# gabrielspmoreira/chameleon_recsys

Measured on AMD Instinct MI355X. Metric: NAR training sessions/sec, higher is better.
Workload: dtype f32

## Files before the change

### chameleon_recsys_amd/_lib.py

```python
import ctypes
import os
from ctypes import c_double, c_float, c_int, c_int32, c_int64, c_long, c_size_t, c_uint32, c_void_p

_HERE = os.path.dirname(os.path.abspath(__file__))
LIB_PATH = os.path.join(_HERE, "libchameleon_nar.so")

P = c_void_p

_SIGNATURES = {
    "cham_neg_sample_workspace_bytes": (c_size_t, [c_int, c_int, c_int]),
    "cham_neg_sample": (c_int, [P, c_int, c_int, P, c_int, c_uint32, c_uint32, c_int, c_int, c_int, c_int, P, P, P, P, P,
                                P, c_size_t, P]),
    "cham_ctx_assemble": (c_int, [P, P, c_int, P, c_int, P, P, P, P, P, P]),
    "cham_set_log_bases": (c_int, [c_float, c_float]),
    "cham_step_ints": (c_int, [P, P, P, P, c_int64, c_int, c_int, P, c_int, P, P, P, P, P, P]),
    "cham_item_dynamic_raw": (c_int, [P, P, c_int, P, P, P, P, P]),
    "cham_norm_stats_from_recent": (c_int, [P, c_int, c_int64, P, P, P, P, P]),
    "cham_norm_stats_from_buffer": (c_int, [P, c_int, c_int64, P, P, P, P, P]),
    "cham_norm_stats_from_rows": (c_int, [P, P, P, c_int, P, P]),
    "cham_row_weights": (c_int, [P, c_int, P, c_size_t, c_int, P, P, P, P]),
    "cham_item_assemble": (c_int, [P, c_int, c_int, c_int, P, c_int, P, c_int, P, P, P, P, c_int, P, P, P, P, P, P]),
    "cham_item_assemble_lds": (c_int, [P, c_int, c_int, c_int, P, c_int, P, c_int, P, P, P, P, c_int, P, c_int, P, c_int, P, P, P, P, P, P]),
    "cham_feature_bwd": (c_int, [P, P, c_int, c_int, P, P, P]),
    "cham_feature_bwd_workspace_bytes": (c_size_t, [c_int]),
    "cham_feature_bwd_ws": (c_int, [P, P, c_int, c_int, P, P, P, c_size_t, P]),
    "cham_emb_grad_scan": (c_int, [P, c_int, c_int, c_int, c_int, P, P, P, c_int, P, P]),
    "cham_group_rows_workspace_bytes": (c_size_t, [c_int]),
    "cham_group_rows_segments_len": (c_size_t, [c_int]),
    "cham_group_rows": (c_int, [P, c_int, c_int, P, P, P, c_size_t, P]),
    "cham_emb_grad_grouped": (c_int, [P, c_int, c_int, c_int, c_int, P, P, P, P, P, P]),
    "cham_dropout": (c_int, [P, P, c_long, c_int, c_int, c_float, c_uint32, c_uint32, c_int, c_int, c_int, P, c_int, c_int, c_int, c_int, P]),
    "cham_dense_rows": (c_int, [P, c_int, P, c_int, c_int, c_int, c_int, P, P, P]),
    "cham_gemm_f32": (c_int, [P, c_int, c_int, P, c_int, c_int, P, c_int, c_int, c_int, c_int, P, c_int, P, c_int, c_int,
                              P, c_int, c_int, c_int, P, c_size_t, c_int, P]),
    "cham_gemm_bf16": (c_int, [P, c_int, c_int, P, c_int, c_int, P, c_int, c_int, c_int, c_int, P, c_int, P, c_int, c_int,
                               P, c_int, c_int, c_int, P, c_size_t, c_int, P]),
    "cham_gemm_f32x3": (c_int, [P, c_int, c_int, P, c_int, c_int, P, c_int, c_int, c_int, c_int, P, c_int, P, c_int, c_int,
                                P, c_int, c_int, c_int, P, c_size_t, c_int, P]),
    "cham_gemm_f32x2h": (c_int, [P, c_int, c_int, P, c_int, c_int, P, c_int, c_int, c_int, c_int, P, c_int,
                                 P, c_int, c_int, c_int, P, c_size_t, c_int, P, P, P]),
    "cham_gemm_f32x3_set_variant": (None, [c_int]),
    "cham_gemm_f32x3_launch_counts": (None, [P, c_int]),
    "cham_gemm_p3": (c_int, [P, c_int64, c_int, P, c_int64, c_int, c_int, P, c_int, c_int, c_int, c_int, P, c_int, P, c_int, c_int, c_int,
                             P, c_size_t, c_int, P]),
    "cham_gemm_b16_dma": (c_int, [P, c_int, P, c_int, c_int, P, c_int, c_int, c_int, c_int, P, c_int, P, c_int, c_int, c_int, P, c_size_t, c_int, P]),
    "cham_gemm_p3_launch_counts": (None, [P, c_int]),
    "cham_gemm_b16_dma_set_nt_wide": (c_int, [c_int]),
    "cham_split3": (c_int, [P, c_int, c_int, c_int, P, c_int64, c_int, P, c_int64, c_int, P]),
    "cham_combine_fwd_p3": (c_int, [P, P, c_int, c_int, c_int, c_int, P, P, c_int64, P]),
    "cham_mulpred_bwd_p3": (c_int, [P, P, P, c_int, c_int, c_int, P, P, c_int64, P, P]),
    "cham_dm_mulpred_p3": (c_int, [P, c_int, c_int, P, c_int64, P, P, c_int, c_int, c_int, P, c_int64, P, P, P]),
    "cham_h2_scale_absmax": (c_int, [P, c_size_t, P, c_size_t, P, P]),
    "cham_h2_scale_rownorm": (c_int, [P, c_long, c_int, c_int, P, P, P]),
    "cham_h2_scale_rownorm2": (c_int, [P, c_long, c_int, c_int, P, P, P, P]),
    "cham_split2h": (c_int, [P, c_int, c_int, c_int, P, c_int64, c_int, P, c_int64, c_int, P, c_int, P]),
    "cham_gemm_h2": (c_int, [P, c_int64, c_int, P, P, c_int64, c_int, P, c_int, P, c_int, c_int, c_int, c_int, P, c_int, P, c_int, c_int, c_int,
                             P, c_size_t, c_int, P]),
    "cham_h2b_block_elements": (c_int, []),
    "cham_gemm_h2b": (c_int, [P, c_int64, c_int, P, P, c_int64, c_int, P, c_int, P, c_int, c_int, c_int, c_int, P, c_int, P, c_int, c_int, c_int,
                              P, c_size_t, c_int, c_int, c_int, c_int, P]),
    "cham_combine_fwd_h2b": (c_int, [P, P, c_int, c_int, c_int, c_int, P, P, c_int64, P, c_int, P]),
    "cham_dm_mulpred_h2_blk": (c_int, [P, c_int, c_int, P, c_int64, P, P, P, P, c_int, c_int, c_int, P, c_int64, P, P, P, P]),
    "cham_gemm_h2_launch_counts": (None, [P, c_int]),
    "cham_gemm_h2_set_nt_wide": (c_int, [c_int]),
    "cham_combine_fwd_h2": (c_int, [P, P, c_int, c_int, c_int, c_int, P, P, c_int64, P, P]),
    "cham_mulpred_bwd_h2": (c_int, [P, P, P, c_int, c_int, c_int, P, P, c_int64, P, P, P]),
    "cham_dm_mulpred_h2": (c_int, [P, c_int, c_int, P, c_int64, P, P, c_int, c_int, c_int, P, c_int64, P, P, P, P]),
    "cham_dm_mulpred_h2h": (c_int, [P, c_int, c_int, P, c_int64, P, P, P, P, c_int, c_int, c_int, P, c_int64, P, P, P, P]),
    "cham_dm_mulpred_b16": (c_int, [P, c_int, c_int, P, P, P, c_int, c_int, c_int, P, P, P, P]),
    "cham_gemm_b16": (c_int, [P, c_int, c_int, P, c_int, c_int, P, c_int, c_int, c_int, c_int, c_int, P, c_int, P, c_int, c_int, c_int,
                              P, c_size_t, c_int, P]),
    "cham_gemm_b16_set_variant": (None, [c_int]),
    "cham_gemm_b16_launch_counts": (None, [P, c_int]),
    "cham_gemm_set_variant": (None, [c_int]),
    "cham_gemm_launch_counts": (None, [P, c_int]),
    "cham_combine_fwd": (c_int, [P, P, c_int, c_int, c_int, c_int, P, P, c_long, c_long, P]),
    "cham_combine_bwd_workspace_bytes": (c_size_t, [c_int, c_int, c_int, c_int]),
    "cham_combine_bwd": (c_int, [P, c_int, c_int, c_int, c_int, P, P, P, P, c_size_t, P]),
    "cham_combine_bwd_gs": (c_int, [P, c_int, c_int, c_int, c_int, P, P, P, P, c_size_t, P, c_size_t, P]),
    "cham_gemm_h2_groupsum_bytes": (c_size_t, [c_int, c_int, c_int]),
    "cham_gemm_h2_dgrad_gs": (c_int, [P, c_int64, c_int, P, P, c_int64, c_int, P, P, c_int, c_int, c_int, c_int, P, c_int, c_int, c_int, c_int, P,
                                      c_size_t, P]),
    "cham_combine_fwd_b16": (c_int, [P, P, c_int, c_int, c_int, c_int, P, P, P]),
    "cham_combine_bwd_b16": (c_int, [P, P, c_int, c_int, c_int, c_int, P, P, P, P, c_size_t, P]),
    "cham_mulpred_bwd_b16": (c_int, [P, P, P, c_int, c_int, c_int, P, P]),
    "cham_mul_rows_b16": (c_int, [P, P, c_int, c_int, c_int, P, P]),
    "cham_score_softmax_fwd_b16": (c_int, [P, c_int, P, P, c_int, c_int, c_float, P, P, P, P, c_float, P, P, P, P]),
    "cham_score_softmax_bwd_b16": (c_int, [P, c_int, P, P, P, c_int, c_int, c_float, c_float, P, P, c_float, P, P, P, P, P]),
    "cham_colsum_b16": (c_int, [P, c_int, c_int, c_int, P, P, c_int, P, c_size_t, P]),
    "cham_cast_b16": (c_int, [P, c_int, c_int, P, P, P]),
    "cham_upcast_b16": (c_int, [P, c_size_t, P, P]),
    "cham_rnn_fwd": (c_int, [c_int, P, P, P, c_int, c_int, c_int, P, P, P, P, P, P, P]),
    "cham_rnn_bwd": (c_int, [c_int, P, P, P, c_int, c_int, c_int, P, P, P, P, P, P]),
    "cham_rnn_coop_workspace_bytes": (c_size_t, [c_int, c_int]),
    "cham_ugrnn_fwd_coop": (c_int, [P, P, P, c_int, c_int, c_int, P, P, P, P, P, c_size_t, P]),
    "cham_ugrnn_bwd_coop": (c_int, [P, P, P, c_int, c_int, c_int, P, P, P, P, P, c_size_t, P]),
    "cham_rnn_coop_timeouts": (c_int, [P, c_int, c_int, P]),
    "cham_ugrnn_point_fwd": (c_int, [P, P, P, c_int, c_int, c_int, c_int, P, P, P, P, P, P]),
    "cham_ugrnn_point_bwd": (c_int, [P, P, P, c_int, c_int, c_int, c_int, P, P, P, P, P, P, P]),
    "cham_transpose_f32": (c_int, [P, c_int, c_int, P, P]),
    "cham_rows_gather": (c_int, [P, P, c_long, c_int, P, P]),
    "cham_rows_scatter": (c_int, [P, P, c_long, c_int, P, P]),
    "cham_mulpred_bwd": (c_int, [P, P, P, c_int, c_int, c_int, P, P]),
    "cham_score_softmax_fwd": (c_int, [P, c_int, P, P, c_int, c_int, c_float, P, P, P, P, c_float, P, P, P, P]),
    "cham_score_softmax_bwd": (c_int, [P, c_int, P, P, P, c_int, c_int, c_float, c_float, P, P, c_float, P, P, P, P, P]),
    "cham_rank_items": (c_int, [P, P, P, P, c_int, c_int, P, P, P, P]),
    "cham_state_workspace_bytes": (c_size_t, [c_int, c_int]),
    "cham_state_update": (c_int, [P, P, c_int, c_int, c_double, P, P, c_int, P, P, P, c_int, c_int, P, P, c_size_t, P]),
    "cham_sumsq_partial": (c_int, [P, c_size_t, P, P]),
    "cham_loss_finalize": (c_int, [P, c_int, c_float, P, c_float, P, P]),
    "cham_adam_tf": (c_int, [P, P, P, P, c_size_t, c_size_t, c_float, c_float, c_float, c_float, c_float, P]),
    "cham_step_scalars_bytes": (c_int, []),
    "cham_step_scalars_set": (c_int, [P, c_uint32, c_uint32, c_int64, c_float, c_float, c_int, P]),
    "cham_neg_sample_dev": (c_int, [P, c_int, c_int, P, c_int, c_uint32, P, c_int, c_int, c_int, c_int, c_int, P, P, P, P, P, P, c_size_t, P]),
    "cham_step_ints_dev": (c_int, [P, P, P, P, P, c_int, c_int, P, c_int, P, P, P, P, P, P]),
    "cham_norm_stats_from_buffer_dev": (c_int, [P, c_int, P, P, P, P, P, P]),
    "cham_score_softmax_bwd_dev": (c_int, [P, c_int, P, P, P, c_int, c_int, c_float, P, P, P, c_float, P, P, P, P, P]),
    "cham_score_softmax_bwd_b16_dev": (c_int, [P, c_int, P, P, P, c_int, c_int, c_float, P, P, P, c_float, P, P, P, P, P]),
    "cham_loss_finalize_dev": (c_int, [P, c_int, P, P, c_float, P, P]),
    "cham_adam_tf_dev": (c_int, [P, P, P, P, c_size_t, c_size_t, c_float, P, c_float, c_float, c_float, P]),
    "cham_accumulate": (c_int, [P, P, c_size_t, c_int, P]),
    "cham_loss_accumulate": (c_int, [P, P, c_int, P]),
    "cham_colsum_workspace_bytes": (c_size_t, [c_int, c_int]),
    "cham_colsum": (c_int, [P, c_int, c_int, c_int, P, P, c_int, P, c_size_t, P]),
    "cham_eval_beyond_accuracy": (c_int, [P, c_int, P, P, c_int, P, c_int, c_int64, P, c_int, c_float, c_float, P, P, P, P]),
    "cham_eval_coverage_seed": (c_int, [P, c_int, c_int64, P, P, P]),
    "cham_eval_coverage_workspace_bytes": (c_size_t, [c_int64]),
    "cham_eval_coverage_count": (c_int, [P, P, c_int64, P, c_size_t, P, P]),
}

EXPORTED_SYMBOLS = tuple(_SIGNATURES.keys())


class ChameleonLibError(RuntimeError):
    pass


_lib = None


def load():
    global _lib
    if _lib is not None:
        return _lib
    if not os.path.exists(LIB_PATH):
        raise ChameleonLibError(
            "HIP extension %s is missing - run `python -c 'import __graft_entry__ as g; g.build()'` "
            "(hipcc --offload-arch=gfx950).  There is no CPU fallback." % LIB_PATH)
    lib = ctypes.CDLL(LIB_PATH)
    for name, (res, args) in _SIGNATURES.items():
        fn = getattr(lib, name)
        fn.restype = res
        fn.argtypes = args
    lib.cham_gemm_h2_set_nt_wide(1 if os.environ.get("CHAM_H2_NT_WIDE", "1") == "1" else 0)
    lib.cham_gemm_b16_dma_set_nt_wide(1 if os.environ.get("CHAM_B16_NT_WIDE", "1") == "1" else 0)
    _lib = lib
    return lib


def check(rc, what):
    if rc != 0:
        raise ChameleonLibError("%s failed with code %d" % (what, rc))


def ptr(t):
# ... 2 lines not shown
```

### chameleon_recsys_amd/csrc/common.h

```cpp
#pragma once
#include <hip/hip_runtime.h>
#include <stdint.h>

#define CHAM_OK 0
#define CHAM_ERR_ARG 22
#define CHAM_ERR_LAUNCH 5

#define CHAM_CHECK_LAUNCH()                                  \
    do {                                                     \
        hipError_t e__ = hipGetLastError();                  \
        if (e__ != hipSuccess) return -CHAM_ERR_LAUNCH;      \
    } while (0)

#include <atomic>
static inline int cham_set_dynamic_lds(const void* kernel, int bytes, std::atomic<unsigned long long>& mask) {
    int dev = 0;
    if (hipGetDevice(&dev) != hipSuccess) return -CHAM_ERR_LAUNCH;
    const unsigned long long bit = 1ull << (dev & 63);
    if (mask.load(std::memory_order_acquire) & bit) return CHAM_OK;
    if (hipFuncSetAttribute(kernel, hipFuncAttributeMaxDynamicSharedMemorySize, bytes) != hipSuccess) return -CHAM_ERR_LAUNCH;
    mask.fetch_or(bit, std::memory_order_release);
    return CHAM_OK;
}
#define CHAM_SET_DYNAMIC_LDS(kernel, bytes)                                                                  \
// ... 50 lines not shown
    for (int r = 0; r < 10; ++r) {
        const uint64_t p0 = (uint64_t)0xD2511F53u * c0;
        const uint64_t p1 = (uint64_t)0xCD9E8D57u * c2;
        const uint32_t n0 = (uint32_t)(p1 >> 32) ^ c1 ^ k0;
        const uint32_t n1 = (uint32_t)p1;
        const uint32_t n2 = (uint32_t)(p0 >> 32) ^ c3 ^ k1;
        const uint32_t n3 = (uint32_t)p0;
        c0 = n0; c1 = n1; c2 = n2; c3 = n3;
        k0 += 0x9E3779B9u; k1 += 0xBB67AE85u;
    }
    return c0;
}
#define CHAM_INF_KEY 0xFFFFFFFFFFFFFFFFull
__device__ __forceinline__ uint64_t philox_sort_key(uint32_t q, uint32_t j, uint32_t b, uint32_t stage,
                                                    uint32_t seed, uint32_t step) {
    return ((uint64_t)philox_rand32(q, j, b, stage, seed, step) << 32) | (uint64_t)q;
}

__device__ __forceinline__ float4 ld4(const float* p) { return *reinterpret_cast<const float4*>(p); }
__device__ __forceinline__ void st4(float* p, const float4& v) { *reinterpret_cast<float4*>(p) = v; }
__device__ __forceinline__ float4 ld4(const __bf16* p) {
    const uint2 u = *reinterpret_cast<const uint2*>(p);
    return make_float4(__uint_as_float(u.x << 16), __uint_as_float(u.x & 0xFFFF0000u), __uint_as_float(u.y << 16),
                       __uint_as_float(u.y & 0xFFFF0000u));
}
__device__ __forceinline__ void st4(__bf16* p, const float4& v) {
    typedef __bf16 bf16x4_t __attribute__((ext_vector_type(4)));
    bf16x4_t b; b[0] = (__bf16)v.x; b[1] = (__bf16)v.y; b[2] = (__bf16)v.z; b[3] = (__bf16)v.w;
    *reinterpret_cast<bf16x4_t*>(p) = b;
}

__device__ __forceinline__ void split3(float a, __bf16& h, __bf16& m, __bf16& l) {
    h = (__bf16)a;
    float r = a - (float)h;
    m = (__bf16)r;
    r -= (float)m;
    l = (__bf16)r;
}

__device__ __forceinline__ void st4_planes(__bf16* p, long long ps, const float4& v) {
    typedef __bf16 bf16x4_t __attribute__((ext_vector_type(4)));
    bf16x4_t h, m, l;
    __bf16 a, b, c;
    split3(v.x, a, b, c); h[0] = a; m[0] = b; l[0] = c;
    split3(v.y, a, b, c); h[1] = a; m[1] = b; l[1] = c;
    split3(v.z, a, b, c); h[2] = a; m[2] = b; l[2] = c;
    split3(v.w, a, b, c); h[3] = a; m[3] = b; l[3] = c;
    *reinterpret_cast<bf16x4_t*>(p) = h;
    *reinterpret_cast<bf16x4_t*>(p + ps) = m;
    *reinterpret_cast<bf16x4_t*>(p + 2 * ps) = l;
}

struct H2Scale { float scale, inv, bound, pad; unsigned max_bits, ticket, pad1, pad2; };
__device__ __forceinline__ void split2h(float xs , _Float16& h, _Float16& l) {
    h = (_Float16)xs;
    l = (_Float16)(xs - (float)h);
}
__device__ __forceinline__ unsigned short h2_keep_sign(_Float16 h, float x) {
    const unsigned short b = __builtin_bit_cast(unsigned short, h);
    return (x > 0.f && b == 0) ? (unsigned short)1 : b;
}
#define H2B_ROWS 256
#define H2B_COLS 32
#ifndef H2B_PAD
#define H2B_PAD 0
#endif
#define H2B_BLOCK (H2B_ROWS * H2B_COLS + H2B_PAD)
__host__ __device__ __forceinline__ size_t h2b_index(size_t row, unsigned col, unsigned col_blocks) {
    return ((row >> 8) * col_blocks + (col >> 5)) * (size_t)H2B_BLOCK + (row & 255u) * H2B_COLS + (col & 31u);
}

__device__ __forceinline__ void st4_planes_h2(_Float16* p, long long ps, const float4& v, float s) {
    typedef unsigned short u16x4_t __attribute__((ext_vector_type(4)));
    typedef _Float16 f16x4_t __attribute__((ext_vector_type(4)));
    u16x4_t h; f16x4_t l;
    _Float16 a, b;
    split2h(v.x * s, a, b); h[0] = h2_keep_sign(a, v.x); l[0] = b;
    split2h(v.y * s, a, b); h[1] = h2_keep_sign(a, v.y); l[1] = b;
    split2h(v.z * s, a, b); h[2] = h2_keep_sign(a, v.z); l[2] = b;
    split2h(v.w * s, a, b); h[3] = h2_keep_sign(a, v.w); l[3] = b;
    *reinterpret_cast<u16x4_t*>(p) = h;
    *reinterpret_cast<f16x4_t*>(p + ps) = l;
}

__device__ __forceinline__ float wave_sum(float v) {
#pragma unroll
    for (int o = 32; o > 0; o >>= 1) v += __shfl_xor(v, o, 64);
    return v;
}
__device__ __forceinline__ float wave_max(float v) {
#pragma unroll
    for (int o = 32; o > 0; o >>= 1) v = fmaxf(v, __shfl_xor(v, o, 64));
    return v;
}
__device__ __forceinline__ float wave_min(float v) {
#pragma unroll
    for (int o = 32; o > 0; o >>= 1) v = fminf(v, __shfl_xor(v, o, 64));
    return v;
}
__device__ __forceinline__ float block_sum(float v, float* red) {
    const int lane = threadIdx.x & 63, w = threadIdx.x >> 6, nw = (blockDim.x + 63) >> 6;
    v = wave_sum(v);
    __syncthreads();
    if (lane == 0) red[w] = v;
    __syncthreads();
    float t = 0.f;
    for (int i = 0; i < nw; ++i) t += red[i];
    return t;
}
```

### chameleon_recsys_amd/csrc/gemm_h2.hip

```cpp
#include "gemm_shared.h"

typedef _Float16 half8 __attribute__((ext_vector_type(8)));
typedef short h2_s16x4 __attribute__((ext_vector_type(4)));

struct H2Params {
    const _Float16* A; const _Float16* B;
    long long a_ps, b_ps;
    int lda, ldb;
    const float* sa; const float* sb;
    float* C; int ldc;
    int M, N, K;
    const float* bias;
    const unsigned short* dref; int ldr;
    int kchunk, splits; float* partial;
    int nbm, nbn, xcd_split, accumulate;
    int a_tiles, b_tiles, r_blk;
    float* gsum; int ggrp, gsk;
};

#define H2_SLAB 8192
#define H2_STAGE (4 * H2_SLAB)
#define H2_RING 4

__device__ __forceinline__ u32x4 h2_rsrc(const void* base, unsigned bytes) {
    const unsigned long long a = (unsigned long long)base;
    u32x4 r;
    r.x = (unsigned)a; r.y = (unsigned)(a >> 32) & 0xFFFFu; r.z = bytes; r.w = 0x00020000u;
    return r;
}

__device__ __forceinline__ void h2_dma_stage(unsigned lds0, unsigned va, unsigned vb, const u32x4& ra0, const u32x4& ra1, const u32x4& rb0,
                                             const u32x4& rb1) {
    unsigned keep;
    const unsigned l1 = lds0 + H2_SLAB, l2 = lds0 + 2 * H2_SLAB, l3 = lds0 + 3 * H2_SLAB;
    asm volatile(
        "s_nop 4\n\t"
        "s_mov_b32 %0, m0\n\t"
        "s_mov_b32 m0, %1\n\ts_nop 0\n\tbuffer_load_dwordx4 %5, %7, 0 offen lds\n\t"
        "s_mov_b32 m0, %2\n\ts_nop 0\n\tbuffer_load_dwordx4 %5, %8, 0 offen lds\n\t"
        "s_mov_b32 m0, %3\n\ts_nop 0\n\tbuffer_load_dwordx4 %6, %9, 0 offen lds\n\t"
        "s_mov_b32 m0, %4\n\ts_nop 0\n\tbuffer_load_dwordx4 %6, %10, 0 offen lds\n\t"
        "s_mov_b32 m0, %0"
        : "=&s"(keep)
        : "s"(lds0), "s"(l1), "s"(l2), "s"(l3), "v"(va), "v"(vb), "s"(ra0), "s"(ra1), "s"(rb0), "s"(rb1)
        : "memory");
}

template <bool TN>
__device__ __forceinline__ half8 h2_frag(const unsigned char* __restrict__ s, unsigned hi_off = 4 * 512) {
    if constexpr (!TN) {
        return *reinterpret_cast<const half8*>(s);
    } else {
        typedef __attribute__((address_space(3))) h2_s16x4 lds_s4;
        const h2_s16x4 lo = __builtin_amdgcn_ds_read_tr16_b64_v4i16((lds_s4*)(s));
        const h2_s16x4 hi = __builtin_amdgcn_ds_read_tr16_b64_v4i16((lds_s4*)(s + hi_off));
        typedef short s16x8 __attribute__((ext_vector_type(8)));
        s16x8 v;
        v[0] = lo[0]; v[1] = lo[1]; v[2] = lo[2]; v[3] = lo[3]; v[4] = hi[0]; v[5] = hi[1]; v[6] = hi[2]; v[7] = hi[3];
        return __builtin_bit_cast(half8, v);
    }
}

__device__ __forceinline__ void h2_barrier() {
    __builtin_amdgcn_fence(__ATOMIC_RELEASE, "workgroup", "local");
    __builtin_amdgcn_s_waitcnt(0xc07f);
    __builtin_amdgcn_s_barrier();
    __builtin_amdgcn_fence(__ATOMIC_ACQUIRE, "workgroup", "local");
    __builtin_amdgcn_sched_barrier(0);
}

template <int EPI, int TM, int TNN>
__device__ __forceinline__ void h2_epilogue(const H2Params& p, floatx16 (&acc)[TM][TNN], int m0, int n0, int wm0, int wn0, int split, int lane) {
    int lane_e = lane;
    asm volatile("" : "+v"(lane_e));
    const int kl = lane_e >> 5, fl = lane_e & 31;
    const float ia = p.sa[1], ib = p.sb[1];
#pragma unroll
    for (int i = 0; i < TM; ++i)
#pragma unroll
        for (int j = 0; j < TNN; ++j)
#pragma unroll
            for (int e = 0; e < 16; ++e) acc[i][j][e] = (acc[i][j][e] * ia) * ib;
    if constexpr (EPI == 3) {
        const int limM = p.M - m0, limN = p.N - n0;
        const __amdgpu_buffer_rsrc_t cw = make_window(p.C + (size_t)m0 * p.ldc + n0);
        const bool rb = p.r_blk != 0;
        const __amdgpu_buffer_rsrc_t dw = make_window(rb ? p.dref + ((size_t)(m0 >> 8) * (size_t)(p.ldr >> 5) + (size_t)(n0 >> 5)) * H2B_BLOCK
                                                         : p.dref + (size_t)m0 * p.ldr + n0);
        const int rstride = rb ? 64 : p.ldr * 2;
        const bool gs = p.gsum != nullptr;
        const int G = gs ? p.ggrp : 1, rbase = m0 + wm0;
        float* gw = gs ? p.gsum + (size_t)(rbase >> 7) * (size_t)p.gsk * (size_t)p.N + n0 + wn0 + fl : nullptr;
        float cur[TNN], hik[TNN];
#pragma unroll
        for (int j = 0; j < TNN; ++j) { cur[j] = 0.f; hik[j] = 0.f; }
        int kk = 0;
        auto emit = [&]() {
#pragma unroll
            for (int j = 0; j < TNN; ++j) {
                const float x = cur[j] + __shfl_xor(cur[j], 32, 64);
                if (kl == 0 && wn0 + j * 32 + fl < limN) gw[(size_t)kk * p.N + j * 32] = x;
            }
            ++kk;
        };
        int bnd = 64;
        auto block_begin = [&](int i) {
            if (!gs) return;
            const int s0 = rbase + 32 * i, gf = s0 / G;
            bnd = (gf + 1) * G - s0;
            if (i > 0 && bnd == G) {
                emit();
#pragma unroll
                for (int j = 0; j < TNN; ++j) cur[j] = 0.f;
            }
        };
        auto block_add = [&](int j, const float (&v)[16]) {
            if (!gs) return;
            float lo = 0.f;
            if (bnd >= 32) {
#pragma unroll
                for (int e = 0; e < 16; ++e) lo += v[e];
            } else {
                float hi = 0.f;
#pragma unroll
                for (int e = 0; e < 16; ++e) {
                    const bool first = (e & 3) + 8 * (e >> 2) + 4 * kl < bnd;
                    lo += first ? v[e] : 0.f;
                    hi += first ? 0.f : v[e];
                }
                hik[j] = hi;
            }
            cur[j] += lo;
        };
        auto block_end = [&]() {
            if (!gs || bnd >= 32) return;
            emit();
#pragma unroll
            for (int j = 0; j < TNN; ++j) cur[j] = hik[j];
        };
        if (limM >= wm0 + TM * 32 && limN >= wn0 + TNN * 32) {
#pragma unroll
            for (int i = 0; i < TM; ++i) {
                block_begin(i);
#pragma unroll
                for (int j = 0; j < TNN; ++j) {
                    const unsigned col = (unsigned)(wn0 + j * 32 + fl), rowb = (unsigned)(wm0 + i * 32 + 4 * kl);
                    const unsigned voff = (rowb * (unsigned)p.ldc + col) * 4u;
                    const unsigned voffr = rb ? (unsigned)((wn0 >> 5) + j) * (unsigned)(H2B_BLOCK * 2) + rowb * 64u + (unsigned)fl * 2u
                                              : (rowb * (unsigned)p.ldr + col) * 2u;
                    unsigned short y[16];
#pragma unroll
                    for (int e = 0; e < 16; ++e) {
                        const int ce = (e & 3) + 8 * (e >> 2);
                        y[e] = __builtin_amdgcn_raw_buffer_load_b16(dw, voffr, ce * rstride, 0);
                    }
                    float v[16];
#pragma unroll
                    for (int e = 0; e < 16; ++e) {
                        const int ce = (e & 3) + 8 * (e >> 2);
                        v[e] = acc[i][j][e] * ((short)y[e] > 0 ? 1.f : 0.2f);
                        __builtin_amdgcn_raw_buffer_store_b32(__float_as_uint(v[e]), cw, voff, ce * p.ldc * 4, 0);
                    }
                    block_add(j, v);
                }
                block_end();
            }
            if (gs) emit();
            return;
        }
#pragma unroll
        for (int i = 0; i < TM; ++i) {
            block_begin(i);
#pragma unroll
            for (int j = 0; j < TNN; ++j) {
                const int col = wn0 + j * 32 + fl;
                const bool cok = col < limN;
                unsigned short y[16];
                unsigned offs[16];
#pragma unroll
                for (int e = 0; e < 16; ++e) {
                    const int row = wm0 + i * 32 + (e & 3) + 8 * (e >> 2) + 4 * kl;
                    const bool ok = cok && row < limM;
                    offs[e] = ok ? ((unsigned)row * (unsigned)p.ldc + (unsigned)col) * 4u : OOB_OFF;
                    const unsigned ro = rb ? (unsigned)((wn0 >> 5) + j) * (unsigned)(H2B_BLOCK * 2) + (unsigned)row * 64u + (unsigned)fl * 2u
                                           : ((unsigned)row * (unsigned)p.ldr + (unsigned)col) * 2u;
                    y[e] = __builtin_amdgcn_raw_buffer_load_b16(dw, ok ? ro : OOB_OFF, 0, 0);
                }
                float v[16];
#pragma unroll
                for (int e = 0; e < 16; ++e) {
                    v[e] = acc[i][j][e] * ((short)y[e] > 0 ? 1.f : 0.2f);
                    __builtin_amdgcn_raw_buffer_store_b32(__float_as_uint(v[e]), cw, offs[e], 0, 0);
                }
                block_add(j, v);
            }
            block_end();
        }
        if (gs) emit();
    } else {
        GemmParams g;
        g.A = nullptr; g.B = nullptr; g.C = p.C; g.M = p.M; g.N = p.N; g.K = p.K; g.lda = 0; g.ldb = 0; g.ldc = p.ldc;
        g.bias = p.bias; g.act = ACT_NONE; g.dref = nullptr; g.ldr = 0; g.dact = ACT_NONE; g.rs = nullptr; g.ldrs = 0; g.rs_div = 1;
        g.accumulate = p.accumulate; g.kchunk = p.kchunk; g.splits = p.splits; g.partial = p.partial; g.nbm = p.nbm; g.nbn = p.nbn; g.xcd_split = p.xcd_split;
        gemm_epilogue<EPI, TM, TNN>(g, acc, m0, n0, wm0, wn0, split, kl, fl);
    }
}

template <bool TN, int EPI>
__global__ __launch_bounds__(512) void gemm_h2_kernel(H2Params p) {
    constexpr int BM = 256, BN = 256, BK = 16, TM = 4, TNN = 2;
    extern __shared__ __attribute__((aligned(1024))) unsigned char h2_smem[];

    const int nwg = p.nbm * p.nbn;
    int tile_m, tile_n, split;
    if (p.xcd_split) {
        const int lin = blockIdx.x + gridDim.x * blockIdx.y, slot = lin >> 3;
        split = (lin & 7) + 8 * (slot / nwg);
        const int t = slot % nwg;
        tile_m = t / p.nbn; tile_n = t % p.nbn;
    } else {
        const int id = blockIdx.x;
        const int q = nwg / 8, rr = nwg % 8, xcd = id % 8;
        const int swz = (xcd < rr ? xcd * (q + 1) : rr * (q + 1) + (xcd - rr) * q) + id / 8;
        tile_m = swz / p.nbn; tile_n = swz % p.nbn;
        split = blockIdx.y;
    }
    const int m0 = tile_m * BM, n0 = tile_n * BN;
    const int kbeg = split * p.kchunk;
    const int kend = min(p.K, kbeg + p.kchunk);
    const int nk = (kend - kbeg + BK - 1) / BK;
    const int lane = threadIdx.x & 63, wave = __builtin_amdgcn_readfirstlane(threadIdx.x >> 6);
    const int wm0 = (wave >> 2) * 128, wn0 = (wave & 3) * 64;

    u32x4 ra[2], rb[2];
    unsigned va, vb, stepa, stepb;
    unsigned tba = 0, tbb = 0;
    int klim = 0;
    if constexpr (!TN) {
        const size_t aall = (size_t)max(p.M - m0, 0) * p.lda * 2, ball = (size_t)max(p.N - n0, 0) * p.ldb * 2, koff = (size_t)kbeg * 2;
        const size_t abytes = aall > koff ? aall - koff : 0, bbytes = ball > koff ? ball - koff : 0;
#pragma unroll
        for (int q = 0; q < 2; ++q) {
            ra[q] = h2_rsrc(p.A + q * p.a_ps + (size_t)m0 * p.lda + kbeg, (unsigned)min(abytes, (size_t)0xFFFFFFF0u));
            rb[q] = h2_rsrc(p.B + q * p.b_ps + (size_t)n0 * p.ldb + kbeg, (unsigned)min(bbytes, (size_t)0xFFFFFFF0u));
        }
        const int row = 32 * wave + (lane >> 1), half = (lane & 1) ^ ((lane >> 4) & 1);
        va = ((unsigned)row * (unsigned)p.lda + 8u * half) * 2u;
        vb = ((unsigned)row * (unsigned)p.ldb + 8u * half) * 2u;
        stepa = stepb = BK * 2;
    } else {
        const size_t abytes = (size_t)max(kend - kbeg, 0) * p.lda * 2, bbytes = (size_t)max(kend - kbeg, 0) * p.ldb * 2;
        const int k = 2 * wave + (lane >> 5), jp = lane & 31, j = ((((jp >> 2) ^ (k & 3)) << 2) | (jp & 3));
        klim = kend - kbeg - (lane >> 2);
        if (p.a_tiles > 0) {
            tba = (unsigned)(p.lda >> 5) * (unsigned)(H2B_BLOCK * 2);
            const size_t t0 = (size_t)(kbeg >> 8), all = ((size_t)p.a_tiles - t0) * tba, skip = (size_t)(m0 >> 5) * (H2B_BLOCK * 2);
#pragma unroll
            for (int q = 0; q < 2; ++q)
                ra[q] = h2_rsrc(p.A + q * p.a_ps + (t0 * (size_t)(p.lda >> 5) + (size_t)(m0 >> 5)) * H2B_BLOCK, (unsigned)min(all > skip ? all - skip : (size_t)0, (size_t)0xFFFFFFF0u));
            va = (unsigned)wave * (unsigned)(H2B_BLOCK * 2) + (unsigned)lane * 16u;
        } else {
#pragma unroll
            for (int q = 0; q < 2; ++q)
                ra[q] = h2_rsrc(p.A + q * p.a_ps + (size_t)kbeg * p.lda + m0, (unsigned)min(abytes > (size_t)m0 * 2 ? abytes - (size_t)m0 * 2 : (size_t)0, (size_t)0xFFFFFFF0u));
            va = ((unsigned)k * (unsigned)p.lda + 8u * j) * 2u;
        }
        if (p.b_tiles > 0) {
            tbb = (unsigned)(p.ldb >> 5) * (unsigned)(H2B_BLOCK * 2);
            const size_t t0 = (size_t)(kbeg >> 8), all = ((size_t)p.b_tiles - t0) * tbb, skip = (size_t)(n0 >> 5) * (H2B_BLOCK * 2);
#pragma unroll
            for (int q = 0; q < 2; ++q)
                rb[q] = h2_rsrc(p.B + q * p.b_ps + (t0 * (size_t)(p.ldb >> 5) + (size_t)(n0 >> 5)) * H2B_BLOCK, (unsigned)min(all > skip ? all - skip : (size_t)0, (size_t)0xFFFFFFF0u));
            vb = (unsigned)wave * (unsigned)(H2B_BLOCK * 2) + (unsigned)lane * 16u;
        } else {
#pragma unroll
            for (int q = 0; q < 2; ++q)
                rb[q] = h2_rsrc(p.B + q * p.b_ps + (size_t)kbeg * p.ldb + n0, (unsigned)min(bbytes > (size_t)n0 * 2 ? bbytes - (size_t)n0 * 2 : (size_t)0, (size_t)0xFFFFFFF0u));
            vb = ((unsigned)k * (unsigned)p.ldb + 8u * j) * 2u;
        }
        stepa = (unsigned)BK * (unsigned)p.lda * 2u; stepb = (unsigned)BK * (unsigned)p.ldb * 2u;
// ... 367 lines not shown
                       reinterpret_cast<H2Scale*>(rec_plain));
    CHAM_CHECK_LAUNCH();
    return CHAM_OK;
}
extern "C" int cham_h2_scale_rownorm(const float* X, long R, int K, int ld, const float* factor, void* rec, void* stream) {
    return cham_h2_scale_rownorm2(X, R, K, ld, factor, rec, nullptr, stream);
}

__global__ __launch_bounds__(256) void k_split2h(const float* __restrict__ X, int R, int Cc, int ld, _Float16* __restrict__ dst, long long ps,
                                                 int ldd, _Float16* __restrict__ dstT, long long psT, int lddT, const H2Scale* __restrict__ rec) {
    const float s = rec->scale;
    const size_t n = (size_t)R * Cc;
    for (size_t i = (size_t)blockIdx.x * 256 + threadIdx.x; i < n; i += (size_t)gridDim.x * 256) {
        const int r = (int)(i / Cc), c = (int)(i % Cc);
        const float x = X[(size_t)r * ld + c];
        _Float16 h, l;
        split2h(x * s, h, l);
        const unsigned short hb = h2_keep_sign(h, x);
        if (dst) { _Float16* d = dst + (size_t)r * ldd + c; *reinterpret_cast<unsigned short*>(d) = hb; d[ps] = l; }
        if (dstT) { _Float16* d = dstT + (size_t)c * lddT + r; *reinterpret_cast<unsigned short*>(d) = hb; d[psT] = l; }
    }
}

extern "C" int cham_split2h(const float* X, int R, int Cc, int ld, void* dst, long long plane_stride, int ldd, void* dstT,
                            long long plane_strideT, int lddT, void* rec, int recompute, void* stream) {
    if (!X || R <= 0 || Cc <= 0 || (!dst && !dstT) || !rec || ((uintptr_t)rec & 15)) return -CHAM_ERR_ARG;
    const size_t n = (size_t)R * Cc;
    if (recompute) {
        if (ld != Cc || (n & 3) || ((uintptr_t)X & 15)) return -CHAM_ERR_ARG;
        const int rc = cham_h2_scale_absmax(X, n, nullptr, 0, rec, stream);
        if (rc != CHAM_OK) return rc;
    }
    int blocks = (int)((n + 255) / 256);
    if (blocks > 8192) blocks = 8192;
    hipLaunchKernelGGL(k_split2h, dim3(blocks), dim3(256), 0, (hipStream_t)stream, X, R, Cc, ld, reinterpret_cast<_Float16*>(dst), plane_stride,
                       ldd, reinterpret_cast<_Float16*>(dstT), plane_strideT, lddT, reinterpret_cast<const H2Scale*>(rec));
    CHAM_CHECK_LAUNCH();
    return CHAM_OK;
}

extern "C" int cham_h2b_block_elements(void) { return H2B_BLOCK; }

static long long g_h2_launches[8];
extern "C" void cham_gemm_h2_launch_counts(long long* out8, int reset) {
    for (int i = 0; i < 8; ++i) { if (out8) out8[i] = g_h2_launches[i]; if (reset) g_h2_launches[i] = 0; }
}

static int g_h2_nt_wide = 1;
extern "C" int cham_gemm_h2_set_nt_wide(int on) { const int was = g_h2_nt_wide; g_h2_nt_wide = on ? 1 : 0; return was; }

template <int EPI, bool ABLK>
static int h2w_launch_l(H2Params& p, hipStream_t st) {
    g_h2_launches[6] = EPI; g_h2_launches[7] = 1; ++g_h2_launches[2];
    if (ABLK) ++g_h2_launches[3];
    constexpr int smem = 2 * H2W_BUF;
    auto k = gemm_h2w_kernel<EPI, ABLK>;
    CHAM_SET_DYNAMIC_LDS(k, smem);
    hipLaunchKernelGGL(k, dim3(p.nbm * p.nbn, 1, 1), dim3(512), smem, st, p);
    CHAM_CHECK_LAUNCH();
    return CHAM_OK;
}
template <int EPI>
static int h2w_launch(H2Params& p, hipStream_t st) {
    return p.a_tiles > 0 ? h2w_launch_l<EPI, true>(p, st) : h2w_launch_l<EPI, false>(p, st);
}

template <bool TN, int EPI>
static int h2_launch(H2Params& p, hipStream_t st) {
    g_h2_launches[6] = EPI; g_h2_launches[7] = p.splits;
    constexpr int smem = H2_RING * H2_STAGE;
    auto k = gemm_h2_kernel<TN, EPI>;
    CHAM_SET_DYNAMIC_LDS(k, smem);
    hipLaunchKernelGGL(k, dim3(p.nbm * p.nbn, p.splits, 1), dim3(512), smem, st, p);
    CHAM_CHECK_LAUNCH();
    return CHAM_OK;
}
extern "C" size_t cham_gemm_h2_groupsum_bytes(int M, int N, int group_rows) {
    if (M <= 0 || N <= 0 || group_rows < 32) return 0;
    return (size_t)2 * ((M + 255) / 256) * (size_t)(127 / group_rows + 2) * (size_t)N * sizeof(float);
}
static int h2_run(const void* A, long long a_plane_stride, int lda, const float* a_scale, const void* B, long long b_plane_stride,
                  int ldb, const float* b_scale, int tn, float* C, int ldc, int M, int N, int K, const float* bias, int act,
                  const void* dref_h, int ldr, int dact, int accumulate, float* workspace, size_t workspace_bytes, int splits_hint,
                  int a_tiles, int b_tiles, int dref_blocked, int group_rows, float* groupsum, size_t groupsum_bytes, void* stream) {
    if (!A || !B || !C || !a_scale || !b_scale || M <= 0 || N <= 0 || K <= 0 || a_tiles < 0 || b_tiles < 0) return -CHAM_ERR_ARG;
    if (groupsum && (tn || !dref_h || group_rows < 32 || groupsum_bytes < cham_gemm_h2_groupsum_bytes(M, N, group_rows) || ((uintptr_t)groupsum & 15)))
        return -CHAM_ERR_ARG;
    {
        const long a_rows = tn ? K : M, b_rows = tn ? K : N;
        if (a_tiles && ((lda & 31) || (long)a_tiles * 256 < a_rows || a_plane_stride < (long long)a_tiles * (lda >> 5) * H2B_BLOCK)) return -CHAM_ERR_ARG;
        if (b_tiles && ((ldb & 31) || (long)b_tiles * 256 < b_rows || b_plane_stride < (long long)b_tiles * (ldb >> 5) * H2B_BLOCK)) return -CHAM_ERR_ARG;
        if (!tn && (b_tiles || (a_tiles && (lda != K || (K & 31) || !g_h2_nt_wide)))) return -CHAM_ERR_ARG;
        if (dref_blocked && (!dref_h || (ldr & 31) || tn)) return -CHAM_ERR_ARG;
    }
    if ((lda & 7) || (ldb & 7) || (a_plane_stride & 7) || (b_plane_stride & 7) || (N & 3) || (ldc & 3)) return -CHAM_ERR_ARG;
    if (((uintptr_t)A | (uintptr_t)B | (uintptr_t)C) & 15) return -CHAM_ERR_ARG;
    if ((size_t)ldc * 4 * 256 >= WINDOW_BYTES || (size_t)ldr * 2 * 256 >= WINDOW_BYTES) return -CHAM_ERR_ARG;
    H2Params p;
    p.A = reinterpret_cast<const _Float16*>(A); p.B = reinterpret_cast<const _Float16*>(B); p.a_ps = a_plane_stride; p.b_ps = b_plane_stride;
    p.lda = lda; p.ldb = ldb; p.sa = a_scale; p.sb = b_scale; p.C = C; p.ldc = ldc; p.M = M; p.N = N; p.K = K; p.bias = bias;
    p.dref = reinterpret_cast<const unsigned short*>(dref_h); p.ldr = ldr; p.partial = workspace; p.xcd_split = 0; p.accumulate = 0;
    p.nbm = (M + 255) / 256; p.nbn = (N + 255) / 256;
    p.a_tiles = a_tiles; p.b_tiles = b_tiles; p.r_blk = dref_blocked ? 1 : 0;
    p.gsum = groupsum; p.ggrp = group_rows; p.gsk = groupsum ? 127 / group_rows + 2 : 0;
    hipStream_t st = (hipStream_t)stream;
    if (!tn) {
        if ((K & 15) || accumulate) return -CHAM_ERR_ARG;
        if ((size_t)256 * lda * 2 >= (1ull << 31) || (size_t)256 * ldb * 2 >= (1ull << 31)) return -CHAM_ERR_ARG;
        p.kchunk = K; p.splits = 1;
        if (dref_h && (bias || act != ACT_NONE || dact != ACT_LEAKY)) return -CHAM_ERR_ARG;
        if (act != ACT_NONE && !(bias && act == ACT_TANH)) return -CHAM_ERR_ARG;
        ++g_h2_launches[0];
        if (groupsum) ++g_h2_launches[5];
        if (g_h2_nt_wide && (K & 31) == 0) {
            if (dref_h) return h2w_launch<3>(p, st);
            if (bias) return act == ACT_TANH ? h2w_launch<2>(p, st) : h2w_launch<5>(p, st);
            return h2w_launch<0>(p, st);
        }
        if (dref_h) return h2_launch<false, 3>(p, st);
        if (bias) return act == ACT_TANH ? h2_launch<false, 2>(p, st) : h2_launch<false, 5>(p, st);
        return h2_launch<false, 0>(p, st);
    }
    if ((M & 255) || (N & 255) || bias || act != ACT_NONE || dref_h) return -CHAM_ERR_ARG;
    if ((size_t)16 * lda * 2 >= (1ull << 31) || (size_t)16 * ldb * 2 >= (1ull << 31)) return -CHAM_ERR_ARG;
    const long tiles = (long)p.nbm * p.nbn;
    int splits = 1;
    if (splits_hint != 1 && workspace) {
        long want = splits_hint > 1 ? splits_hint : (tiles >= 192 ? 1 : (256 + tiles - 1) / tiles);
        const long maxk = (K + 511) / 512;
        if (want > maxk) want = maxk;
        const long maxw = (long)(workspace_bytes / ((size_t)M * N * sizeof(float)));
        if (want > maxw) want = maxw;
        if (splits_hint <= 0 && want >= 8) want = want / 8 * 8;
        if (want > 1) splits = (int)want;
    }
    int kchunk = (K + splits - 1) / splits;
    kchunk = ((kchunk + 15) / 16) * 16;
    p.kchunk = kchunk;
    p.splits = (K + kchunk - 1) / kchunk;
    if ((size_t)kchunk * (lda > ldb ? lda : ldb) * 2 >= 0xFFFFFFF0ull) return -CHAM_ERR_ARG;
    if ((a_tiles || b_tiles) && ((size_t)kchunk + 512 + 64) * (size_t)(lda > ldb ? lda : ldb) * 2 >= 0xFFFFFFF0ull) return -CHAM_ERR_ARG;
    ++g_h2_launches[1];
    if (a_tiles || b_tiles) ++g_h2_launches[4];
    if (p.splits > 1) {
        p.xcd_split = (p.splits % 8 == 0) ? 1 : 0;
        const int rc = h2_launch<true, 6>(p, st);
        if (rc != CHAM_OK) return rc;
        GemmParams g;
        g.A = nullptr; g.B = nullptr; g.C = C; g.M = M; g.N = N; g.K = K; g.lda = 0; g.ldb = 0; g.ldc = ldc; g.bias = nullptr; g.act = ACT_NONE;
        g.dref = nullptr; g.ldr = 0; g.dact = ACT_NONE; g.rs = nullptr; g.ldrs = 0; g.rs_div = 1; g.accumulate = accumulate;
        g.kchunk = kchunk; g.splits = p.splits; g.partial = workspace; g.nbm = p.nbm; g.nbn = p.nbn; g.xcd_split = p.xcd_split;
        launch_splitk_reduce(g, st);
        CHAM_CHECK_LAUNCH();
        return CHAM_OK;
    }
    p.accumulate = accumulate;
    return h2_launch<true, 0>(p, st);
}

extern "C" int cham_gemm_h2b(const void* A, long long a_plane_stride, int lda, const float* a_scale, const void* B, long long b_plane_stride,
                             int ldb, const float* b_scale, int tn, float* C, int ldc, int M, int N, int K, const float* bias, int act,
                             const void* dref_h, int ldr, int dact, int accumulate, float* workspace, size_t workspace_bytes, int splits_hint,
                             int a_tiles, int b_tiles, int dref_blocked, void* stream) {
    return h2_run(A, a_plane_stride, lda, a_scale, B, b_plane_stride, ldb, b_scale, tn, C, ldc, M, N, K, bias, act, dref_h, ldr, dact, accumulate,
                  workspace, workspace_bytes, splits_hint, a_tiles, b_tiles, dref_blocked, 0, nullptr, 0, stream);
}
extern "C" int cham_gemm_h2_dgrad_gs(const void* A, long long a_plane_stride, int lda, const float* a_scale, const void* B, long long b_plane_stride,
                                     int ldb, const float* b_scale, float* C, int ldc, int M, int N, int K, const void* dref_h, int ldr,
                                     int a_tiles, int dref_blocked, int group_rows, float* groupsum, size_t groupsum_bytes, void* stream) {
    if (!groupsum) return -CHAM_ERR_ARG;
    return h2_run(A, a_plane_stride, lda, a_scale, B, b_plane_stride, ldb, b_scale, 0, C, ldc, M, N, K, nullptr, ACT_NONE, dref_h, ldr, ACT_LEAKY, 0,
                  nullptr, 0, 1, a_tiles, 0, dref_blocked, group_rows, groupsum, groupsum_bytes, stream);
}

extern "C" int cham_gemm_h2(const void* A, long long a_plane_stride, int lda, const float* a_scale, const void* B, long long b_plane_stride,
                            int ldb, const float* b_scale, int tn, float* C, int ldc, int M, int N, int K, const float* bias, int act,
                            const void* dref_h, int ldr, int dact, int accumulate, float* workspace, size_t workspace_bytes, int splits_hint,
                            void* stream) {
    return cham_gemm_h2b(A, a_plane_stride, lda, a_scale, B, b_plane_stride, ldb, b_scale, tn, C, ldc, M, N, K, bias, act, dref_h, ldr, dact, accumulate,
                         workspace, workspace_bytes, splits_hint, 0, 0, 0, stream);
}
```

### chameleon_recsys_amd/csrc/scorer.hip

```cpp
#include "common.h"

__device__ __forceinline__ int cand_vrow(int bt, int c, int BT, int N, int pmax, const int* __restrict__ neg_slot) {
    if (c == 0) return BT + bt;
    int s = neg_slot[(size_t)bt * N + (c - 1)];
    if (s < 0) s = pmax;
    return 2 * BT + s;
}

__global__ __launch_bounds__(256) void k_combine_fwd(const float* __restrict__ U, const float* __restrict__ V, int C,
                                                     int BT, int N, int pmax, const int* __restrict__ neg_slot,
                                                     float* __restrict__ Z1, int row_begin) {
    const int row = row_begin + blockIdx.x;
    int u, v;
    if (row < BT) { u = row; v = row; }
    else {
        const int i = row - BT, bt = i / (N + 1), c = i % (N + 1);
        u = bt; v = cand_vrow(bt, c, BT, N, pmax, neg_slot);
    }
    const float4* pu = reinterpret_cast<const float4*>(U + (size_t)u * C);
    const float4* pv = reinterpret_cast<const float4*>(V + (size_t)v * C);
    float4* po = reinterpret_cast<float4*>(Z1 + (size_t)row * C);
    for (int k = threadIdx.x; k < C / 4; k += 256) {
        const float4 a = pu[k], b = pv[k];
        float4 o;
// ... 5 lines not shown

template <typename T>
__global__ __launch_bounds__(256) void k_combine_fwd_cand(const float* __restrict__ U, const float* __restrict__ V, int C,
                                                          int BT, int N, int pmax, const int* __restrict__ neg_slot,
                                                          T* __restrict__ Z1c ) {
    const int bt = blockIdx.x, NC = N + 1;
    const float4* pu = reinterpret_cast<const float4*>(U + (size_t)bt * C);
    T* po = Z1c + (size_t)bt * NC * C;
    for (int k = threadIdx.x; k < C / 4; k += 256) {
        const float4 a = pu[k];
        for (int c0 = 0; c0 < NC; c0 += 4) {
            float4 b[4];
#pragma unroll
            for (int i = 0; i < 4; ++i) {
                const int c = c0 + i < NC ? c0 + i : NC - 1;
                b[i] = reinterpret_cast<const float4*>(V + (size_t)cand_vrow(bt, c, BT, N, pmax, neg_slot) * C)[k];
            }
#pragma unroll
            for (int i = 0; i < 4; ++i) {
                if (c0 + i >= NC) break;
                float4 o;
                o.x = act_fwd(a.x + b[i].x, ACT_LEAKY); o.y = act_fwd(a.y + b[i].y, ACT_LEAKY);
                o.z = act_fwd(a.z + b[i].z, ACT_LEAKY); o.w = act_fwd(a.w + b[i].w, ACT_LEAKY);
                st4(po + (size_t)(c0 + i) * C + 4 * k, o);
            }
        }
    }
}

__global__ __launch_bounds__(256) void k_combine_fwd_cand_p3(const float* __restrict__ U, const float* __restrict__ V, int C,
                                                             int BT, int N, int pmax, const int* __restrict__ neg_slot,
                                                             __bf16* __restrict__ Z1p , long long ps) {
    const int bt = blockIdx.x, NC = N + 1;
    const float4* pu = reinterpret_cast<const float4*>(U + (size_t)bt * C);
    __bf16* po = Z1p + (size_t)bt * NC * C;
    for (int k = threadIdx.x; k < C / 4; k += 256) {
        const float4 a = pu[k];
        for (int c0 = 0; c0 < NC; c0 += 4) {
            float4 b[4];
#pragma unroll
            for (int i = 0; i < 4; ++i) {
                const int c = c0 + i < NC ? c0 + i : NC - 1;
                b[i] = reinterpret_cast<const float4*>(V + (size_t)cand_vrow(bt, c, BT, N, pmax, neg_slot) * C)[k];
            }
#pragma unroll
            for (int i = 0; i < 4; ++i) {
                if (c0 + i >= NC) break;
                float4 o;
                o.x = act_fwd(a.x + b[i].x, ACT_LEAKY); o.y = act_fwd(a.y + b[i].y, ACT_LEAKY);
                o.z = act_fwd(a.z + b[i].z, ACT_LEAKY); o.w = act_fwd(a.w + b[i].w, ACT_LEAKY);
                st4_planes(po + (size_t)(c0 + i) * C + 4 * k, ps, o);
            }
        }
    }
}

__global__ __launch_bounds__(256) void k_combine_fwd_cand_h2(const float* __restrict__ U, const float* __restrict__ V, int C,
                                                             int BT, int N, int pmax, const int* __restrict__ neg_slot,
                                                             _Float16* __restrict__ Z1p , long long ps,
                                                             const H2Scale* __restrict__ rec, int blocked) {
    const int bt = blockIdx.x, NC = N + 1;
    const float sc = rec->scale;
    const float4* pu = reinterpret_cast<const float4*>(U + (size_t)bt * C);
    _Float16* po = Z1p + (size_t)bt * NC * C;
    const size_t grow0 = (size_t)bt * NC;
    const unsigned ncb = (unsigned)C >> 5;
    for (int k = threadIdx.x; k < C / 4; k += 256) {
        const float4 a = pu[k];
        for (int c0 = 0; c0 < NC; c0 += 4) {
            float4 b[4];
#pragma unroll
            for (int i = 0; i < 4; ++i) {
                const int c = c0 + i < NC ? c0 + i : NC - 1;
                b[i] = reinterpret_cast<const float4*>(V + (size_t)cand_vrow(bt, c, BT, N, pmax, neg_slot) * C)[k];
            }
#pragma unroll
            for (int i = 0; i < 4; ++i) {
                if (c0 + i >= NC) break;
                float4 o;
                o.x = act_fwd(a.x + b[i].x, ACT_LEAKY); o.y = act_fwd(a.y + b[i].y, ACT_LEAKY);
                o.z = act_fwd(a.z + b[i].z, ACT_LEAKY); o.w = act_fwd(a.w + b[i].w, ACT_LEAKY);
                st4_planes_h2(blocked ? Z1p + h2b_index(grow0 + (size_t)(c0 + i), 4u * (unsigned)k, ncb) : po + (size_t)(c0 + i) * C + 4 * k, ps, o, sc);
            }
        }
    }
}

template <typename T>
__global__ __launch_bounds__(256) void k_combine_bwd_u(const float* __restrict__ dpre_in, const T* __restrict__ dpre_cand, int C, int BT,
                                                       int N, float* __restrict__ dU, float* __restrict__ dV) {
    const int bt = blockIdx.x;
    const float4* pin = reinterpret_cast<const float4*>(dpre_in + (size_t)bt * C);
    const T* pc = dpre_cand + (size_t)bt * (N + 1) * C;
    for (int k = threadIdx.x; k < C / 4; k += 256) {
        const float4 a = pin[k];
        const float4 p0 = ld4(pc + 4 * k);
        float4 s = make_float4(a.x + p0.x, a.y + p0.y, a.z + p0.z, a.w + p0.w);
        for (int c = 1; c <= N; c += 8) {
            float4 x[8];
#pragma unroll
            for (int u = 0; u < 8; ++u) x[u] = ld4(pc + (size_t)min(c + u, N) * C + 4 * k);
#pragma unroll
            for (int u = 0; u < 8; ++u)
                if (c + u <= N) { s.x += x[u].x; s.y += x[u].y; s.z += x[u].z; s.w += x[u].w; }
        }
        reinterpret_cast<float4*>(dU + (size_t)bt * C)[k] = s;
        reinterpret_cast<float4*>(dV + (size_t)bt * C)[k] = a;
        reinterpret_cast<float4*>(dV + ((size_t)BT + bt) * C)[k] = p0;
    }
}

__global__ __launch_bounds__(256) void k_combine_bwd_u_gs(const float* __restrict__ dpre_in, const float* __restrict__ dpre_cand, int C, int BT,
                                                          int N, const float* __restrict__ gsum, float* __restrict__ dU, float* __restrict__ dV) {
    const int bt = blockIdx.x, G = N + 1, gsk = 127 / G + 2;
    const long r0 = (long)bt * G, r1 = r0 + G - 1;
    const int q0 = (int)(r0 >> 7), q1 = (int)(r1 >> 7);
    const float4* pin = reinterpret_cast<const float4*>(dpre_in + (size_t)bt * C);
    const float4* pc = reinterpret_cast<const float4*>(dpre_cand + (size_t)r0 * C);
    for (int k = threadIdx.x; k < C / 4; k += 256) {
        const float4 a = pin[k], p0 = pc[k];
        float4 s = a;
        for (int q = q0; q <= q1; ++q) {
            const int piece = bt - (int)(((long)q << 7) / G);
            const float4 x = reinterpret_cast<const float4*>(gsum + ((size_t)q * gsk + piece) * C)[k];
            s.x += x.x; s.y += x.y; s.z += x.z; s.w += x.w;
        }
        reinterpret_cast<float4*>(dU + (size_t)bt * C)[k] = s;
        reinterpret_cast<float4*>(dV + (size_t)bt * C)[k] = a;
        reinterpret_cast<float4*>(dV + ((size_t)BT + bt) * C)[k] = p0;
    }
}

#define SLOT_HOT 512
#define SLOT_LIST 2048
__global__ __launch_bounds__(256) void k_slot_bitmap(const int* __restrict__ neg_slot, size_t n, int N, int pmax, int W,
                                                     unsigned* __restrict__ bitmap ) {
    const size_t i = (size_t)blockIdx.x * 256 + threadIdx.x;
    if (i >= n) return;
    const int s = neg_slot[i];
    if (s < 0 || s >= pmax) return;
    const unsigned p = (unsigned)(i / N);
    atomicOr(bitmap + (size_t)s * W + (p >> 5), 1u << (p & 31));
}

__device__ __forceinline__ int block_sum_int(int v, int* red ) {
#pragma unroll
    for (int o = 32; o > 0; o >>= 1) v += __shfl_xor(v, o, 64);
    __syncthreads();
    if ((threadIdx.x & 63) == 0) red[threadIdx.x >> 6] = v;
    __syncthreads();
    return red[0] + red[1] + red[2] + red[3];
}

template <typename T>
__global__ __launch_bounds__(256) void k_slot_reduce(const T* __restrict__ cand , int C, int BT, int N,
                                                     const int* __restrict__ neg_slot, const unsigned* __restrict__ bitmap, int W,
                                                     int nslots, float* __restrict__ partial ,
                                                     float* __restrict__ dV) {
    __shared__ int list[SLOT_HOT];
    __shared__ int red[4];
    const int s = blockIdx.x, chunk = blockIdx.y, tid = threadIdx.x, lane = tid & 63, wave = tid >> 6;
    const unsigned* bm = bitmap + (size_t)s * W;
    int c = 0;
    for (int w = tid; w < W; w += 256) c += __popc(bm[w]);
    const int total = block_sum_int(c, red);
    const bool hot = total > SLOT_HOT;
// ... 307 lines not shown
__global__ __launch_bounds__(256) void k_score_softmax_bwd(const T* __restrict__ S3, const float* __restrict__ w4,
                                                           const float* __restrict__ probs, const unsigned char* __restrict__ mask,
                                                           int BT, int N, float scale ,
                                                           float* __restrict__ ds, T* __restrict__ dS3, float nov_factor,
                                                           const int64_t* __restrict__ neg_ids, const float* __restrict__ pop_norm,
                                                           const float* __restrict__ logits, float inv_tau,
                                                           const float* __restrict__ nov_aux, float inv_log2_base,
                                                           const ChamStepScalars* __restrict__ sc, float tau) {
    const size_t row = (size_t)blockIdx.x * 256 + threadIdx.x;
    const int NC = N + 1;
    if (row >= (size_t)BT * NC) return;
    if (sc) scale = 1.0f / (tau * sc->sum_mask);
    const int bt = (int)(row / NC), c = (int)(row % NC);
    float g = mask[bt] ? (probs[row] - (c == 0 ? 1.f : 0.f)) * scale : 0.f;
    if (nov_factor > 0.f && c > 0 && mask[bt]) {
        const float q = expf(logits[row] * inv_tau - nov_aux[(size_t)bt * 3]) / nov_aux[(size_t)bt * 3 + 1];
        const float nov_c = -log2f(pop_norm[neg_ids[(size_t)bt * N + (c - 1)]]) * inv_log2_base;
        g -= nov_factor * scale * q * (nov_c - nov_aux[(size_t)bt * 3 + 2]);
    }
    ds[row] = g;
    const T* r = S3 + row * K3;
    T* o = dS3 + row * K3;
#pragma unroll
    for (int k = 0; k < K3 / 4; ++k) {
        const float4 x = ld4(r + 4 * k);
        float4 y;
        y.x = g * w4[4 * k] * act_bwd_from_out(x.x, ACT_LEAKY);
        y.y = g * w4[4 * k + 1] * act_bwd_from_out(x.y, ACT_LEAKY);
        y.z = g * w4[4 * k + 2] * act_bwd_from_out(x.z, ACT_LEAKY);
        y.w = g * w4[4 * k + 3] * act_bwd_from_out(x.w, ACT_LEAKY);
        st4(o + 4 * k, y);
    }
}


__global__ __launch_bounds__(256) void k_rank_items(const float* __restrict__ probs, const int64_t* __restrict__ label_next,
                                                    const int64_t* __restrict__ neg_ids, const unsigned char* __restrict__ mask,
                                                    int BT, int N, int64_t* __restrict__ pred_ids, float* __restrict__ pred_probs,
                                                    int32_t* __restrict__ label_rank) {
    extern __shared__ float sp[];
    const int lane = threadIdx.x & 63, w = threadIdx.x >> 6, bt = blockIdx.x * 4 + w;
    const int NC = N + 1;
    float* p = sp + (size_t)w * NC;
    if (bt < BT)
        for (int c = lane; c < NC; c += 64) p[c] = probs[(size_t)bt * NC + c];
    __syncthreads();
    if (bt >= BT) return;
    for (int c = lane; c < NC; c += 64) {
        const float pc = p[c];
        int r = 0;
        for (int j = 0; j < NC; ++j) {
            const float pj = p[j];
            r += (pj > pc) || (pj == pc && j < c);
        }
        pred_ids[(size_t)bt * NC + r] = c == 0 ? label_next[bt] : neg_ids[(size_t)bt * N + (c - 1)];
        pred_probs[(size_t)bt * NC + r] = pc;
        if (c == 0) label_rank[bt] = mask[bt] ? r : -1;
    }
}

extern "C" int cham_combine_fwd(const float* U, const float* V, int C, int BT, int N, int pmax, const int32_t* neg_slot,
                                float* Z1, long row_begin, long row_count, void* stream) {
    if (!U || !V || !neg_slot || !Z1 || (C & 3) || BT <= 0 || N <= 0) return -CHAM_ERR_ARG;
    const long rows = (long)BT + (long)BT * (N + 1);
    if (row_begin < 0 || row_count <= 0 || row_begin + row_count > rows) return -CHAM_ERR_ARG;
    if (row_begin == BT && row_count == (long)BT * (N + 1))
        hipLaunchKernelGGL(k_combine_fwd_cand<float>, dim3((unsigned)BT), dim3(256), 0, (hipStream_t)stream, U, V, C, BT, N, pmax, neg_slot,
                           Z1 + (size_t)BT * C);
    else
        hipLaunchKernelGGL(k_combine_fwd, dim3((unsigned)row_count), dim3(256), 0, (hipStream_t)stream, U, V, C, BT, N, pmax,
                           neg_slot, Z1, (int)row_begin);
    CHAM_CHECK_LAUNCH();
    return CHAM_OK;
}
extern "C" int cham_combine_fwd_b16(const float* U, const float* V, int C, int BT, int N, int pmax, const int32_t* neg_slot,
                                    void* Z1c, void* stream) {
    if (!U || !V || !neg_slot || !Z1c || (C & 3) || BT <= 0 || N <= 0) return -CHAM_ERR_ARG;
    hipLaunchKernelGGL(k_combine_fwd_cand<__bf16>, dim3((unsigned)BT), dim3(256), 0, (hipStream_t)stream, U, V, C, BT, N, pmax, neg_slot,
                       reinterpret_cast<__bf16*>(Z1c));
    CHAM_CHECK_LAUNCH();
    return CHAM_OK;
}

static inline size_t al256(size_t x) { return (x + 255) & ~(size_t)255; }
struct SlotWs { size_t bitmap_bytes, partial_bytes, pad_bytes; int W, nchunk, nchunk_pad; };
static SlotWs slot_ws(int C, int BT, int N, int pmax) {
    SlotWs w;
    w.W = (BT + 31) / 32;
    w.nchunk = (w.W + SLOT_HOT / 32 - 1) / (SLOT_HOT / 32);
    w.nchunk_pad = (int)(((size_t)BT * N + SLOT_LIST - 1) / SLOT_LIST);
    w.bitmap_bytes = al256((size_t)pmax * w.W * sizeof(unsigned));
    w.partial_bytes = al256((size_t)w.nchunk * pmax * C * sizeof(float));
    w.pad_bytes = al256((size_t)w.nchunk_pad * C * sizeof(float));
    return w;
}
extern "C" size_t cham_combine_bwd_workspace_bytes(int C, int BT, int N, int pmax) {
    if (C <= 0 || BT <= 0 || N <= 0 || pmax <= 0) return 0;
    const SlotWs w = slot_ws(C, BT, N, pmax);
    return w.bitmap_bytes + w.partial_bytes + w.pad_bytes;
}

template <typename T>
static int combine_bwd_impl(const float* dpre_in, const T* dpre_cand, int C, int BT, int N, int pmax, const int32_t* neg_slot,
                            float* dU, float* dV, float* workspace, size_t workspace_bytes, void* stream, const float* gsum = nullptr) {
    if (!dpre_in || !dpre_cand || !neg_slot || !dU || !dV || !workspace || (C & 3) || BT <= 0 || N <= 0 || pmax <= 0) return -CHAM_ERR_ARG;
    if (workspace_bytes < cham_combine_bwd_workspace_bytes(C, BT, N, pmax) || ((uintptr_t)workspace & 15)) return -CHAM_ERR_ARG;
    hipStream_t st = (hipStream_t)stream;
    const SlotWs w = slot_ws(C, BT, N, pmax);
    unsigned* bitmap = reinterpret_cast<unsigned*>(workspace);
    float* partial = reinterpret_cast<float*>(reinterpret_cast<char*>(workspace) + w.bitmap_bytes);
    float* pad_partial = reinterpret_cast<float*>(reinterpret_cast<char*>(workspace) + w.bitmap_bytes + w.partial_bytes);
    const size_t n = (size_t)BT * N;
    if constexpr (sizeof(T) == 4) {
        if (gsum) hipLaunchKernelGGL(k_combine_bwd_u_gs, dim3(BT), dim3(256), 0, st, dpre_in, reinterpret_cast<const float*>(dpre_cand), C, BT, N, gsum, dU, dV);
        else hipLaunchKernelGGL(k_combine_bwd_u<T>, dim3(BT), dim3(256), 0, st, dpre_in, dpre_cand, C, BT, N, dU, dV);
    } else {
        hipLaunchKernelGGL(k_combine_bwd_u<T>, dim3(BT), dim3(256), 0, st, dpre_in, dpre_cand, C, BT, N, dU, dV);
    }
    if (hipMemsetAsync(bitmap, 0, (size_t)pmax * w.W * sizeof(unsigned), st) != hipSuccess) return -CHAM_ERR_LAUNCH;
    hipLaunchKernelGGL(k_slot_bitmap, dim3((unsigned)((n + 255) / 256)), dim3(256), 0, st, neg_slot, n, N, pmax, w.W, bitmap);
    hipLaunchKernelGGL(k_slot_reduce<T>, dim3(pmax, w.nchunk), dim3(256), 0, st, dpre_cand, C, BT, N, neg_slot, bitmap, w.W, pmax, partial, dV);
    hipLaunchKernelGGL(k_slot_final, dim3(pmax), dim3(256), 0, st, partial, C, pmax, w.nchunk, BT, bitmap, w.W, dV);
    hipLaunchKernelGGL(k_combine_bwd_slots_partial<T>, dim3(w.nchunk_pad), dim3(256), 0, st, dpre_cand, C, BT, N, neg_slot, pmax,
                       pad_partial, SLOT_LIST);
    hipLaunchKernelGGL(k_combine_bwd_pad_final, dim3(1), dim3(256), 0, st, pad_partial, C, w.nchunk_pad,
                       dV + ((size_t)2 * BT + pmax) * C);
    CHAM_CHECK_LAUNCH();
    return CHAM_OK;
}
extern "C" int cham_combine_bwd(const float* dpre, int C, int BT, int N, int pmax, const int32_t* neg_slot,
                                float* dU, float* dV, float* workspace, size_t workspace_bytes, void* stream) {
    if (!dpre || BT <= 0 || C <= 0) return -CHAM_ERR_ARG;
    return combine_bwd_impl<float>(dpre, dpre + (size_t)BT * C, C, BT, N, pmax, neg_slot, dU, dV, workspace, workspace_bytes, stream);
}
extern "C" int cham_combine_bwd_gs(const float* dpre, int C, int BT, int N, int pmax, const int32_t* neg_slot, float* dU, float* dV,
                                   float* workspace, size_t workspace_bytes, const float* groupsum, size_t groupsum_bytes, void* stream) {
    if (!dpre || BT <= 0 || C <= 0 || !groupsum || N + 1 < 32 || ((uintptr_t)groupsum & 15)) return -CHAM_ERR_ARG;
    const size_t rows = (size_t)BT * (N + 1);
    if (groupsum_bytes < (size_t)2 * ((rows + 255) / 256) * (size_t)(127 / (N + 1) + 2) * (size_t)C * sizeof(float)) return -CHAM_ERR_ARG;
    return combine_bwd_impl<float>(dpre, dpre + (size_t)BT * C, C, BT, N, pmax, neg_slot, dU, dV, workspace, workspace_bytes, stream, groupsum);
}
extern "C" int cham_combine_bwd_b16(const float* dpre_in, const void* dpre_cand, int C, int BT, int N, int pmax, const int32_t* neg_slot,
                                    float* dU, float* dV, float* workspace, size_t workspace_bytes, void* stream) {
    return combine_bwd_impl<__bf16>(dpre_in, reinterpret_cast<const __bf16*>(dpre_cand), C, BT, N, pmax, neg_slot, dU, dV, workspace,
                                    workspace_bytes, stream);
}

extern "C" int cham_mulpred_bwd(float* dM, const float* Z2c, const float* pred, int C, int BT, int N, float* dpred_pre,
                                void* stream) {
    if (!dM || !Z2c || !pred || !dpred_pre || (C & 3) || BT <= 0) return -CHAM_ERR_ARG;
    hipLaunchKernelGGL(k_mulpred_bwd<float>, dim3(BT), dim3(256), 0, (hipStream_t)stream, dM, Z2c, pred, C, N, dpred_pre);
    CHAM_CHECK_LAUNCH();
    return CHAM_OK;
}
extern "C" int cham_mulpred_bwd_b16(void* dM, const void* Z2c, const float* pred, int C, int BT, int N, float* dpred_pre, void* stream) {
    if (!dM || !Z2c || !pred || !dpred_pre || (C & 3) || BT <= 0) return -CHAM_ERR_ARG;
    hipLaunchKernelGGL(k_mulpred_bwd<__bf16>, dim3(BT), dim3(256), 0, (hipStream_t)stream, reinterpret_cast<__bf16*>(dM),
                       reinterpret_cast<const __bf16*>(Z2c), pred, C, N, dpred_pre);
    CHAM_CHECK_LAUNCH();
    return CHAM_OK;
}
extern "C" int cham_combine_fwd_p3(const float* U, const float* V, int C, int BT, int N, int pmax, const int32_t* neg_slot, void* Z1p,
                                   long long plane_stride, void* stream) {
    if (!U || !V || !neg_slot || !Z1p || C <= 0 || (C & 3) || BT < 0 || N < 0 || (plane_stride & 3)) return -CHAM_ERR_ARG;
    if (BT == 0) return CHAM_OK;
    hipLaunchKernelGGL(k_combine_fwd_cand_p3, dim3(BT), dim3(256), 0, (hipStream_t)stream, U, V, C, BT, N, pmax, neg_slot,
// ... 129 lines not shown
```

### chameleon_recsys_amd/nar/nar_model.py

```python
import math
import os

import numpy as np
import torch

from .. import _lib
from .. import _roctx
from .._lib import check, ptr
from .clicked_items_state import lane_stream
from .layout import COL_ITEMEMB, ParamLayout
from .metrics import BEYOND_ACCURACY_PER_CLICK, ItemCoverage

ACT_NONE, ACT_LEAKY, ACT_TANH = 0, 1, 2


class ModeKeys:
    TRAIN = 'train'
    EVAL = 'eval'
    PREDICT = 'infer'


_raw_stream = getattr(torch._C, '_cuda_getCurrentRawStream', None)
_raw_device = getattr(torch._C, '_cuda_getDevice', None)

# ... 50 lines not shown

    def __enter__(self):
        global _VARIABLE_STORE
        self._prev, _VARIABLE_STORE = _VARIABLE_STORE, self.store
        return self.store

    def __exit__(self, *a):
        global _VARIABLE_STORE
        _VARIABLE_STORE = self._prev


_TORCH_DTYPE = {np.dtype(n).str: t for n, t in (('int64', torch.int64), ('int32', torch.int32), ('float32', torch.float32),
                                                   ('uint8', torch.uint8))}


def pack_offsets(arrays, align=256):
    offs, total = {}, 0
    for k, a in arrays.items():
        offs[k] = total
        total += (a.nbytes + align - 1) & ~(align - 1)
    return offs, total


class _PinnedRing:

    def __init__(self, n=4, nbytes=4 << 20):
        self.n, self.nbytes = n, nbytes
        self.bufs, self.events, self.k, self.off = [None] * n, [None] * n, -1, 0

    def begin(self, need):
        self.k = (self.k + 1) % self.n
        if self.events[self.k] is not None:
            self.events[self.k].synchronize()
        if self.bufs[self.k] is None or self.bufs[self.k].numel() < need:
            self.bufs[self.k] = torch.empty(max(need, self.nbytes), dtype=torch.uint8, pin_memory=True)
        self.off = 0

    def stage(self, a):
        n = a.nbytes
        if n == 0 or self.off + n > self.bufs[self.k].numel():
            return torch.from_numpy(a)
        view = self.bufs[self.k][self.off:self.off + n]
        self.off += (n + 255) & ~255
        t = view.view(torch.from_numpy(a).dtype).view(a.shape)
        t.copy_(torch.from_numpy(a))
        return t

    def end(self, stream):
        ev = torch.cuda.Event()
        ev.record(stream)
        self.events[self.k] = ev


class NARRuntime:

    def __init__(self, params, device='cuda:0', seed=42, weights=None):
        self.lib = _lib.load()
        self._views = {}
        if not torch.cuda.is_available():
            raise _lib.ChameleonLibError("no ROCm device visible: the NAR step has no CPU path")
        self.device = torch.device(device)
        self.params = params
        acfg = params['articles_features_config']
        ace = np.ascontiguousarray(params['content_article_embeddings_matrix'], dtype=np.float32)
        self.n_items = acfg['article_id'].get('cardinality', ace.shape[0]) if 'article_id' in acfg else ace.shape[0]
        if self.n_items != ace.shape[0]:
            raise ValueError("article_id cardinality (%d) != ACE rows (%d)" % (self.n_items, ace.shape[0]))
        self.item_id_bits = max(1, int(self.n_items - 1).bit_length())
        self.layout = ParamLayout(params['session_features_config'], acfg, self.n_items, ace.shape[1],
                                  params['CAR_embedding_size'], params['rnn_units'],
                                  params.get('rnn_num_layers', 1), params.get('rnn_cell', 'ugrnn'),
                                  params.get('internal_features_config'), params.get('max_cardinality_for_ohe', 10))
        L = self.layout
        logical = weights if weights is not None else L.init_logical(seed)
        dev = self.device
        self.flat = torch.from_numpy(L.pack(logical)).to(dev)
        self.m = torch.zeros_like(self.flat)
        self.v = torch.zeros_like(self.flat)
        self.grads = torch.zeros_like(self.flat)
        self.global_step = 0
        self.dev_scalars = os.environ.get("CHAM_DEV_SCALARS", "1") == "1"
        self.loss_side = os.environ.get("CHAM_LOSS_SIDE", "1") == "1"
        self.dgrad_groupsum = os.environ.get("CHAM_DGRAD_GROUPSUM", "1") == "1"
        self.feature_bwd_ws = os.environ.get("CHAM_FEATURE_BWD_WS", "1") == "1"
        self.tail_split = os.environ.get("CHAM_TAIL_SPLIT", "1") == "1"
        self.capturing = False
        self.scalars = None
        self.gemm_dtype = params.get('gemm_dtype', 'f32')
        if self.gemm_dtype not in ('f32', 'f32_native', 'bf16'):
            raise ValueError("gemm_dtype must be 'f32', 'f32_native' or 'bf16'")
        self.x3 = self.gemm_dtype == 'f32' and os.environ.get("CHAM_GEMM_X3", "1") == "1"
        self.p3 = self.x3 and os.environ.get("CHAM_GEMM_P3", "1") == "1" and self.layout.C % 256 == 0
        self.h2 = self.p3 and os.environ.get("CHAM_GEMM_H2", "1") == "1"
        blk = os.environ.get("CHAM_H2_BLOCKED", "0")
        self.h2_blocked = (self.h2 and blk in ("1", "dz2", "z1") and os.environ.get("CHAM_H2_NT_WIDE", "1") == "1" and self.layout.C % 32 == 0)
        self.h2_blocked_which = blk if self.h2_blocked else "0"
        mode = os.environ.get("CHAM_S1_H2", "1") if self.h2 else "0"
        self.s1_h2 = mode in ("1", "a")
        self.dm_f16 = self.s1_h2
        self.s1_h2_fwd = mode == "a"
        self.tf_random_seed = int(params.get('tf_random_seed', 42))
        meta = params['articles_metadata']
        self.ace = torch.from_numpy(ace).to(dev)
        self.created = torch.from_numpy(np.ascontiguousarray(meta['created_at_ts'], dtype=np.int64)).to(dev)
        def meta_column(n):
            a = np.asarray(meta[n])
            if n in L.meta_is_float:
                return np.ascontiguousarray(a, dtype=np.float32).view(np.int32).astype(np.int64)
            if acfg[n]['type'] == 'numerical' and not np.issubdtype(a.dtype, np.integer) and not np.array_equal(a, np.round(a)):
                raise ValueError("article feature %r holds non-integer values but its config says dtype %r: declare it "
                                 "{'type': 'numerical', 'dtype': 'float'}" % (n, acfg[n].get('dtype')))
            return a.astype(np.int64)
        if L.meta_names:
            mc = np.stack([meta_column(n) for n in L.meta_names])
        else:
            mc = np.zeros((1, self.n_items), np.int64)
        self.meta_cat = torch.from_numpy(np.ascontiguousarray(mc)).to(dev)
        self.ctx_desc = torch.from_numpy(L.ctx_descriptors()).to(dev)
        self.ctx_emb_groups, self.item_emb_groups = L.ctx_emb_groups(), L.item_emb_groups()
        segs, singles = L.item_segments()
        self.item_segs, self.n_item_segs = torch.from_numpy(np.ascontiguousarray(segs)).to(dev), int(segs.shape[0])
        self.item_singles, self.n_item_singles = torch.from_numpy(np.ascontiguousarray(singles)).to(dev), int(singles.shape[0])
        self.item_lds = L.Fi * 4 * 8 <= 64 * 1024
        self.item_desc = torch.from_numpy(L.item_descriptors()).to(dev)
        self.gemm_ws = torch.empty(64 << 20, dtype=torch.float32, device=dev)
        self.colsum_ws = torch.empty(4 << 20, dtype=torch.float32, device=dev)
        self.side_stream = lane_stream(dev, "side", 0)
        self._side_raw = self.side_stream.cuda_stream
        self.gemm_ws_side = torch.empty(32 << 20, dtype=torch.float32, device=dev)
        self.colsum_ws_side = torch.empty(2 << 20, dtype=torch.float32, device=dev)
        self.wgrad_aux = os.environ.get("CHAM_WGRAD_AUX", "1") == "1"
        self.aux_stream = lane_stream(dev, "aux", 0)
        self._aux_raw = self.aux_stream.cuda_stream
        self.gemm_ws_aux = torch.empty(16 << 20, dtype=torch.float32, device=dev)
        self.colsum_ws_aux = torch.empty(2 << 20, dtype=torch.float32, device=dev)
        self.head_split = os.environ.get("CHAM_HEAD_SPLIT", "1") == "1"
        self.overlap = os.environ.get("CHAM_OVERLAP", "1") == "1"
        self.compact = os.environ.get("CHAM_COMPACT", "1") == "1"
        self.p3_w2_splits = 32
        self.w2_main_rows = 131072
        self.rnn_coop_rows = 131072 if (L.cell == 'ugrnn' and L.Hp == 256 and not L.rnn_stepwise) else -1
        self._rnn_coop_ws = {}
        self.presample = os.environ.get("CHAM_PRESAMPLE", "1") == "1"
        self.upload_stream = lane_stream(dev, "upload")
        self.pinned = _PinnedRing()
        self.sumsq = torch.zeros(1024, dtype=torch.float32, device=dev)
        self.b16 = self.gemm_dtype == 'bf16'
        self.shadow, self._shadow_key, self.weights_version = {}, None, 0
        if self.b16:
            if L.C % 128:
                raise ValueError("gemm_dtype='bf16' needs CAR_embedding_size % 128 == 0")
            for name in ('W2', 'Ws1', 'Ws2', 'Ws3'):
                r, c = L.entries[name].shape
                self.shadow[name] = torch.zeros(r, c, dtype=torch.bfloat16, device=dev)
                self.shadow[name + 'T'] = torch.zeros(c, r, dtype=torch.bfloat16, device=dev)
        self.b16_dma = self.gemm_dtype == 'bf16' and L.C % 256 == 0
        self.dm_fused_b16 = self.gemm_dtype == 'bf16' and L.entries['Ws1'].shape == (L.C, 128) and L.C % 64 == 0
        if self.p3:
            C_ = L.C
            npl, pdt = (2, torch.float16) if self.h2 else (3, torch.bfloat16)
            self.w2p = torch.zeros(npl, C_, C_, dtype=pdt, device=dev)
            self.w2tp = torch.zeros(npl, C_, C_, dtype=pdt, device=dev)
            if self.h2:
                self.sc_w2 = torch.zeros(8, dtype=torch.float32, device=dev)
                self.sc_ws1n = torch.zeros(8, dtype=torch.float32, device=dev)
                self.sc_unit = torch.tensor([16384.0, 1.0 / 16384.0, 1.0, 0, 0, 0, 0, 0], dtype=torch.float32, device=dev)
# ... 143 lines not shown
                     ws.numel() * 4 if ws is not None else 0, splits, _stream()), "cham_gemm_f32")
        if prof is not None:
            e1.record()
            c1 = self._tile_counts()
            tile = next((i for i in range(13) if c1[i] != c0[i]), -1)
            rec = dict(M=M, N=N, K=K, transA=transA, transB=transB, splits=int(c1[15]), act=act, dref=dref is not None, dact=dact,
                       bias=bias is not None, rowscale=rowscale is not None, bf16=bf16, tile=tile, epi=int(c1[14]), ev=(e0, e1))
            if x3:
                x1 = self._tile_counts_x3()
                xt = next((i for i in (0, 1, 2, 4, 5) if x1[i] != x0[i]), -1)
                if xt >= 0:
                    rec.update(x3=True, tile=xt & 3, x2h=xt >= 4, epi=int(x1[6]), splits=int(x1[7]))
            prof.append(rec)

    def _tile_counts(self):
        import ctypes
        out = (ctypes.c_longlong * 16)()
        self.lib.cham_gemm_launch_counts(out, 0)
        return list(out)

    def _tile_counts_x3(self):
        import ctypes
        out = (ctypes.c_longlong * 8)()
        self.lib.cham_gemm_f32x3_launch_counts(out, 0)
        return list(out)

    def gemm_b16(self, A, lda, transA, B, ldb, transB, C, ldc, out_f32, M, N, K, bias=None, act=ACT_NONE, dref=None, ldr=0,
                 dact=ACT_NONE, accumulate=0, splits=1, dma=False):
        ws = None
        if splits != 1:
            ws = self._lane_ws('gemm_ws')
        prof = self.profile
        if prof is not None:
            e0, e1 = torch.cuda.Event(enable_timing=True), torch.cuda.Event(enable_timing=True)
            c0 = self._tile_counts_b16()
            e0.record()
        if dma:
            if prof is not None:
                import ctypes
                cw0 = (ctypes.c_longlong * 8)()
                self.lib.cham_gemm_p3_launch_counts(cw0, 0)
            check(self.lib.cham_gemm_b16_dma(ptr(A), lda, ptr(B), ldb, transA, ptr(C), ldc, M, N, K, ptr(bias), act, ptr(dref), ldr, dact,
                                             accumulate, ptr(ws), ws.numel() * 4 if ws is not None else 0, splits, _stream()), "cham_gemm_b16_dma")
            if prof is not None:
                e1.record()
                import ctypes
                c = (ctypes.c_longlong * 8)()
                self.lib.cham_gemm_p3_launch_counts(c, 0)
                prof.append(dict(M=M, N=N, K=K, transA=transA, transB=transB, splits=int(c[7]), act=act, dref=dref is not None, dact=dact,
                                 bias=bias is not None, rowscale=False, bf16=True, b1=True, b1w=bool(c[4] > cw0[4]), out_f32=int(transA), tile=0, epi=int(c[6]),
                                 ev=(e0, e1)))
            return
        check(self.lib.cham_gemm_b16(ptr(A), lda, transA, ptr(B), ldb, transB, ptr(C), ldc, out_f32, M, N, K, ptr(bias), act, ptr(dref),
                                     ldr, dact, accumulate, ptr(ws), ws.numel() * 4 if ws is not None else 0, splits, _stream()),
              "cham_gemm_b16")
        if prof is not None:
            e1.record()
            c1 = self._tile_counts_b16()
            tile = next((i for i in range(5) if c1[i] != c0[i]), -1)
            prof.append(dict(M=M, N=N, K=K, transA=transA, transB=transB, splits=int(c1[7]), act=act, dref=dref is not None, dact=dact,
                             bias=bias is not None, rowscale=False, bf16=True, b16=True, out_f32=int(c1[5]), tile=tile, epi=int(c1[6]),
                             ev=(e0, e1)))

    def gemm_p3(self, A, a_ps, lda, B, b_ps, ldb, tn, C, ldc, M, N, K, bias=None, act=ACT_NONE, dref_h=None, ldr=0, dact=ACT_NONE,
                accumulate=0, splits=1):
        ws = None
        if splits != 1:
            ws = self._lane_ws('gemm_ws')
        prof = self.profile
        if prof is not None:
            e0, e1 = torch.cuda.Event(enable_timing=True), torch.cuda.Event(enable_timing=True)
            e0.record()
        check(self.lib.cham_gemm_p3(ptr(A), a_ps, lda, ptr(B), b_ps, ldb, tn, ptr(C), ldc, M, N, K, ptr(bias), act, ptr(dref_h), ldr, dact,
                                    accumulate, ptr(ws), ws.numel() * 4 if ws is not None else 0, splits, _stream()), "cham_gemm_p3")
        if prof is not None:
            e1.record()
            import ctypes
            c = (ctypes.c_longlong * 8)()
            self.lib.cham_gemm_p3_launch_counts(c, 0)
            prof.append(dict(M=M, N=N, K=K, transA=tn, transB=0 if tn else 1, splits=int(c[7]), act=act, dref=dref_h is not None, dact=dact,
                             bias=bias is not None, rowscale=False, bf16=False, p3=True, tile=0, epi=int(c[6]), ev=(e0, e1)))

    def gemm_h2(self, A, a_ps, lda, a_sc, B, b_ps, ldb, b_sc, tn, C, ldc, M, N, K, bias=None, act=ACT_NONE, dref_h=None, ldr=0, dact=ACT_NONE,
                accumulate=0, splits=1, a_tiles=0, b_tiles=0, dref_blocked=0, group_rows=0, groupsum=None):
        ws = None
        if splits != 1:
            ws = self._lane_ws('gemm_ws')
        prof = self.profile
        if prof is not None:
            import ctypes
            c0 = (ctypes.c_longlong * 8)()
            self.lib.cham_gemm_h2_launch_counts(c0, 0)
            e0, e1 = torch.cuda.Event(enable_timing=True), torch.cuda.Event(enable_timing=True)
            e0.record()
        if groupsum is not None:
            check(self.lib.cham_gemm_h2_dgrad_gs(ptr(A), a_ps, lda, ptr(a_sc), ptr(B), b_ps, ldb, ptr(b_sc), ptr(C), ldc, M, N, K, ptr(dref_h), ldr,
                                                 a_tiles, dref_blocked, group_rows, ptr(groupsum), groupsum.numel() * 4, _stream()), "cham_gemm_h2_dgrad_gs")
        else:
            check(self.lib.cham_gemm_h2b(ptr(A), a_ps, lda, ptr(a_sc), ptr(B), b_ps, ldb, ptr(b_sc), tn, ptr(C), ldc, M, N, K, ptr(bias), act, ptr(dref_h),
                                         ldr, dact, accumulate, ptr(ws), ws.numel() * 4 if ws is not None else 0, splits, a_tiles, b_tiles, dref_blocked,
                                         _stream()), "cham_gemm_h2b")
        if prof is not None:
            e1.record()
            c = (ctypes.c_longlong * 8)()
            self.lib.cham_gemm_h2_launch_counts(c, 0)
            prof.append(dict(M=M, N=N, K=K, transA=tn, transB=0 if tn else 1, splits=int(c[7]), act=act, dref=dref_h is not None, dact=dact,
                             bias=bias is not None, rowscale=False, bf16=False, h2=True, h2w=bool(c[2] > c0[2]), h2blk=bool(c[3] > c0[3]), tile=0, epi=int(c[6]), ev=(e0, e1)))

    def _tile_counts_b16(self):
        import ctypes
        out = (ctypes.c_longlong * 8)()
        self.lib.cham_gemm_b16_launch_counts(out, 0)
        return list(out)

    def colsum(self, X, ld, R, F, out, w=None, accumulate=0, b16=False):
        ws = self._lane_ws('colsum_ws')
        check((self.lib.cham_colsum_b16 if b16 else self.lib.cham_colsum)(ptr(X), ld, R, F, ptr(w), ptr(out), accumulate, ptr(ws),
                                                                           ws.numel() * 4, _stream()), "cham_colsum")

    def set_step_scalars(self, step=0, max_ts=0, sum_mask=1.0, lr_t=0.0, fields=7, stream=None):
        if self.capturing:
            return
        if self.scalars is None:
            self.scalars = torch.zeros(max(8, self.lib.cham_step_scalars_bytes() // 4), dtype=torch.int32, device=self.device)
        check(self.lib.cham_step_scalars_set(ptr(self.scalars), int(step) & 0xFFFFFFFF, (int(step) + 1) & 0xFFFFFFFF, int(max_ts), float(sum_mask),
                                             float(lr_t), fields, _stream() if stream is None else stream), "cham_step_scalars_set")

    def side(self):
        import contextlib
        return torch.cuda.stream(self.side_stream) if self.overlap else contextlib.nullcontext()

    def fork(self):
        if self.overlap:
            self.side_stream.wait_stream(torch.cuda.current_stream())

    def join(self):
        if self.overlap:
            torch.cuda.current_stream().wait_stream(self.side_stream)


def _h2b_block():
    from .. import _lib
    return int(_lib.load().cham_h2b_block_elements())


def blocked_plane_elements(tiles, C):
    return tiles * (C // 32) * _h2b_block()


def planes_from_blocked(t, tiles, C=None):
    npl = t.shape[0]
    C = t.shape[2] if C is None else C
    blk = _h2b_block()
    flat = t.reshape(npl, -1)[:, :tiles * (C // 32) * blk]
    return flat.reshape(npl, tiles, C // 32, blk)[..., :8192].reshape(npl, tiles, C // 32, 256, 32).permute(0, 1, 3, 2, 4).reshape(npl, tiles * 256, C)


def planes_to_blocked(t):
    npl, R, C = t.shape
    tiles = -(-R // 256)
    blk = _h2b_block()
    pad = torch.zeros(npl, tiles * 256, C, dtype=t.dtype, device=t.device)
    pad[:, :R] = t
    out = torch.zeros(npl, tiles, C // 32, blk, dtype=t.dtype, device=t.device)
    out[..., :8192] = pad.reshape(npl, tiles, 256, C // 32, 32).permute(0, 1, 3, 2, 4).reshape(npl, tiles, C // 32, 8192)
    return out.reshape(npl, -1), tiles


class StepPlan:

    @staticmethod
    def estimate_bytes(L, B, T, N, rt=None):
        rows = B * T * (N + 2)
        need = 4 * (4 * rows * L.C + 2 * rows * (128 + 64 + 32))
        if rt is not None and rt.p3:
            rc = B * T * (N + 1)
            need += 2 * (2 if rt.h2 else 3) * 2 * rc * L.C + 4 * B * T * L.C
            need += 4 * int(rt.lib.cham_group_rows_segments_len(2 * B * T + 20 * N + 1))
        return need

    def allocated_bytes(self):
        seen, total = set(), 0

        def walk(x):
            nonlocal total
            if torch.is_tensor(x):
                st = x.untyped_storage()
                if st.data_ptr() not in seen:
                    seen.add(st.data_ptr())
                    total += st.nbytes()
            elif isinstance(x, (list, tuple)):
                for y in x:
                    walk(y)
            elif isinstance(x, dict):
                for y in x.values():
                    walk(y)
        for v in vars(self).values():
            walk(v)
        return total

    def __init__(self, rt, B, T, N, n_buf, Bg):
        L, dev = rt.layout, rt.device
        self.B, self.T, self.N, self.n_buf, self.Bg = B, T, N, n_buf, Bg
        self.BT = BT = B * T
        self.NC = NC = N + 1
        self.Rc = Rc = BT * NC
        self.Rall = Rall = BT + Rc
        self.pmax = pmax = 20 * N
        self.RV = RV = 2 * BT + pmax + 1
        C, Hp, Fc, Fi = L.C, L.Hp, L.Fc, L.Fi
        self.C = C
        f32 = lambda *s: torch.empty(*s, dtype=torch.float32, device=dev)
        i64 = lambda *s: torch.zeros(*s, dtype=torch.int64, device=dev)
        self._samp = [dict(neg_ids=i64(B, T, N), neg_slot=torch.zeros(B, T, N, dtype=torch.int32, device=dev), pool=i64(pmax),
                           canon=torch.zeros(pmax, dtype=torch.int32, device=dev), meta=torch.zeros(4, dtype=torch.int32, device=dev))
                      for _ in range(2)]
        self.use_sampler_set(0)
        need = rt.lib.cham_combine_bwd_workspace_bytes(L.C, B * T, N, 20 * N)
        if need > rt.gemm_ws.numel() * 4:
            rt.gemm_ws = torch.empty((need + 3) // 4, dtype=torch.float32, device=dev)
        if need > rt.gemm_ws_side.numel() * 4:
            rt.gemm_ws_side = torch.empty((need + 3) // 4, dtype=torch.float32, device=dev)
        self.ws_bytes = rt.lib.cham_neg_sample_workspace_bytes(Bg * (T + 1), int(rt.params['recent_clicks_buffer_max_size']), n_buf)
        self.sampler_ws = torch.empty(self.ws_bytes, dtype=torch.uint8, device=dev)
        self.ids_all = i64(RV)
        self.ref_ts = i64(RV)
        self.rec_raw, self.nov_raw = f32(RV), f32(RV)
        self.stats = f32(3, 8)
        self.stat_scratch = f32(3 * max(1, int(rt.params['recent_clicks_for_normalization'])))
        self.w_rows = f32(RV)
        self.perm = torch.zeros(RV, dtype=torch.int32, device=dev)
        self.seg = torch.zeros(int(rt.lib.cham_group_rows_segments_len(RV)), dtype=torch.int32, device=dev)
        self.group_ws = torch.zeros(int(rt.lib.cham_group_rows_workspace_bytes(RV)) // 4, dtype=torch.int32, device=dev)
        self.Xc_raw, self.Xc_s, self.dXc = f32(BT, Fc), f32(BT, Fc), f32(BT, Fc)
        self.Xi_raw, self.Xi_s, self.dXi = f32(RV, Fi), f32(RV, Fi), f32(RV, Fi)
        self.U, self.dU = f32(BT, C), f32(BT, C)
        self.V, self.dV = f32(RV, C), f32(RV, C)
        b16 = rt.b16
        bf = lambda *s: torch.empty(*s, dtype=torch.bfloat16, device=dev)
        cand = bf if b16 else f32
        if b16:
            self.Z1, self.Z2, self.dZ2, self.dZ1 = f32(BT, C), f32(BT, C), f32(BT, C), f32(BT, C)
            self.Z1c, self.Z2c, self.dZ2c, self.dZ1c, self.Mc = bf(Rc, C), bf(Rc, C), bf(Rc, C), bf(Rc, C), bf(Rc, C)
            self.b2part = f32(BT, C)
        else:
            fused = rt.p3 and rt.dm_fused and 32 <= NC <= 256
            self.Z1 = f32(BT if rt.p3 else Rall, C)
            self.Z2 = f32(Rall, C)
            self.dZ2 = f32(BT if fused else Rall, C)
            self.dZ1 = f32(Rall, C)
        self.p3 = rt.p3
        self.h2 = rt.h2
        if rt.p3:
            self.z1_tiles = self.dz2_tiles = 0
            if rt.h2:
                tiles = -(-Rc // 256) + 1
                if rt.h2_blocked:
                    self.z1_tiles = tiles if rt.h2_blocked_which in ("1", "z1") else 0
                    self.dz2_tiles = tiles if (rt.dm_fused and 32 <= NC <= 256 and rt.h2_blocked_which in ("1", "dz2")) else 0
                self.Z1p = (torch.zeros(2, blocked_plane_elements(self.z1_tiles, C), dtype=torch.float16, device=dev) if self.z1_tiles
                            else torch.zeros(2, Rc, C, dtype=torch.float16, device=dev))
                self.dZ2p = (torch.zeros(2, blocked_plane_elements(self.dz2_tiles, C), dtype=torch.float16, device=dev) if self.dz2_tiles
                             else torch.zeros(2, Rc, C, dtype=torch.float16, device=dev))
                self.sc_z1 = torch.zeros(8, dtype=torch.float32, device=dev)
                self.sc_dz2 = torch.zeros(8, dtype=torch.float32, device=dev)
                self.sc_ds1 = torch.zeros(8, dtype=torch.float32, device=dev)
                self.gsum = (torch.empty(int(rt.lib.cham_gemm_h2_groupsum_bytes(Rc, C, NC)) // 4, dtype=torch.float32, device=dev)
                             if rt.dgrad_groupsum and NC >= 32 and Rc > 0 else None)
            else:
                self.Z1p, self.dZ2p = bf(3, Rc, C), bf(3, Rc, C)
            self.p3_ps = Rc * C
            self.z1_ps = self.Z1p[0].numel()
            self.dz2_ps = self.dZ2p[0].numel()
            self.b2part = f32(BT, C)
        self.seq_len = torch.zeros(B, dtype=torch.int32, device=dev)
        NG = L.NG
        self.xproj = [f32(BT, NG * Hp) for _ in range(L.L)]
        self.dxproj = f32(BT, NG * Hp)
        self.rnn_out = [f32(BT, Hp) for _ in range(L.L)]
        self.hprev = [f32(BT, Hp) for _ in range(L.L)]
        self.G = [f32(BT, Hp) for _ in range(L.L)]
        self.Cc = [f32(BT, Hp) for _ in range(L.L)]
        gru = L.cell == 'gru'
        self.R = [f32(BT, Hp) if gru else None for _ in range(L.L)]
        self.RH = [f32(BT, Hp) if gru else None for _ in range(L.L)]
        self.drnn = f32(BT, Hp)
        self.WhT = f32(NG * Hp, Hp)
        if L.rnn_stepwise:
            self.h_state, self.zh, self.carry = f32(B, Hp), f32(B, 2 * Hp), f32(B, Hp)
            self.dzs, self.direct = f32(B, 2 * Hp), f32(B, Hp)
        self.FC1, self.dFC1 = f32(BT, 512), f32(BT, 512)
        self.pred, self.dpred = f32(BT, C), f32(BT, C)
        self.S1, self.dS1 = cand(Rc, 128), cand(Rc, 128)
        self.S2, self.dS2 = cand(Rc, 64), cand(Rc, 64)
        self.S3, self.dS3 = cand(Rc, 32), cand(Rc, 32)
        self.ds = f32(Rc)
        self.logits, self.probs = f32(BT, NC), f32(BT, NC)
        self.nll = f32(BT)
        self.nov_aux = f32(BT, 3)
        self.mask = torch.zeros(BT, dtype=torch.uint8, device=dev)
        self.loss = torch.zeros(3, dtype=torch.float32, device=dev)
        self.neg_ids_c = i64(BT, N)
        self.neg_slot_c = torch.zeros(BT, N, dtype=torch.int32, device=dev)
        self.Z2f, self.rnn_c, self.drnn_c, self.dxproj_c = f32(BT, C), f32(BT, Hp), f32(BT, Hp), f32(BT, NG * Hp)
        self.pos, self.P = None, BT
        self.created = torch.cuda.Event()
        self.created.record()

    def ensure_rows(self, name):
        t = getattr(self, name)
        if t.shape[0] < self.Rall:
            t = torch.empty(self.Rall, t.shape[1], dtype=t.dtype, device=t.device)
            setattr(self, name, t)
            if hasattr(self, 'nbytes'):
                self.nbytes = self.allocated_bytes()
        return t

    def dropout_buffers(self, rt):
        if not rt.b16:
            self.ensure_rows('Z1'); self.ensure_rows('dZ2')
        if getattr(self, 'Xd', None) is None:
            L, dev = rt.layout, rt.device
            f32 = lambda *s: torch.empty(*s, dtype=torch.float32, device=dev)
            Fw = L.Fc + L.Fi
            self.Xd, self.dXd = f32(self.Rall, Fw), f32(self.Rall, Fw)
            self.dUx, self.dVx = f32(self.BT, Fw), f32(self.RV, Fw)
            self.FC1d = f32(self.BT, 512)
            self.rnn_drop = [f32(self.BT, L.Hp) for _ in range(L.L)]
            need = rt.lib.cham_combine_bwd_workspace_bytes(Fw, self.B * self.T, self.N, self.pmax)
            self.drop_ws = torch.empty((need + 3) // 4, dtype=torch.float32, device=dev)
            if rt.b16:
                self.Z1f, self.dZ1f = f32(self.Rall, L.C), f32(self.Rall, L.C)

    def cand_Z1(self, P=None):
        P = self.P if P is None else P
        n = P * self.NC
        if getattr(self, 'used_p3', False):
            if getattr(self, 'z1_tiles', 0):
                z = planes_from_blocked(self.Z1p, self.z1_tiles, self.C)[:, :n].float()
            else:
                z = self.Z1p[:, :n].float()
            if self.h2:
                return (z[0] + z[1]) * self.sc_z1[1]
            return z[0] + z[1] + z[2]
        if self.Z1.shape[0] == self.BT and hasattr(self, 'Z1c'):
            return self.Z1c[:n].float()
        return self.Z1[P:P + n]

    def use_sampler_set(self, k):
        self._samp_cur = k
        for name, t in self._samp[k].items():
            setattr(self, name, t)

    def full_rows(self, x, group=1):
        x = x[:self.P * group]
        if self.pos is None:
            return x
        out = torch.zeros((self.BT * group,) + tuple(x.shape[1:]), dtype=x.dtype, device=x.device)
        out.view(self.BT, -1)[self.pos.long()] = x.reshape(self.P, -1)
        return out


class NARModuleModel:

    def __init__(self, mode, inputs, labels, session_features_config, articles_features_config, batch_size, lr, keep_prob,
                 negative_samples, negative_sample_from_buffer, content_article_embeddings_matrix, rnn_num_layers=1,
                 softmax_temperature=1.0, reg_weight_decay=0.0, recent_clicks_buffer_hours=1.0,
                 recent_clicks_buffer_max_size=1000, recent_clicks_for_normalization=1000, articles_metadata=None,
                 plot_histograms=False, metrics_top_n=5, elapsed_days_smooth_log_base=1.3, popularity_smooth_log_base=2.0,
                 CAR_embedding_size=256, rnn_units=256, max_cardinality_for_ohe=10, novelty_reg_factor=0.0,
                 diversity_reg_factor=0.0,
                 internal_features_config={'recency': True, 'novelty': True, 'article_content_embeddings': True,
                                           'item_clicked_embeddings': True},
                 eval_cold_start=False, runtime=None, rnn_cell='ugrnn', gemm_dtype='f32'):
        for b in (elapsed_days_smooth_log_base, popularity_smooth_log_base):
            if not (b > 0.0) or b == 1.0:
                raise ValueError("log bases must be > 0 and != 1")
        self.elapsed_days_smooth_log_base = float(elapsed_days_smooth_log_base)
        self.popularity_smooth_log_base = float(popularity_smooth_log_base)
        self.novelty_reg_factor = float(novelty_reg_factor)
        self.is_training = (mode == ModeKeys.TRAIN)
        if self.is_training and not (0.0 < keep_prob <= 1.0):
            raise ValueError("dropout_keep_prob must be in (0, 1]")
        self.mode = mode
        self.inputs, self.labels = inputs, labels
        self.lr, self.keep_prob = lr, keep_prob
        self.negative_samples = negative_samples
        self.negative_sample_from_buffer = negative_sample_from_buffer
        self.softmax_temperature = softmax_temperature
        self.reg_weight_decay = reg_weight_decay
        self.metrics_top_n = metrics_top_n
        self.recent_clicks_for_normalization = recent_clicks_for_normalization
        self.recent_clicks_buffer_max_size = recent_clicks_buffer_max_size
        self.eval_cold_start = eval_cold_start
        if runtime is None and _VARIABLE_STORE is not None and _VARIABLE_STORE.get('runtime') is not None:
            runtime = _VARIABLE_STORE['runtime']
        if runtime is None:
            seed = _VARIABLE_STORE.get('tf_random_seed', 42) if _VARIABLE_STORE is not None else 42
            runtime = NARRuntime(dict(tf_random_seed=seed,session_features_config=session_features_config,
# ... 108 lines not shown
        main, up, ring = torch.cuda.current_stream(), self.rt.upload_stream, self.rt.pinned
        arrs = {k: np.ascontiguousarray(a) for k, a in host.items()}
        out = {}
        if ring is not None:
            offs, total = pack_offsets(arrs)
            ring.begin(total)
            arena = ring.bufs[ring.k]
            bytes_view = arena.numpy()
            for k, a in arrs.items():
                if a.nbytes:
                    bytes_view[offs[k]:offs[k] + a.nbytes] = a.reshape(-1).view(np.uint8)
            with torch.cuda.stream(up if up is not None else main):
                block = torch.empty(max(total, 256), dtype=torch.uint8, device=dev)
                block[:total].copy_(arena[:total], non_blocking=True)
            if up is not None:
                block.record_stream(main)
            for k, a in arrs.items():
                out[k] = block[offs[k]:offs[k] + a.nbytes].view(_TORCH_DTYPE[a.dtype.str]).view(a.shape)
            out['_block'], out['_total'] = block, total
            out['_layout'] = tuple((k, offs[k], a.dtype.str, a.shape) for k, a in arrs.items())
        else:
            for k, a in arrs.items():
                x = torch.from_numpy(a)
                if up is None:
                    out[k] = x.to(dev, non_blocking=True)
                    continue
                with torch.cuda.stream(up):
                    x = x.to(dev, non_blocking=True)
                x.record_stream(main)
                out[k] = x
        out['uploaded'] = torch.cuda.Event()
        out['uploaded'].record(up if up is not None else main)
        if ring is not None:
            ring.end(up if up is not None else main)
        return out

    def _neg_sample(self, pl, d, step, k, stream, which=None):
        rt, st, o = self.rt, self._dev_state, pl._samp[k]
        if which is not None:
            check(rt.lib.cham_neg_sample_dev(ptr(d['aci']), d['Bg'], d['T'] + 1, ptr(st['buffer']), st['buffer'].numel(),
                                             rt.tf_random_seed, ptr(rt.scalars), which, d['row_begin'], d['B'], self.negative_samples,
                                             self.negative_sample_from_buffer, ptr(o['neg_ids']), ptr(o['neg_slot']), ptr(o['pool']),
                                             ptr(o['canon']), ptr(o['meta']), ptr(pl.sampler_ws), pl.ws_bytes, stream), "cham_neg_sample_dev")
            return
        check(rt.lib.cham_neg_sample(ptr(d['aci']), d['Bg'], d['T'] + 1, ptr(st['buffer']), st['buffer'].numel(),
                                     rt.tf_random_seed, step, d['row_begin'], d['B'], self.negative_samples,
                                     self.negative_sample_from_buffer, ptr(o['neg_ids']), ptr(o['neg_slot']), ptr(o['pool']),
                                     ptr(o['canon']), ptr(o['meta']), ptr(pl.sampler_ws), pl.ws_bytes, stream), "cham_neg_sample")

    def presample(self, d):
        rt, state = self.rt, self.articles_recent_pop_norm
        if not (rt.presample and self.is_training and getattr(state, 'is_device', False) and state.stream is not None
                and self._dev_state is not None and self._dev_state.get('device')):
            return False
        pl = rt.plan(d['B'], d['T'], self.negative_samples, self.negative_sample_from_buffer, d['Bg'])
        k, step = 1 - pl._samp_cur, rt.global_step
        if not rt.capturing:
            state.stream.wait_event(pl.created)
            if d.get('uploaded') is not None:
                state.stream.wait_event(d['uploaded'])
            d['aci'].record_stream(state.stream)
        with torch.cuda.stream(state.stream):
            self._neg_sample(pl, d, step, k, state.stream.cuda_stream, which=1 if rt.capturing else None)
            ev = torch.cuda.Event()
            ev.record()
        d['_presampled'] = (pl, k, step, ev)
        return True

    def forward(self, d, step=None):
        depth = _roctx.depth()
        try:
            return self._forward(d, step)
        finally:
            _roctx.unwind(depth)

    def _forward(self, d, step):
        rt, lib, L = self.rt, self.rt.lib, self.rt.layout
        st = self._dev_state
        if st is None:
            raise RuntimeError("feed_state() must be called before every step (ItemsStateUpdaterHook.before_run)")
        B, T, N = d['B'], d['T'], self.negative_samples
        pl = rt.plan(B, T, N, self.negative_sample_from_buffer, d['Bg'])
        self._plan, self._d = pl, d
        pl.used_p3 = False
        check(lib.cham_set_log_bases(self.elapsed_days_smooth_log_base, self.popularity_smooth_log_base), "cham_set_log_bases")
        if d.get('uploaded') is not None:
            torch.cuda.current_stream().wait_event(d['uploaded'])
        s = _stream()
        shadows_ev = None
        if rt.overlap and rt.shadows_stale():
            rt.side_stream.wait_stream(torch.cuda.current_stream())
            with torch.cuda.stream(rt.side_stream):
                rt.refresh_shadows()
                shadows_ev = torch.cuda.Event()
                shadows_ev.record()
        pos, BT, BTf, NC, pmax = d['pos'], d['P'], pl.BT, pl.NC, pl.pmax
        pl.pos, pl.P = pos, BT
        Rc = BT * NC; Rall = BT + Rc; RV = 2 * BT + pmax + 1
        C, Hp, Fc, Fi = L.C, L.Hp, L.Fc, L.Fi
        cell, NGH = (1 if L.cell == 'gru' else 0), L.NG * L.Hp
        if step is None:
            step = rt.global_step if self.is_training else self.eval_step_key(rt.global_step, self._eval_iter)
        p = rt.p
        _roctx.push("K0 negative sampling")
        ps = d.pop('_presampled', None)
        dsc = rt.dev_scalars
        if dsc:
            rt.set_step_scalars(step, d['max_ts'], d['sum_mask'], fields=3, stream=s)
        if ps is not None and ps[0] is pl and ps[2] == step and st.get('device'):
            pl.use_sampler_set(ps[1])
            if ps[3] is not None:
                torch.cuda.current_stream().wait_event(ps[3])
        else:
            self._neg_sample(pl, d, step, pl._samp_cur, s, which=0 if dsc else None)
        if rt.dp_mode in ('sparse', 'sparse_rs') and getattr(rt, 'dp_active', rt.dp_world > 1):
            n1 = d['aci'].numel()
            if getattr(pl, 'touched', None) is None or pl.touched.numel() < n1 + pmax + 1:
                pl.touched = torch.zeros(n1 + pmax + 1, dtype=torch.int32, device=rt.device)
            pl.touched[:n1].copy_(d['aci'].reshape(-1))
            pl.touched[n1:n1 + pmax].copy_(pl.pool)
            pl.touched[n1 + pmax:n1 + pmax + 1].zero_()
            rt.dp_touched = pl.touched[:n1 + pmax + 1]
        neg_ids, neg_slot = pl.neg_ids, pl.neg_slot
        if pos is not None:
            neg_ids, neg_slot = pl.neg_ids_c, pl.neg_slot_c
            check(lib.cham_rows_gather(ptr(pl.neg_ids), ptr(pos), BT, 2 * N, ptr(neg_ids), s), "cham_rows_gather")
            check(lib.cham_rows_gather(ptr(pl.neg_slot), ptr(pos), BT, N, ptr(neg_slot), s), "cham_rows_gather")
        pl.cur_neg_ids, pl.cur_neg_slot = neg_ids, neg_slot
        if getattr(pl, 'grouped_ev', None) is not None:
            torch.cuda.current_stream().wait_event(pl.grouped_ev)
        _roctx.pop(); _roctx.push("K1 features (gather, normalise, scale / center)")
        if dsc:
            check(lib.cham_step_ints_dev(ptr(d['ic_rows']), ptr(d['ln_rows']), ptr(pl.pool), ptr(d['ets_rows']), ptr(rt.scalars), BT, pmax, ptr(d['seq_len']),
                                         B, ptr(d['mask']), ptr(pl.ids_all), ptr(pl.ref_ts), ptr(pl.seq_len), ptr(pl.mask), s), "cham_step_ints_dev")
        else:
            check(lib.cham_step_ints(ptr(d['ic_rows']), ptr(d['ln_rows']), ptr(pl.pool), ptr(d['ets_rows']), int(d['max_ts']), BT, pmax, ptr(d['seq_len']),
                                     B, ptr(d['mask']), ptr(pl.ids_all), ptr(pl.ref_ts), ptr(pl.seq_len), ptr(pl.mask), s), "cham_step_ints")
        pl.grouped_ev = None
        if self.is_training:
            if rt.overlap:
                e_ids = torch.cuda.Event()
                e_ids.record()
                rt.side_stream.wait_event(e_ids)
                with torch.cuda.stream(rt.side_stream):
                    check(lib.cham_group_rows(ptr(pl.ids_all), RV, rt.item_id_bits, ptr(pl.perm), ptr(pl.seg), ptr(pl.group_ws),
                                              pl.group_ws.numel() * 4, _stream()), "cham_group_rows")
                    pl.grouped_ev = torch.cuda.Event()
                    pl.grouped_ev.record()
            else:
                check(lib.cham_group_rows(ptr(pl.ids_all), RV, rt.item_id_bits, ptr(pl.perm), ptr(pl.seg), ptr(pl.group_ws),
                                          pl.group_ws.numel() * 4, s), "cham_group_rows")
        check(lib.cham_item_dynamic_raw(ptr(pl.ids_all), ptr(pl.ref_ts), RV, ptr(rt.created), ptr(st['pop_norm']),
                                        ptr(pl.rec_raw), ptr(pl.nov_raw), s), "cham_item_dynamic_raw")
        if st['n_last'] > 0 and st.get('device') and dsc:
            check(lib.cham_norm_stats_from_buffer_dev(ptr(st['last']), st['n_last'], ptr(rt.scalars), ptr(rt.created),
                                                      ptr(st['pop_norm']), ptr(pl.stat_scratch), ptr(pl.stats), s),
                  "cham_norm_stats_from_buffer_dev")
        elif st['n_last'] > 0 and st.get('device'):
            check(lib.cham_norm_stats_from_buffer(ptr(st['last']), st['n_last'], d['max_ts'], ptr(rt.created),
                                                  ptr(st['pop_norm']), ptr(pl.stat_scratch), ptr(pl.stats), s),
                  "cham_norm_stats_from_buffer")
        elif st['n_last'] > 0:
            check(lib.cham_norm_stats_from_recent(ptr(st['last']), st['n_last'], d['max_ts'], ptr(rt.created),
                                                  ptr(st['pop_norm']), ptr(pl.stat_scratch), ptr(pl.stats), s),
                  "cham_norm_stats_from_recent")
        else:
            check(lib.cham_row_weights(ptr(pl.ids_all), 2 * BT, ptr(neg_slot), BT * N, pmax, ptr(pl.pool),
# ... 27 lines not shown
            keep, Fw, e1, e2 = float(self.keep_prob), Fc + Fi, L.entries['W1c'], L.entries['W1i']
            assert e2.offset == e1.offset + e1.size
            W1 = rt.flat[e1.offset:e2.offset + e2.size].view(Fw, C)
            gW1 = rt.grads[e1.offset:e2.offset + e2.size].view(Fw, C)

            def dropout(x, y, rows, cols, ld, site_first, site_rest, group, posmap, col_split=None, col_shift=0):
                check(lib.cham_dropout(ptr(x), ptr(y), rows, cols, ld, keep, rt.tf_random_seed, step & 0xFFFFFFFF, site_first, site_rest,
                                       group, ptr(posmap), T, d['row_begin'], cols if col_split is None else col_split, col_shift,
                                       _stream()), "cham_dropout")
            self._drop = dict(fn=dropout, W1=W1, gW1=gW1, Fw=Fw)
            check(lib.cham_dense_rows(ptr(pl.Xc_s), Fc, ptr(pl.Xi_s), Fi, BT, N, pmax, ptr(neg_slot), ptr(pl.Xd), s), "cham_dense_rows")
            dropout(pl.Xd, pl.Xd, BT, Fw, Fw, 16, 16, 1, pos, Fc, Fc - L.f_ctx)
            dropout(pl.Xd[BT:], pl.Xd[BT:], Rc, Fw, Fw, 17, 18, NC, pos, Fc, Fc - L.f_ctx)
            rt.gemm(pl.Xd, W1, pl.Z1, BT, C, Fw, Fw, C, C, bias=p('b1'), act=ACT_LEAKY)
        else:
            self._drop = None
            rt.gemm(pl.Xc_s, p('W1c'), pl.U, BT, C, Fc, Fc, C, C, bias=p('b1'))
            rt.gemm(pl.Xi_s, p('W1i'), pl.V, RV, C, Fi, Fi, C, C)
            if not head_split:
                check(lib.cham_combine_fwd(ptr(pl.U), ptr(pl.V), C, BT, N, pmax, ptr(neg_slot), ptr(pl.Z1), 0, BT, s), "cham_combine_fwd")
        if not head_split:
            rt.gemm(pl.Z1, p('W2'), pl.Z2, BT, C, C, C, C, C, bias=p('b2'), act=ACT_TANH)
        rt.fork()
        with rt.side():
            if head_split:
                if not drop:
                    check(lib.cham_combine_fwd(ptr(pl.U), ptr(pl.V), C, BT, N, pmax, ptr(neg_slot), ptr(pl.Z1), 0, BT, _stream()), "cham_combine_fwd")
                rt.gemm(pl.Z1, p('W2'), pl.Z2, BT, C, C, C, C, C, bias=p('b2'), act=ACT_TANH)
            x, ldx, K = pl.Z2, C, C
            if pos is not None:
                pl.Z2f.zero_()
                check(lib.cham_rows_scatter(ptr(pl.Z2), ptr(pos), BT, C, ptr(pl.Z2f), _stream()), "cham_rows_scatter")
                x = pl.Z2f
            for l in range(L.L):
                rt.gemm(x, p('rnn%d/Wx' % l), pl.xproj[l], BTf, NGH, K, ldx, NGH, NGH, bias=p('rnn%d/b' % l))
                if L.rnn_stepwise:
                    pl.h_state.zero_()
                    for t in range(T):
                        rt.gemm(pl.h_state, p('rnn%d/Wh' % l), pl.zh, B, 2 * Hp, Hp, Hp, 2 * Hp, 2 * Hp, force_f32=True)
                        check(lib.cham_ugrnn_point_fwd(ptr(pl.xproj[l]), ptr(pl.zh), ptr(pl.seq_len), B, T, t, Hp, ptr(pl.h_state),
                                                       ptr(pl.rnn_out[l]), ptr(pl.hprev[l]), ptr(pl.G[l]), ptr(pl.Cc[l]), _stream()),
                              "cham_ugrnn_point_fwd")
                elif 0 < Rc <= rt.rnn_coop_rows and B <= 1024:
                    ws = rt.rnn_coop_ws(B)
                    check(lib.cham_ugrnn_fwd_coop(ptr(pl.xproj[l]), ptr(p('rnn%d/Wh' % l)), ptr(pl.seq_len), B, T, Hp, ptr(pl.rnn_out[l]),
                                                  ptr(pl.hprev[l]), ptr(pl.G[l]), ptr(pl.Cc[l]), ptr(ws), ws.numel(), _stream()), "cham_ugrnn_fwd_coop")
                else:
                    check(lib.cham_rnn_fwd(cell, ptr(pl.xproj[l]), ptr(p('rnn%d/Wh' % l)), ptr(pl.seq_len), B, T, Hp,
                                           ptr(pl.rnn_out[l]), ptr(pl.hprev[l]), ptr(pl.G[l]), ptr(pl.Cc[l]), ptr(pl.R[l]),
                                           ptr(pl.RH[l]), _stream()), "cham_rnn_fwd")
                x, ldx, K = pl.rnn_out[l], Hp, Hp
                if drop:
                    dropout(pl.rnn_out[l], pl.rnn_drop[l], BTf, Hp, Hp, 20 + l, 20 + l, 1, None)
                    x = pl.rnn_drop[l]
            if pos is not None:
                check(lib.cham_rows_gather(ptr(x), ptr(pos), BT, Hp, ptr(pl.rnn_c), _stream()), "cham_rows_gather")
                x = pl.rnn_c
            rt.gemm(x, p('Wf1'), pl.FC1, BT, 512, Hp, Hp, 512, 512, bias=p('bf1'), act=ACT_LEAKY)
            fc1 = pl.FC1
            if drop:
                dropout(pl.FC1, pl.FC1d, BT, 512, 512, 19, 19, 1, pos)
                fc1 = pl.FC1d
            rt.gemm(fc1, p('Wf2'), pl.pred, BT, C, 512, 512, C, C, bias=p('bf2'), act=ACT_TANH)
        if rt.b16:
            sh = rt.shadow
            if drop:
                rt.gemm(pl.Xd[BT:], self._drop['W1'], pl.Z1f[BT:], Rc, C, Fc + Fi, Fc + Fi, C, C, bias=p('b1'), act=ACT_LEAKY)
                check(lib.cham_cast_b16(pl.Z1f[BT:].data_ptr(), Rc, C, ptr(pl.Z1c), None, s), "cham_cast_b16")
            else:
                check(lib.cham_combine_fwd_b16(ptr(pl.U), ptr(pl.V), C, BT, N, pmax, ptr(neg_slot), ptr(pl.Z1c), s), "cham_combine_fwd_b16")
            rt.gemm_b16(pl.Z1c, C, 0, sh['W2T'], C, 1, pl.Z2c, C, 0, Rc, C, C, bias=p('b2'), act=ACT_TANH, dma=rt.b16_dma)
            rt.join()
            check(lib.cham_mul_rows_b16(ptr(pl.Z2c), ptr(pl.pred), C, BT, NC, ptr(pl.Mc), s), "cham_mul_rows_b16")
            rt.gemm_b16(pl.Mc, C, 0, sh['Ws1T'], C, 1, pl.S1, 128, 0, Rc, 128, C, bias=p('bs1'), act=ACT_LEAKY)
            rt.gemm_b16(pl.S1, 128, 0, sh['Ws2T'], 128, 1, pl.S2, 64, 0, Rc, 64, 128, bias=p('bs2'), act=ACT_LEAKY)
            rt.gemm_b16(pl.S2, 64, 0, sh['Ws3T'], 64, 1, pl.S3, 32, 0, Rc, 32, 64, bias=p('bs3'), act=ACT_LEAKY)
            softmax_fwd = lib.cham_score_softmax_fwd_b16
        else:
            use_p3 = pl.used_p3 = rt.p3 and not drop and Rc > 0
            if drop:
                rt.gemm(pl.Xd[BT:], self._drop['W1'], pl.Z1[BT:], Rc, C, Fc + Fi, Fc + Fi, C, C, bias=p('b1'), act=ACT_LEAKY)
            elif use_p3 and rt.h2:
                check(lib.cham_h2_scale_absmax(ptr(pl.U), BT * C, ptr(pl.V), RV * C, ptr(pl.sc_z1), s), "cham_h2_scale_absmax")
                check(lib.cham_combine_fwd_h2b(ptr(pl.U), ptr(pl.V), C, BT, N, pmax, ptr(neg_slot), ptr(pl.Z1p), pl.z1_ps, ptr(pl.sc_z1), 1 if pl.z1_tiles else 0, s),
                      "cham_combine_fwd_h2")
            elif use_p3:
                check(lib.cham_combine_fwd_p3(ptr(pl.U), ptr(pl.V), C, BT, N, pmax, ptr(neg_slot), ptr(pl.Z1p), pl.p3_ps, s), "cham_combine_fwd_p3")
            else:
                check(lib.cham_combine_fwd(ptr(pl.U), ptr(pl.V), C, BT, N, pmax, ptr(neg_slot), ptr(pl.Z1), BT, Rc, s), "cham_combine_fwd")
            if use_p3 and rt.h2:
                rt.gemm_h2(pl.Z1p, pl.z1_ps, C, pl.sc_z1, rt.w2tp, C * C, C, rt.sc_w2, 0, pl.Z2[BT:], C, Rc, C, C, bias=p('b2'), act=ACT_TANH, a_tiles=pl.z1_tiles)
            elif use_p3:
                rt.gemm_p3(pl.Z1p, pl.p3_ps, C, rt.w2tp, C * C, C, 0, pl.Z2[BT:], C, Rc, C, C, bias=p('b2'), act=ACT_TANH)
            else:
                rt.gemm(pl.Z1[BT:], p('W2'), pl.Z2[BT:], Rc, C, C, C, C, C, bias=p('b2'), act=ACT_TANH)
            rt.join()
            _roctx.pop(); _roctx.push("K5 scorer, softmax, loss")
            Z2c = pl.Z2[BT:Rall]
            rt.gemm(Z2c, p('Ws1'), pl.S1, Rc, 128, C, C, 128, 128, bias=p('bs1'), act=ACT_LEAKY, rowscale=pl.pred, ldrs=C, rs_div=NC,
                    h2scales=(rt.sc_unit, rt.sc_ws1n) if rt.s1_h2_fwd else None)
            rt.gemm(pl.S1, p('Ws2'), pl.S2, Rc, 64, 128, 128, 64, 64, bias=p('bs2'), act=ACT_LEAKY)
            rt.gemm(pl.S2, p('Ws3'), pl.S3, Rc, 32, 64, 64, 32, 32, bias=p('bs3'), act=ACT_LEAKY)
            softmax_fwd = lib.cham_score_softmax_fwd
        check(softmax_fwd(ptr(pl.S3), 32, ptr(p('Ws4')), ptr(p('bs4')), BT, N, float(self.softmax_temperature),
                          ptr(pl.mask), ptr(pl.logits), ptr(pl.probs), ptr(pl.nll), self.novelty_reg_factor,
                          ptr(neg_ids), ptr(st['pop_norm']), ptr(pl.nov_aux), s), "cham_score_softmax_fwd")
        def loss_kernels(s):
            check(lib.cham_sumsq_partial(ptr(rt.flat), L.n_reg, ptr(rt.sumsq), s), "cham_sumsq_partial")
            if dsc:
                check(lib.cham_loss_finalize_dev(ptr(pl.nll), BT, ptr(rt.scalars), ptr(rt.sumsq), float(self.reg_weight_decay), ptr(pl.loss), s),
                      "cham_loss_finalize_dev")
            else:
                check(lib.cham_loss_finalize(ptr(pl.nll), BT, d['sum_mask'], ptr(rt.sumsq), float(self.reg_weight_decay), ptr(pl.loss), s),
                      "cham_loss_finalize")
        if getattr(self, '_defer_loss', False) and rt.overlap and rt.loss_side:
            e_nll = torch.cuda.Event(); e_nll.record()
            rt.side_stream.wait_event(e_nll)
            with torch.cuda.stream(rt.side_stream):
                loss_kernels(_stream())
        else:
            loss_kernels(s)
        _roctx.pop()
        self.total_loss = pl.loss
        if not self.is_training and st.get('device'):
            self.articles_recent_pop_norm.note_consumed(d['aci'])
        return pl

    def backward(self):
        rt, lib, L = self.rt, self.rt.lib, self.rt.layout
        pl, d = self._plan, self._d
        check(lib.cham_set_log_bases(self.elapsed_days_smooth_log_base, self.popularity_smooth_log_base), "cham_set_log_bases")
        s = _stream()
        B, T, N = pl.B, pl.T, pl.N
        pos, BT, BTf, NC, pmax = pl.pos, pl.P, pl.BT, pl.NC, pl.pmax
        Rc = BT * NC; Rall = BT + Rc; RV = 2 * BT + pmax + 1
        neg_ids, neg_slot = pl.cur_neg_ids, pl.cur_neg_slot
        C, Hp, Fc, Fi = L.C, L.Hp, L.Fc, L.Fi
        cell, NGH = (1 if L.cell == 'gru' else 0), L.NG * L.Hp
        p, g = rt.p, rt.g
        main_stream, on = torch.cuda.current_stream(), rt.overlap
        b16 = rt.b16
        sh = rt.shadow
        drop = self._drop
        dropout = drop['fn'] if drop else None
        use_p3 = getattr(pl, 'used_p3', False)

        def mark():
            if not on:
                return None
            ev = torch.cuda.Event(); ev.record()
            return ev

        import contextlib

        @contextlib.contextmanager
        def side(*events):
            if not on:
                yield
                return
            for ev in events:
                rt.side_stream.wait_event(ev)
            with torch.cuda.stream(rt.side_stream):
                yield

        def main_wait(ev):
            if on:
                main_stream.wait_event(ev)

# ... 51 lines not shown
            if b16:
                rt.gemm_b16(pl.S1, 128, 1, pl.dS2, 64, 0, g('Ws2'), 64, 1, 128, 64, Rc, splits=0)
                rt.colsum(pl.dS2, 64, Rc, 64, g('bs2'), b16=True)
                rt.gemm_b16(pl.S2, 64, 1, pl.dS3, 32, 0, g('Ws3'), 32, 1, 64, 32, Rc, splits=0)
                rt.colsum(pl.dS3, 32, Rc, 32, g('bs3'), b16=True)
                rt.colsum(pl.S3, 32, Rc, 32, g('Ws4'), w=pl.ds, b16=True)
            else:
                rt.gemm(pl.S1, pl.dS2, g('Ws2'), 128, 64, Rc, 128, 64, 64, transA=1, splits=0)
                rt.colsum(pl.dS2, 64, Rc, 64, g('bs2'))
                rt.gemm(pl.S2, pl.dS3, g('Ws3'), 64, 32, Rc, 64, 32, 32, transA=1, splits=0)
                rt.colsum(pl.dS3, 32, Rc, 32, g('bs3'))
                rt.colsum(pl.S3, 32, Rc, 32, g('Ws4'), w=pl.ds)
            rt.colsum(pl.ds, 1, Rc, 1, g('bs4'))
        crit_first = on and (not b16 or pos is not None)
        w2_main = bool(on and use_p3 and 0 < Rc <= rt.w2_main_rows)
        use_aux = bool(on and rt.wgrad_aux and use_p3 and not w2_main and not b16 and L.L == 1 and cell == 0 and not L.rnn_stepwise and not drop)
        def ws1_wgrad():
            if b16:
                rt.gemm_b16(pl.Mc, C, 1, pl.dS1, 128, 0, g('Ws1'), 128, 1, C, 128, Rc, splits=0)
                rt.colsum(pl.dS1, 128, Rc, 128, g('bs1'), b16=True)
            else:
                rt.gemm(Z2c, pl.dS1, g('Ws1'), C, 128, Rc, C, 128, 128, transA=1, rowscale=pl.pred, ldrs=C, rs_div=NC, splits=0,
                        h2scales=(rt.sc_unit, pl.sc_ds1) if (rt.s1_h2 and use_p3) else None)
                rt.colsum(pl.dS1, 128, Rc, 128, g('bs1'))
        with side(e_start, e_dS1):
            ws1_wgrad()
            if not crit_first:
                scorer_small_wgrads()
        if dm_fused:
            prof = rt.profile
            if prof is not None:
                e0, e1 = torch.cuda.Event(enable_timing=True), torch.cuda.Event(enable_timing=True)
                e0.record()
            if h2 and pl.dz2_tiles:
                f16 = rt.dm_f16
                check(lib.cham_dm_mulpred_h2_blk(ptr(pl.dS1), 128, 128, ptr(rt.ws1h if f16 else rt.ws1p), C * 128, ptr(pl.sc_ds1) if f16 else None,
                                                 ptr(rt.sc_ws1n) if f16 else None, ptr(Z2c), ptr(pl.pred), C, BT, N, ptr(pl.dZ2p), pl.dz2_ps, ptr(pl.sc_dz2),
                                                 ptr(pl.dpred), ptr(pl.b2part), s), "cham_dm_mulpred_h2_blk")
            elif h2:
                if rt.dm_f16:
                    check(lib.cham_dm_mulpred_h2h(ptr(pl.dS1), 128, 128, ptr(rt.ws1h), C * 128, ptr(pl.sc_ds1), ptr(rt.sc_ws1n), ptr(Z2c), ptr(pl.pred),
                                                  C, BT, N, ptr(pl.dZ2p), pl.dz2_ps, ptr(pl.sc_dz2), ptr(pl.dpred), ptr(pl.b2part), s), "cham_dm_mulpred_h2h")
                else:
                    check(lib.cham_dm_mulpred_h2(ptr(pl.dS1), 128, 128, ptr(rt.ws1p), C * 128, ptr(Z2c), ptr(pl.pred), C, BT, N, ptr(pl.dZ2p), pl.dz2_ps,
                                                 ptr(pl.sc_dz2), ptr(pl.dpred), ptr(pl.b2part), s), "cham_dm_mulpred_h2")
            else:
                check(lib.cham_dm_mulpred_p3(ptr(pl.dS1), 128, 128, ptr(rt.ws1p), C * 128, ptr(Z2c), ptr(pl.pred), C, BT, N, ptr(pl.dZ2p), pl.p3_ps,
                                             ptr(pl.dpred), ptr(pl.b2part), s), "cham_dm_mulpred_p3")
            if prof is not None:
                e1.record()
                prof.append(dict(M=Rc, N=C, K=128, transA=0, transB=1, splits=1, act=0, dref=False, dact=0, bias=False, rowscale=False, bf16=False,
                                 dmf=True, h2out=bool(h2), f16p=bool(h2 and rt.dm_f16), tile=0, epi=0, ev=(e0, e1)))
        elif dm_fused_b16:
            prof = rt.profile
            if prof is not None:
                e0, e1 = torch.cuda.Event(enable_timing=True), torch.cuda.Event(enable_timing=True)
                e0.record()
            check(lib.cham_dm_mulpred_b16(ptr(pl.dS1), 128, 128, ptr(sh['Ws1']), ptr(Z2c), ptr(pl.pred), C, BT, N, ptr(dZ2c), ptr(pl.dpred),
                                          ptr(pl.b2part), s), "cham_dm_mulpred_b16")
            if prof is not None:
                e1.record()
                prof.append(dict(M=Rc, N=C, K=128, transA=0, transB=1, splits=1, act=0, dref=False, dact=0, bias=False, rowscale=False, bf16=True,
                                 dmf=True, tile=0, epi=0, ev=(e0, e1)))
        elif h2:
            check(lib.cham_mulpred_bwd_h2(ptr(dZ2c), ptr(Z2c), ptr(pl.pred), C, BT, N, ptr(pl.dpred), ptr(pl.dZ2p), pl.dz2_ps, ptr(pl.b2part),
                                          ptr(pl.sc_dz2), s), "cham_mulpred_bwd_h2")
        elif use_p3:
            check(lib.cham_mulpred_bwd_p3(ptr(dZ2c), ptr(Z2c), ptr(pl.pred), C, BT, N, ptr(pl.dpred), ptr(pl.dZ2p), pl.p3_ps, ptr(pl.b2part), s),
                  "cham_mulpred_bwd_p3")
        else:
            check((lib.cham_mulpred_bwd_b16 if b16 else lib.cham_mulpred_bwd)(ptr(dZ2c), ptr(Z2c), ptr(pl.pred), C, BT, N, ptr(pl.dpred), s),
                  "cham_mulpred_bwd")
        e_dZ2c = mark()
        if b16:
            rt.gemm_b16(dZ2c, C, 0, sh['W2'], C, 1, pl.dZ1c, C, 0, Rc, C, C, dref=pl.Z1c, ldr=C, dact=ACT_LEAKY, dma=rt.b16_dma)
        def w2_wgrad_planes(splits):
            if h2:
                rt.gemm_h2(pl.Z1p, pl.z1_ps, C, pl.sc_z1, pl.dZ2p, pl.dz2_ps, C, pl.sc_dz2, 1, g('W2'), C, C, C, Rc, splits=splits,
                           a_tiles=pl.z1_tiles, b_tiles=pl.dz2_tiles)
            else:
                rt.gemm_p3(pl.Z1p, pl.p3_ps, C, pl.dZ2p, pl.p3_ps, C, 1, g('W2'), C, C, C, Rc, splits=splits)
        if h2:
            gsum = getattr(pl, 'gsum', None) if not drop else None
            rt.gemm_h2(pl.dZ2p, pl.dz2_ps, C, pl.sc_dz2, rt.w2p, C * C, C, rt.sc_w2, 0, pl.dZ1[BT:], C, Rc, C, C, dref_h=pl.Z1p, ldr=C, dact=ACT_LEAKY,
                       a_tiles=pl.dz2_tiles, dref_blocked=1 if pl.z1_tiles else 0, group_rows=NC, groupsum=gsum)
        elif use_p3:
            rt.gemm_p3(pl.dZ2p, pl.p3_ps, C, rt.w2p, C * C, C, 0, pl.dZ1[BT:], C, Rc, C, C, dref_h=pl.Z1p, ldr=C, dact=ACT_LEAKY)
        elif not b16 and Rc > 0:
            rt.gemm(pl.dZ2[BT:Rall], p('W2'), pl.dZ1[BT:Rall], Rc, C, C, C, C, C, transB=1, dref=pl.Z1[BT:Rall], ldr=C, dact=ACT_LEAKY)
        e_cdgrad = mark()
        e_w2main = None
        if w2_main:
            w2_wgrad_planes(0)
            e_w2main = mark()
        last = L.L - 1
        deferred_w2 = None
        with side(e_dZ2c):
            ss = _stream()
            rnn_y = (lambda l: pl.rnn_drop[l]) if drop else (lambda l: pl.rnn_out[l])

            def fc_wgrads():
                rt.gemm(pl.FC1d if drop else pl.FC1, pl.dpred, g('Wf2'), 512, C, BT, 512, C, C, transA=1, splits=0)
                rt.colsum(pl.dpred, C, BT, C, g('bf2'))
                rt.gemm(pl.rnn_c if pos is not None else rnn_y(last), pl.dFC1, g('Wf1'), Hp, 512, BT, Hp, 512, 512, transA=1, splits=0)
                rt.colsum(pl.dFC1, 512, BT, 512, g('bf1'))
                if crit_first:
                    scorer_small_wgrads()
                if rt.dp_early_bucket is not None and not self._accumulating:
                    rt.dp_early_bucket(rt.grads)
            rt.gemm(pl.dpred, p('Wf2'), pl.dFC1, BT, 512, C, C, C, 512, transB=1, dref=pl.FC1, ldr=512, dact=ACT_LEAKY)
            if drop:
                dropout(pl.dFC1, pl.dFC1, BT, 512, 512, 19, 19, 1, pos)
            if not crit_first:
                fc_wgrads()
            if pos is not None:
                rt.gemm(pl.dFC1, p('Wf1'), pl.drnn_c, BT, Hp, 512, 512, 512, Hp, transB=1)
                pl.drnn.zero_()
                check(lib.cham_rows_scatter(ptr(pl.drnn_c), ptr(pos), BT, Hp, ptr(pl.drnn), ss), "cham_rows_scatter")
            else:
                rt.gemm(pl.dFC1, p('Wf1'), pl.drnn, BT, Hp, 512, 512, 512, Hp, transB=1)
            if drop:
                dropout(pl.drnn, pl.drnn, BTf, Hp, Hp, 20 + last, 20 + last, 1, None)
            for l in range(last, -1, -1):
                if L.rnn_stepwise:
                    pl.carry.zero_()
                    for t in range(T - 1, -1, -1):
                        check(lib.cham_ugrnn_point_bwd(ptr(pl.drnn), ptr(pl.carry), ptr(pl.seq_len), B, T, t, Hp, ptr(pl.hprev[l]),
                                                       ptr(pl.G[l]), ptr(pl.Cc[l]), ptr(pl.dxproj), ptr(pl.dzs), ptr(pl.direct), ss),
                              "cham_ugrnn_point_bwd")
                        pl.carry.copy_(pl.direct)
                        rt.gemm(pl.dzs, p('rnn%d/Wh' % l), pl.carry, B, Hp, 2 * Hp, 2 * Hp, 2 * Hp, Hp, transB=1, accumulate=1, force_f32=True)
                elif 0 < Rc <= rt.rnn_coop_rows and B <= 1024:
                    ws = rt.rnn_coop_ws(B)
                    check(lib.cham_ugrnn_bwd_coop(ptr(pl.drnn), ptr(p('rnn%d/Wh' % l)), ptr(pl.seq_len), B, T, Hp, ptr(pl.hprev[l]), ptr(pl.G[l]),
                                                  ptr(pl.Cc[l]), ptr(pl.dxproj), ptr(ws), ws.numel(), ss), "cham_ugrnn_bwd_coop")
                else:
                    check(lib.cham_transpose_f32(ptr(p('rnn%d/Wh' % l)), Hp, 2 * Hp, ptr(pl.WhT), ss), "cham_transpose_f32")
                    if cell == 1:
                        check(lib.cham_transpose_f32(ptr(p('rnn%d/Wch' % l)), Hp, Hp, pl.WhT[2 * Hp:].data_ptr(), ss), "cham_transpose_f32")
                    check(lib.cham_rnn_bwd(cell, ptr(pl.drnn), ptr(pl.WhT), ptr(pl.seq_len), B, T, Hp, ptr(pl.hprev[l]), ptr(pl.G[l]),
                                           ptr(pl.Cc[l]), ptr(pl.R[l]), ptr(pl.dxproj), ss), "cham_rnn_bwd")
                if l == 0:
                    dxp = pl.dxproj
                    if pos is not None:
                        dxp = pl.dxproj_c
                        check(lib.cham_rows_gather(ptr(pl.dxproj), ptr(pos), BT, NGH, ptr(dxp), ss), "cham_rows_gather")
                    rt.gemm(dxp, p('rnn0/Wx'), pl.dZ2, BT, C, NGH, NGH, NGH, C, transB=1, dref=pl.Z2, ldr=C, dact=ACT_TANH)
                    rt.gemm(pl.dZ2, p('W2'), pl.dZ1, BT, C, C, C, C, C, transB=1, dref=pl.Z1, ldr=C, dact=ACT_LEAKY)
                    e_dZ1in = mark()
                    if crit_first and not use_aux:
                        fc_wgrads()
                    if b16:
                        rt.gemm_b16(pl.Z1c, C, 1, dZ2c, C, 0, g('W2'), C, 1, C, C, Rc, splits=0, dma=rt.b16_dma)
                        rt.gemm(pl.Z1, pl.dZ2, g('W2'), C, C, BT, C, C, C, transA=1, splits=0, accumulate=1)
                        if dm_fused_b16:
                            rt.colsum(pl.b2part, C, BT, C, g('b2'))
                        else:
                            rt.colsum(dZ2c, C, Rc, C, g('b2'), b16=True)
                        rt.colsum(pl.dZ2, C, BT, C, g('b2'), accumulate=1)
                    elif use_p3 and use_aux:
                        with aux(e_dZ1in):
                            if crit_first:
                                fc_wgrads()
                            rt.colsum(pl.b2part, C, BT, C, g('b2'))
                            rt.colsum(pl.dZ2, C, BT, C, g('b2'), accumulate=1)
                            rt.gemm(pl.Z2, dxp, g('rnn0/Wx'), C, NGH, BT, C, NGH, NGH, transA=1, splits=0)
                            rt.gemm(pl.hprev[0], pl.dxproj, g('rnn0/Wh'), Hp, 2 * Hp, BTf, Hp, NGH, 2 * Hp, transA=1, splits=0, force_f32=True)
                            rt.colsum(pl.dxproj, NGH, BTf, NGH, g('rnn0/b'))
# ... 555 lines not shown
```

### include/chameleon_nar.h

```cpp
#ifndef CHAMELEON_NAR_H
#define CHAMELEON_NAR_H
#include <stddef.h>
#include <stdint.h>
#ifdef __cplusplus
extern "C" {
#endif

#define CHAM_ACT_NONE 0
#define CHAM_ACT_LEAKY 1
#define CHAM_ACT_TANH 2

size_t cham_neg_sample_workspace_bytes(int n_aci, int buf_size, int n_from_buffer);
int cham_neg_sample(const int64_t* aci, int Bg, int T1, const int64_t* buffer, int buf_size, uint32_t seed, uint32_t step,
                    int row_begin, int row_count, int N, int n_from_buffer, int64_t* neg_ids, int32_t* neg_slot,
                    int64_t* pool, int32_t* canon, int32_t* meta, void* workspace, size_t workspace_bytes, void* stream);

int cham_ctx_assemble(const int64_t* cat, const float* num, int R, const int64_t* desc, int F, const float* params,
                      const float* gamma, const float* beta, float* xraw, float* xs, void* stream);
int cham_set_log_bases(float elapsed_days_smooth_log_base, float popularity_smooth_log_base);

int cham_step_ints(const int64_t* ic_rows, const int64_t* ln_rows, const int64_t* pool, const int64_t* ets_rows, int64_t max_ts, int BT, int pmax,
                   const int32_t* seq_len_in, int B, const uint8_t* mask_in, int64_t* ids_all, int64_t* ref_ts, int32_t* seq_len, uint8_t* mask,
                   void* stream);

// ... 46 lines not shown
int cham_gemm_f32x3(const float* A, int lda, int transA, const float* B, int ldb, int transB, float* C, int ldc, int M, int N,
                    int K, const float* bias, int act, const float* dref, int ldr, int dact, const float* rowscale, int ldrs,
                    int rs_div, int accumulate, float* workspace, size_t workspace_bytes, int splits_hint, void* stream);
void cham_gemm_f32x3_set_variant(int variant);
void cham_gemm_f32x3_launch_counts(long long* out8, int reset);

int cham_gemm_f32x2h(const float* A, int lda, int transA, const float* B, int ldb, int transB, float* C, int ldc, int M, int N, int K,
                     const float* bias, int act, const float* rowscale, int ldrs, int rs_div, int accumulate, float* workspace,
                     size_t workspace_bytes, int splits_hint, const float* sa_rec, const float* sb_rec, void* stream);

int cham_gemm_p3(const void* A, long long a_plane_stride, int lda, const void* B, long long b_plane_stride, int ldb, int tn, float* C,
                 int ldc, int M, int N, int K, const float* bias, int act, const void* dref_h, int ldr, int dact, int accumulate,
                 float* workspace, size_t workspace_bytes, int splits_hint, void* stream);

int cham_gemm_b16_dma(const void* A, int lda, const void* B, int ldb, int tn, void* C, int ldc, int M, int N, int K, const float* bias,
                      int act, const void* dref, int ldr, int dact, int accumulate, float* workspace, size_t workspace_bytes,
                      int splits_hint, void* stream);
void cham_gemm_p3_launch_counts(long long* out8, int reset);
int cham_gemm_b16_dma_set_nt_wide(int on);
int cham_split3(const float* X, int R, int Cc, int ld, void* dst, long long plane_stride, int ldd, void* dstT, long long plane_strideT,
                int lddT, void* stream);

int cham_h2_scale_absmax(const float* x0, size_t n0, const float* x1, size_t n1, void* rec, void* stream);
int cham_h2_scale_rownorm(const float* X, long R, int K, int ld, const float* factor, void* rec, void* stream);
int cham_h2_scale_rownorm2(const float* X, long R, int K, int ld, const float* factor, void* rec, void* rec_plain, void* stream);
int cham_split2h(const float* X, int R, int Cc, int ld, void* dst, long long plane_stride, int ldd, void* dstT, long long plane_strideT,
                 int lddT, void* rec, int recompute, void* stream);
int cham_gemm_h2(const void* A, long long a_plane_stride, int lda, const float* a_scale, const void* B, long long b_plane_stride, int ldb,
                 const float* b_scale, int tn, float* C, int ldc, int M, int N, int K, const float* bias, int act, const void* dref_h, int ldr,
                 int dact, int accumulate, float* workspace, size_t workspace_bytes, int splits_hint, void* stream);
void cham_gemm_h2_launch_counts(long long* out8, int reset);
int cham_gemm_h2_set_nt_wide(int on);
int cham_h2b_block_elements(void);
int cham_gemm_h2b(const void* A, long long a_plane_stride, int lda, const float* a_scale, const void* B, long long b_plane_stride, int ldb,
                  const float* b_scale, int tn, float* C, int ldc, int M, int N, int K, const float* bias, int act, const void* dref_h, int ldr,
                  int dact, int accumulate, float* workspace, size_t workspace_bytes, int splits_hint, int a_tiles, int b_tiles,
                  int dref_blocked, void* stream);
int cham_combine_fwd_h2b(const float* U, const float* V, int C, int BT, int N, int pmax, const int32_t* neg_slot, void* Z1p,
                         long long plane_stride, const void* scale_rec, int blocked, void* stream);
int cham_dm_mulpred_h2_blk(const float* dS1, int lds1, int K, const void* Wp, long long w_plane_stride, const void* ds1_scale_rec,
                           const void* w_scale_rec, const float* Z2c, const float* pred, int C, int BT, int N, void* dZ2p,
                           long long out_plane_stride, const void* out_scale_rec, float* dpred_pre, float* col_part, void* stream);
int cham_combine_fwd_h2(const float* U, const float* V, int C, int BT, int N, int pmax, const int32_t* neg_slot, void* Z1p,
                        long long plane_stride, const void* scale_rec, void* stream);
int cham_mulpred_bwd_h2(const float* dM, const float* Z2c, const float* pred, int C, int BT, int N, float* dpred_pre, void* dZ2p,
                        long long plane_stride, float* col_part, const void* scale_rec, void* stream);
int cham_dm_mulpred_h2(const float* dS1, int lds1, int K, const void* Wp, long long w_plane_stride, const float* Z2c, const float* pred,
                       int C, int BT, int N, void* dZ2p, long long out_plane_stride, const void* out_scale_rec, float* dpred_pre,
                       float* col_part, void* stream);
int cham_dm_mulpred_h2h(const float* dS1, int lds1, int K, const void* Wh, long long w_plane_stride, const void* ds1_scale_rec,
                        const void* w_scale_rec, const float* Z2c, const float* pred, int C, int BT, int N, void* dZ2p,
                        long long out_plane_stride, const void* out_scale_rec, float* dpred_pre, float* col_part, void* stream);
int cham_dm_mulpred_b16(const void* dS1, int lds1, int K, const void* Ws1b, const void* Z2c, const float* pred, int C, int BT, int N, void* dZ2c,
                        float* dpred_pre, float* col_part, void* stream);

int cham_combine_fwd_p3(const float* U, const float* V, int C, int BT, int N, int pmax, const int32_t* neg_slot, void* Z1p,
                        long long plane_stride, void* stream);
int cham_mulpred_bwd_p3(const float* dM, const float* Z2c, const float* pred, int C, int BT, int N, float* dpred_pre, void* dZ2p,
                        long long plane_stride, float* col_part, void* stream);

int cham_dm_mulpred_p3(const float* dS1, int lds1, int K, const void* Wp, long long w_plane_stride, const float* Z2c, const float* pred,
                       int C, int BT, int N, void* dZ2p, long long out_plane_stride, float* dpred_pre, float* col_part, void* stream);

int cham_gemm_b16(const void* A, int lda, int transA, const void* B, int ldb, int transB, void* C, int ldc, int out_f32, int M,
                  int N, int K, const float* bias, int act, const void* dref, int ldr, int dact, int accumulate, float* workspace,
                  size_t workspace_bytes, int splits_hint, void* stream);
void cham_gemm_b16_set_variant(int variant);
void cham_gemm_b16_launch_counts(long long* out8, int reset);

void cham_gemm_set_variant(int variant);
void cham_gemm_launch_counts(long long* out16, int reset);

int cham_combine_fwd(const float* U, const float* V, int C, int BT, int N, int pmax, const int32_t* neg_slot, float* Z1,
                     long row_begin, long row_count, void* stream);
size_t cham_combine_bwd_workspace_bytes(int C, int BT, int N, int pmax);
int cham_combine_bwd(const float* dpre, int C, int BT, int N, int pmax, const int32_t* neg_slot, float* dU, float* dV,
                     float* workspace, size_t workspace_bytes, void* stream);
size_t cham_gemm_h2_groupsum_bytes(int M, int N, int group_rows);
int cham_gemm_h2_dgrad_gs(const void* A, long long a_plane_stride, int lda, const float* a_scale, const void* B, long long b_plane_stride, int ldb,
                          const float* b_scale, float* C, int ldc, int M, int N, int K, const void* dref_h, int ldr, int a_tiles, int dref_blocked,
                          int group_rows, float* groupsum, size_t groupsum_bytes, void* stream);
int cham_combine_bwd_gs(const float* dpre, int C, int BT, int N, int pmax, const int32_t* neg_slot, float* dU, float* dV, float* workspace,
                        size_t workspace_bytes, const float* groupsum, size_t groupsum_bytes, void* stream);

int cham_combine_fwd_b16(const float* U, const float* V, int C, int BT, int N, int pmax, const int32_t* neg_slot, void* Z1c,
                         void* stream);
int cham_combine_bwd_b16(const float* dpre_in, const void* dpre_cand, int C, int BT, int N, int pmax, const int32_t* neg_slot,
                         float* dU, float* dV, float* workspace, size_t workspace_bytes, void* stream);
int cham_mulpred_bwd_b16(void* dM, const void* Z2c, const float* pred, int C, int BT, int N, float* dpred_pre, void* stream);
int cham_mul_rows_b16(const void* Z2c, const float* pred, int C, int BT, int NC, void* Mc, void* stream);
int cham_score_softmax_fwd_b16(const void* S3, int K3, const float* w4, const float* b4, int BT, int N, float tau,
                               const uint8_t* mask, float* logits, float* probs, float* nll, float novelty_reg_factor,
                               const int64_t* neg_ids, const float* pop_norm, float* nov_aux, void* stream);
int cham_score_softmax_bwd_b16(const void* S3, int K3, const float* w4, const float* probs, const uint8_t* mask, int BT, int N,
                               float tau, float sum_mask, float* ds, void* dS3, float novelty_reg_factor, const int64_t* neg_ids,
                               const float* pop_norm, const float* logits, const float* nov_aux, void* stream);
int cham_colsum_b16(const void* X, int ld, int R, int F, const float* w, float* out, int accumulate, float* workspace,
                    size_t workspace_bytes, void* stream);
int cham_cast_b16(const float* W, int R, int Cc, void* dst, void* dstT, void* stream);
int cham_upcast_b16(const void* src, size_t n, float* dst, void* stream);

int cham_rnn_fwd(int cell_kind, const float* xproj, const float* Wh, const int32_t* seq_len, int B, int T, int Hp, float* out,
                 float* hprev, float* G, float* Cc, float* R, float* RH, void* stream);
int cham_rnn_bwd(int cell_kind, const float* dout, const float* WhT, const int32_t* seq_len, int B, int T, int Hp,
                 const float* hprev, const float* G, const float* Cc, const float* R, float* dxproj, void* stream);
size_t cham_rnn_coop_workspace_bytes(int B, int Hp);
int cham_ugrnn_fwd_coop(const float* xproj, const float* Wh, const int32_t* seq_len, int B, int T, int Hp, float* out, float* hprev, float* G,
                        float* Cc, void* workspace, size_t workspace_bytes, void* stream);
int cham_ugrnn_bwd_coop(const float* dout, const float* Wh, const int32_t* seq_len, int B, int T, int Hp, const float* hprev, const float* G,
                        const float* Cc, float* dxproj, void* workspace, size_t workspace_bytes, void* stream);
int cham_rnn_coop_timeouts(const void* workspace, int B, int Hp, void* stream);
int cham_ugrnn_point_fwd(const float* xproj, const float* zh, const int32_t* seq_len, int B, int T, int t, int Hp, float* h,
                         float* out, float* hprev, float* G, float* Cc, void* stream);
int cham_ugrnn_point_bwd(const float* dout, const float* carry, const int32_t* seq_len, int B, int T, int t, int Hp,
                         const float* hprev, const float* G, const float* Cc, float* dxproj, float* dzs, float* direct,
                         void* stream);
int cham_transpose_f32(const float* in, int rows, int cols, float* out, void* stream);
int cham_rows_gather(const void* src, const int32_t* pos, long n_rows, int words, void* dst, void* stream);
int cham_rows_scatter(const void* src, const int32_t* pos, long n_rows, int words, void* dst, void* stream);

int cham_mulpred_bwd(float* dM, const float* Z2c, const float* pred, int C, int BT, int N, float* dpred_pre, void* stream);
int cham_score_softmax_fwd(const float* S3, int K3, const float* w4, const float* b4, int BT, int N, float tau,
                           const uint8_t* mask, float* logits, float* probs, float* nll, float novelty_reg_factor,
                           const int64_t* neg_ids, const float* pop_norm, float* nov_aux, void* stream);
int cham_score_softmax_bwd(const float* S3, int K3, const float* w4, const float* probs, const uint8_t* mask, int BT, int N,
                           float tau, float sum_mask, float* ds, float* dS3, float novelty_reg_factor, const int64_t* neg_ids,
                           const float* pop_norm, const float* logits, const float* nov_aux, void* stream);

int cham_rank_items(const float* probs, const int64_t* label_next, const int64_t* neg_ids, const uint8_t* mask, int BT, int N,
                    int64_t* pred_ids, float* pred_probs, int32_t* label_rank, void* stream);

size_t cham_state_workspace_bytes(int B, int buffer_size);
int cham_state_update(const int64_t* aci, const int64_t* event_ts, int B, int T, double buffer_hours, int64_t* buf_ids,
                      int64_t* buf_ts, int buffer_size, int32_t* recent_pop, float* pop_norm, int64_t* articles_pop, int n_items,
                      int for_norm, int32_t* n_valid, void* workspace, size_t workspace_bytes, void* stream);

int cham_sumsq_partial(const float* params, size_t n_reg, float* partial, void* stream);
int cham_loss_finalize(const float* nll, int BT, float sum_mask, const float* sumsq_partial, float lambda, float* loss,
                       void* stream);
int cham_adam_tf(float* params, const float* grads, float* m, float* v, size_t n, size_t n_reg, float lambda, float lr_t,
                 float beta1, float beta2, float eps, void* stream);
int cham_accumulate(float* acc, const float* x, size_t n, int first, void* stream);
int cham_loss_accumulate(float* acc, const float* loss, int first, void* stream);
size_t cham_colsum_workspace_bytes(int R, int F);
int cham_colsum(const float* X, int ld, int R, int F, const float* w, float* out, int accumulate, float* workspace,
                size_t workspace_bytes, void* stream);


int cham_step_scalars_bytes(void);
int cham_step_scalars_set(void* rec, uint32_t step, uint32_t step_next, int64_t max_ts, float sum_mask, float lr_t, int fields, void* stream);
int cham_neg_sample_dev(const int64_t* aci, int Bg, int T1, const int64_t* buffer, int buf_size, uint32_t seed, const void* scalars, int which,
                        int row_begin, int row_count, int N, int n_from_buffer, int64_t* neg_ids, int32_t* neg_slot, int64_t* pool, int32_t* canon,
                        int32_t* meta, void* workspace, size_t workspace_bytes, void* stream);
int cham_step_ints_dev(const int64_t* ic_rows, const int64_t* ln_rows, const int64_t* pool, const int64_t* ets_rows, const void* scalars, int BT,
                       int pmax, const int32_t* seq_len_in, int B, const uint8_t* mask_in, int64_t* ids_all, int64_t* ref_ts, int32_t* seq_len,
                       uint8_t* mask, void* stream);
int cham_norm_stats_from_buffer_dev(const int64_t* buffer_ids, int n_prefix, const void* scalars, const int64_t* created, const float* pop_norm,
                                    float* scratch, float* stats, void* stream);
int cham_score_softmax_bwd_dev(const float* S3, int K3, const float* w4, const float* probs, const uint8_t* mask, int BT, int N, float tau,
                               const void* scalars, float* ds, float* dS3, float novelty_reg_factor, const int64_t* neg_ids, const float* pop_norm,
                               const float* logits, const float* nov_aux, void* stream);
int cham_score_softmax_bwd_b16_dev(const void* S3, int K3, const float* w4, const float* probs, const uint8_t* mask, int BT, int N, float tau,
                                   const void* scalars, float* ds, void* dS3, float novelty_reg_factor, const int64_t* neg_ids,
                                   const float* pop_norm, const float* logits, const float* nov_aux, void* stream);
int cham_loss_finalize_dev(const float* nll, int BT, const void* scalars, const float* sumsq_partial, float lambda, float* loss, void* stream);
int cham_adam_tf_dev(float* params, const float* grads, float* m, float* v, size_t n, size_t n_reg, float lambda, const void* scalars,
// ... 16 lines not shown
```

Baseline: 34150.

## Pack Z1 sign bits in forward combine and use them in dgrad epilogue

The forward combine kernel now also writes a packed bitmask with one bit per Z1 element, recording whether it is positive. The backward dgrad GEMM epilogue reads 32-bit mask words instead of 16 fp16 high-plane values per element to apply the leaky-ReLU derivative. This cuts epilogue read traffic, at the cost of an extra mask buffer, mask writes in the forward pass, and more template variants in the epilogue.

```diff
diff --git a/chameleon_recsys_amd/_lib.py b/chameleon_recsys_amd/_lib.py
--- a/chameleon_recsys_amd/_lib.py
+++ b/chameleon_recsys_amd/_lib.py
@@ -81,6 +81,9 @@
     "cham_gemm_h2_groupsum_bytes": (c_size_t, [c_int, c_int, c_int]),
     "cham_gemm_h2_dgrad_gs": (c_int, [P, c_int64, c_int, P, P, c_int64, c_int, P, P, c_int, c_int, c_int, c_int, P, c_int, c_int, c_int, c_int, P,
                                       c_size_t, P]),
+    "cham_combine_fwd_h2m": (c_int, [P, P, c_int, c_int, c_int, c_int, P, P, c_int64, P, c_int, P, c_int, P]),
+    "cham_gemm_h2_dgrad_mask": (c_int, [P, c_int64, c_int, P, P, c_int64, c_int, P, c_int, P, c_int, c_int, c_int, c_int, P, c_int, P, c_int, c_int,
+                                        c_int, c_int, P, c_size_t, P]),
     "cham_combine_fwd_b16": (c_int, [P, P, c_int, c_int, c_int, c_int, P, P, P]),
     "cham_combine_bwd_b16": (c_int, [P, P, c_int, c_int, c_int, c_int, P, P, P, P, c_size_t, P]),
     "cham_mulpred_bwd_b16": (c_int, [P, P, P, c_int, c_int, c_int, P, P]),
diff --git a/chameleon_recsys_amd/csrc/common.h b/chameleon_recsys_amd/csrc/common.h
--- a/chameleon_recsys_amd/csrc/common.h
+++ b/chameleon_recsys_amd/csrc/common.h
@@ -156,6 +156,20 @@
     *reinterpret_cast<u16x4_t*>(p) = h;
     *reinterpret_cast<f16x4_t*>(p + ps) = l;
 }
+__device__ __forceinline__ unsigned st4_planes_h2_sign(_Float16* p, long long ps, const float4& v, float s) {
+    typedef unsigned short u16x4_t __attribute__((ext_vector_type(4)));
+    typedef _Float16 f16x4_t __attribute__((ext_vector_type(4)));
+    u16x4_t h; f16x4_t l;
+    _Float16 a, b;
+    split2h(v.x * s, a, b); h[0] = h2_keep_sign(a, v.x); l[0] = b;
+    split2h(v.y * s, a, b); h[1] = h2_keep_sign(a, v.y); l[1] = b;
+    split2h(v.z * s, a, b); h[2] = h2_keep_sign(a, v.z); l[2] = b;
+    split2h(v.w * s, a, b); h[3] = h2_keep_sign(a, v.w); l[3] = b;
+    *reinterpret_cast<u16x4_t*>(p) = h;
+    *reinterpret_cast<f16x4_t*>(p + ps) = l;
+    return ((short)h[0] > 0 ? 1u : 0u) | ((short)h[1] > 0 ? 2u : 0u) | ((short)h[2] > 0 ? 4u : 0u) | ((short)h[3] > 0 ? 8u : 0u);
+}
+__host__ __device__ __forceinline__ size_t h2_signmask_words(size_t rows, size_t ldm) { return ((rows + 31) >> 5) * ldm; }
 
 __device__ __forceinline__ float wave_sum(float v) {
 #pragma unroll
diff --git a/chameleon_recsys_amd/csrc/gemm_h2.hip b/chameleon_recsys_amd/csrc/gemm_h2.hip
--- a/chameleon_recsys_amd/csrc/gemm_h2.hip
+++ b/chameleon_recsys_amd/csrc/gemm_h2.hip
@@ -16,6 +16,7 @@
     int nbm, nbn, xcd_split, accumulate;
     int a_tiles, b_tiles, r_blk;
     float* gsum; int ggrp, gsk;
+    const unsigned* mask; int ldm;
 };
 
 #define H2_SLAB 8192
@@ -69,11 +70,30 @@
     __builtin_amdgcn_sched_barrier(0);
 }
 
+template <bool B> struct h2_flag { static constexpr bool value = B; };
 template <int EPI, int TM, int TNN>
 __device__ __forceinline__ void h2_epilogue(const H2Params& p, floatx16 (&acc)[TM][TNN], int m0, int n0, int wm0, int wn0, int split, int lane) {
     int lane_e = lane;
     asm volatile("" : "+v"(lane_e));
     const int kl = lane_e >> 5, fl = lane_e & 31;
+    unsigned mw[TM][TNN];
+    bool um = false;
+    if constexpr (EPI == 3) {
+        um = p.mask != nullptr;
+        if (um) {
+            const size_t first = (size_t)(m0 >> 5) * (size_t)p.ldm + (size_t)n0, bytes = (h2_signmask_words((size_t)p.M, (size_t)p.ldm) - first) * 4;
+            const __amdgpu_buffer_rsrc_t mwin =
+                __builtin_amdgcn_make_buffer_rsrc(const_cast<unsigned*>(p.mask + first), 0, (int)min(bytes, (size_t)WINDOW_BYTES), 0x00020000);
+#pragma unroll
+            for (int i = 0; i < TM; ++i)
+#pragma unroll
+                for (int j = 0; j < TNN; ++j) {
+                    const bool ok = wm0 + i * 32 < p.M - m0 && wn0 + j * 32 + fl < p.N - n0;
+                    const unsigned off = ((unsigned)((wm0 >> 5) + i) * (unsigned)p.ldm + (unsigned)(wn0 + j * 32 + fl)) * 4u;
+                    mw[i][j] = __builtin_amdgcn_raw_buffer_load_b32(mwin, ok ? off : OOB_OFF, 0, 0);
+                }
+        }
+    }
     const float ia = p.sa[1], ib = p.sb[1];
 #pragma unroll
     for (int i = 0; i < TM; ++i)
@@ -85,8 +105,9 @@
         const int limM = p.M - m0, limN = p.N - n0;
         const __amdgpu_buffer_rsrc_t cw = make_window(p.C + (size_t)m0 * p.ldc + n0);
         const bool rb = p.r_blk != 0;
-        const __amdgpu_buffer_rsrc_t dw = make_window(rb ? p.dref + ((size_t)(m0 >> 8) * (size_t)(p.ldr >> 5) + (size_t)(n0 >> 5)) * H2B_BLOCK
-                                                         : p.dref + (size_t)m0 * p.ldr + n0);
+        const __amdgpu_buffer_rsrc_t dw = make_window(um ? (const void*)p.C
+                                                      : rb ? (const void*)(p.dref + ((size_t)(m0 >> 8) * (size_t)(p.ldr >> 5) + (size_t)(n0 >> 5)) * H2B_BLOCK)
+                                                           : (const void*)(p.dref + (size_t)m0 * p.ldr + n0));
         const int rstride = rb ? 64 : p.ldr * 2;
         const bool gs = p.gsum != nullptr;
         const int G = gs ? p.ggrp : 1, rbase = m0 + wm0;
@@ -139,63 +160,85 @@
             for (int j = 0; j < TNN; ++j) cur[j] = hik[j];
         };
         if (limM >= wm0 + TM * 32 && limN >= wn0 + TNN * 32) {
+            auto interior = [&](auto MK) {
+#pragma unroll
+                for (int i = 0; i < TM; ++i) {
+                    block_begin(i);
+#pragma unroll
+                    for (int j = 0; j < TNN; ++j) {
+                        const unsigned col = (unsigned)(wn0 + j * 32 + fl), rowb = (unsigned)(wm0 + i * 32 + 4 * kl);
+                        const unsigned voff = (rowb * (unsigned)p.ldc + col) * 4u;
+                        float v[16];
+                        if constexpr (decltype(MK)::value) {
+                            const unsigned w = mw[i][j] >> (4 * kl);
+#pragma unroll
+                            for (int e = 0; e < 16; ++e) {
+                                const int ce = (e & 3) + 8 * (e >> 2);
+                                v[e] = acc[i][j][e] * ((w & (1u << ce)) != 0u ? 1.f : 0.2f);
+                                __builtin_amdgcn_raw_buffer_store_b32(__float_as_uint(v[e]), cw, voff, ce * p.ldc * 4, 0);
+                            }
+                        } else {
+                            const unsigned voffr = rb ? (unsigned)((wn0 >> 5) + j) * (unsigned)(H2B_BLOCK * 2) + rowb * 64u + (unsigned)fl * 2u
+                                                      : (rowb * (unsigned)p.ldr + col) * 2u;
+                            unsigned short y[16];
+#pragma unroll
+                            for (int e = 0; e < 16; ++e) {
+                                const int ce = (e & 3) + 8 * (e >> 2);
+                                y[e] = __builtin_amdgcn_raw_buffer_load_b16(dw, voffr, ce * rstride, 0);
+                            }
+#pragma unroll
+                            for (int e = 0; e < 16; ++e) {
+                                const int ce = (e & 3) + 8 * (e >> 2);
+                                v[e] = acc[i][j][e] * ((short)y[e] > 0 ? 1.f : 0.2f);
+                                __builtin_amdgcn_raw_buffer_store_b32(__float_as_uint(v[e]), cw, voff, ce * p.ldc * 4, 0);
+                            }
+                        }
+                        block_add(j, v);
+                    }
+                    block_end();
+                }
+                if (gs) emit();
+            };
+            if (um) interior(h2_flag<true>{}); else interior(h2_flag<false>{});
+            return;
+        }
+        auto edge = [&](auto MK) {
 #pragma unroll
             for (int i = 0; i < TM; ++i) {
                 block_begin(i);
 #pragma unroll
                 for (int j = 0; j < TNN; ++j) {
-                    const unsigned col = (unsigned)(wn0 + j * 32 + fl), rowb = (unsigned)(wm0 + i * 32 + 4 * kl);
-                    const unsigned voff = (rowb * (unsigned)p.ldc + col) * 4u;
-                    const unsigned voffr = rb ? (unsigned)((wn0 >> 5) + j) * (unsigned)(H2B_BLOCK * 2) + rowb * 64u + (unsigned)fl * 2u
-                                              : (rowb * (unsigned)p.ldr + col) * 2u;
+                    const int col = wn0 + j * 32 + fl;
+                    const bool cok = col < limN;
                     unsigned short y[16];
+                    unsigned offs[16];
 #pragma unroll
                     for (int e = 0; e < 16; ++e) {
-                        const int ce = (e & 3) + 8 * (e >> 2);
-                        y[e] = __builtin_amdgcn_raw_buffer_load_b16(dw, voffr, ce * rstride, 0);
+                        const int row = wm0 + i * 32 + (e & 3) + 8 * (e >> 2) + 4 * kl;
+                        const bool ok = cok && row < limM;
+                        offs[e] = ok ? ((unsigned)row * (unsigned)p.ldc + (unsigned)col) * 4u : OOB_OFF;
+                        if constexpr (!decltype(MK)::value) {
+                            const unsigned ro = rb ? (unsigned)((wn0 >> 5) + j) * (unsigned)(H2B_BLOCK * 2) + (unsigned)row * 64u + (unsigned)fl * 2u
+                                                   : ((unsigned)row * (unsigned)p.ldr + (unsigned)col) * 2u;
+                            y[e] = __builtin_amdgcn_raw_buffer_load_b16(dw, ok ? ro : OOB_OFF, 0, 0);
+                        }
                     }
+                    const unsigned w = decltype(MK)::value ? mw[i][j] >> (4 * kl) : 0u;
                     float v[16];
 #pragma unroll
                     for (int e = 0; e < 16; ++e) {
-                        const int ce = (e & 3) + 8 * (e >> 2);
-                        v[e] = acc[i][j][e] * ((short)y[e] > 0 ? 1.f : 0.2f);
-                        __builtin_amdgcn_raw_buffer_store_b32(__float_as_uint(v[e]), cw, voff, ce * p.ldc * 4, 0);
+                        bool pos;
+                        if constexpr (decltype(MK)::value) pos = (w & (1u << ((e & 3) + 8 * (e >> 2)))) != 0u;
+                        else pos = (short)y[e] > 0;
+                        v[e] = acc[i][j][e] * (pos ? 1.f : 0.2f);
+                        __builtin_amdgcn_raw_buffer_store_b32(__float_as_uint(v[e]), cw, offs[e], 0, 0);
                     }
                     block_add(j, v);
                 }
                 block_end();
             }
-            if (gs) emit();
-            return;
-        }
-#pragma unroll
-        for (int i = 0; i < TM; ++i) {
-            block_begin(i);
-#pragma unroll
-            for (int j = 0; j < TNN; ++j) {
-                const int col = wn0 + j * 32 + fl;
-                const bool cok = col < limN;
-                unsigned short y[16];
-                unsigned offs[16];
-#pragma unroll
-                for (int e = 0; e < 16; ++e) {
-                    const int row = wm0 + i * 32 + (e & 3) + 8 * (e >> 2) + 4 * kl;
-                    const bool ok = cok && row < limM;
-                    offs[e] = ok ? ((unsigned)row * (unsigned)p.ldc + (unsigned)col) * 4u : OOB_OFF;
-                    const unsigned ro = rb ? (unsigned)((wn0 >> 5) + j) * (unsigned)(H2B_BLOCK * 2) + (unsigned)row * 64u + (unsigned)fl * 2u
-                                           : ((unsigned)row * (unsigned)p.ldr + (unsigned)col) * 2u;
-                    y[e] = __builtin_amdgcn_raw_buffer_load_b16(dw, ok ? ro : OOB_OFF, 0, 0);
-                }
-                float v[16];
-#pragma unroll
-                for (int e = 0; e < 16; ++e) {
-                    v[e] = acc[i][j][e] * ((short)y[e] > 0 ? 1.f : 0.2f);
-                    __builtin_amdgcn_raw_buffer_store_b32(__float_as_uint(v[e]), cw, offs[e], 0, 0);
-                }
-                block_add(j, v);
-            }
-            block_end();
-        }
+        };
+        if (um) edge(h2_flag<true>{}); else edge(h2_flag<false>{});
         if (gs) emit();
     } else {
         GemmParams g;
@@ -729,9 +772,12 @@
 static int h2_run(const void* A, long long a_plane_stride, int lda, const float* a_scale, const void* B, long long b_plane_stride,
                   int ldb, const float* b_scale, int tn, float* C, int ldc, int M, int N, int K, const float* bias, int act,
                   const void* dref_h, int ldr, int dact, int accumulate, float* workspace, size_t workspace_bytes, int splits_hint,
-                  int a_tiles, int b_tiles, int dref_blocked, int group_rows, float* groupsum, size_t groupsum_bytes, void* stream) {
+                  int a_tiles, int b_tiles, int dref_blocked, int group_rows, float* groupsum, size_t groupsum_bytes, const void* sign_mask, int ldm,
+                  void* stream) {
     if (!A || !B || !C || !a_scale || !b_scale || M <= 0 || N <= 0 || K <= 0 || a_tiles < 0 || b_tiles < 0) return -CHAM_ERR_ARG;
-    if (groupsum && (tn || !dref_h || group_rows < 32 || groupsum_bytes < cham_gemm_h2_groupsum_bytes(M, N, group_rows) || ((uintptr_t)groupsum & 15)))
+    if (sign_mask && (tn || ((uintptr_t)sign_mask & 15) || ldm < N || (ldm & 3) || (size_t)ldm * 4 * 8 >= WINDOW_BYTES)) return -CHAM_ERR_ARG;
+    const bool dgrad = dref_h || sign_mask;
+    if (groupsum && (tn || !dgrad || group_rows < 32 || groupsum_bytes < cham_gemm_h2_groupsum_bytes(M, N, group_rows) || ((uintptr_t)groupsum & 15)))
         return -CHAM_ERR_ARG;
     {
         const long a_rows = tn ? K : M, b_rows = tn ? K : N;
@@ -750,25 +796,26 @@
     p.nbm = (M + 255) / 256; p.nbn = (N + 255) / 256;
     p.a_tiles = a_tiles; p.b_tiles = b_tiles; p.r_blk = dref_blocked ? 1 : 0;
     p.gsum = groupsum; p.ggrp = group_rows; p.gsk = groupsum ? 127 / group_rows + 2 : 0;
+    p.mask = reinterpret_cast<const unsigned*>(sign_mask); p.ldm = ldm;
     hipStream_t st = (hipStream_t)stream;
     if (!tn) {
         if ((K & 15) || accumulate) return -CHAM_ERR_ARG;
         if ((size_t)256 * lda * 2 >= (1ull << 31) || (size_t)256 * ldb * 2 >= (1ull << 31)) return -CHAM_ERR_ARG;
         p.kchunk = K; p.splits = 1;
-        if (dref_h && (bias || act != ACT_NONE || dact != ACT_LEAKY)) return -CHAM_ERR_ARG;
+        if (dgrad && (bias || act != ACT_NONE || dact != ACT_LEAKY)) return -CHAM_ERR_ARG;
         if (act != ACT_NONE && !(bias && act == ACT_TANH)) return -CHAM_ERR_ARG;
         ++g_h2_launches[0];
         if (groupsum) ++g_h2_launches[5];
         if (g_h2_nt_wide && (K & 31) == 0) {
-            if (dref_h) return h2w_launch<3>(p, st);
+            if (dgrad) return h2w_launch<3>(p, st);
             if (bias) return act == ACT_TANH ? h2w_launch<2>(p, st) : h2w_launch<5>(p, st);
             return h2w_launch<0>(p, st);
         }
-        if (dref_h) return h2_launch<false, 3>(p, st);
+        if (dgrad) return h2_launch<false, 3>(p, st);
         if (bias) return act == ACT_TANH ? h2_launch<false, 2>(p, st) : h2_launch<false, 5>(p, st);
         return h2_launch<false, 0>(p, st);
     }
-    if ((M & 255) || (N & 255) || bias || act != ACT_NONE || dref_h) return -CHAM_ERR_ARG;
+    if ((M & 255) || (N & 255) || bias || act != ACT_NONE || dgrad) return -CHAM_ERR_ARG;
     if ((size_t)16 * lda * 2 >= (1ull << 31) || (size_t)16 * ldb * 2 >= (1ull << 31)) return -CHAM_ERR_ARG;
     const long tiles = (long)p.nbm * p.nbn;
     int splits = 1;
@@ -810,14 +857,22 @@
                              const void* dref_h, int ldr, int dact, int accumulate, float* workspace, size_t workspace_bytes, int splits_hint,
                              int a_tiles, int b_tiles, int dref_blocked, void* stream) {
     return h2_run(A, a_plane_stride, lda, a_scale, B, b_plane_stride, ldb, b_scale, tn, C, ldc, M, N, K, bias, act, dref_h, ldr, dact, accumulate,
-                  workspace, workspace_bytes, splits_hint, a_tiles, b_tiles, dref_blocked, 0, nullptr, 0, stream);
+                  workspace, workspace_bytes, splits_hint, a_tiles, b_tiles, dref_blocked, 0, nullptr, 0, nullptr, 0, stream);
 }
 extern "C" int cham_gemm_h2_dgrad_gs(const void* A, long long a_plane_stride, int lda, const float* a_scale, const void* B, long long b_plane_stride,
                                      int ldb, const float* b_scale, float* C, int ldc, int M, int N, int K, const void* dref_h, int ldr,
                                      int a_tiles, int dref_blocked, int group_rows, float* groupsum, size_t groupsum_bytes, void* stream) {
     if (!groupsum) return -CHAM_ERR_ARG;
     return h2_run(A, a_plane_stride, lda, a_scale, B, b_plane_stride, ldb, b_scale, 0, C, ldc, M, N, K, nullptr, ACT_NONE, dref_h, ldr, ACT_LEAKY, 0,
-                  nullptr, 0, 1, a_tiles, 0, dref_blocked, group_rows, groupsum, groupsum_bytes, stream);
+                  nullptr, 0, 1, a_tiles, 0, dref_blocked, group_rows, groupsum, groupsum_bytes, nullptr, 0, stream);
+}
+extern "C" int cham_gemm_h2_dgrad_mask(const void* A, long long a_plane_stride, int lda, const float* a_scale, const void* B, long long b_plane_stride,
+                                       int ldb, const float* b_scale, int tn, float* C, int ldc, int M, int N, int K, const float* bias, int act,
+                                       const void* sign_mask, int ldm, int dact, int a_tiles, int group_rows, float* groupsum, size_t groupsum_bytes,
+                                       void* stream) {
+    if (!sign_mask) return -CHAM_ERR_ARG;
+    return h2_run(A, a_plane_stride, lda, a_scale, B, b_plane_stride, ldb, b_scale, tn, C, ldc, M, N, K, bias, act, nullptr, 0, dact, 0,
+                  nullptr, 0, 1, a_tiles, 0, 0, group_rows, groupsum, groupsum_bytes, sign_mask, ldm, stream);
 }
 
 extern "C" int cham_gemm_h2(const void* A, long long a_plane_stride, int lda, const float* a_scale, const void* B, long long b_plane_stride,
diff --git a/chameleon_recsys_amd/csrc/scorer.hip b/chameleon_recsys_amd/csrc/scorer.hip
--- a/chameleon_recsys_amd/csrc/scorer.hip
+++ b/chameleon_recsys_amd/csrc/scorer.hip
@@ -111,6 +111,57 @@
                 o.z = act_fwd(a.z + b[i].z, ACT_LEAKY); o.w = act_fwd(a.w + b[i].w, ACT_LEAKY);
                 st4_planes_h2(blocked ? Z1p + h2b_index(grow0 + (size_t)(c0 + i), 4u * (unsigned)k, ncb) : po + (size_t)(c0 + i) * C + 4 * k, ps, o, sc);
             }
+        }
+    }
+}
+
+#define COMBINE_MASK_ROWS 64
+__global__ __launch_bounds__(256) void k_combine_fwd_cand_h2m(const float* __restrict__ U, const float* __restrict__ V, int C,
+                                                              int BT, int N, int pmax, const int* __restrict__ neg_slot,
+                                                              _Float16* __restrict__ Z1p , long long ps,
+                                                              const H2Scale* __restrict__ rec, int blocked, unsigned* __restrict__ mask, int ldm) {
+    const int NC = N + 1;
+    const long M = (long)BT * NC;
+    const long r0 = (long)blockIdx.x * COMBINE_MASK_ROWS;
+    const float sc = rec->scale;
+    const unsigned ncb = (unsigned)C >> 5;
+    const int bt0 = (int)(r0 / NC), c0 = (int)(r0 - (long)bt0 * NC);
+    for (int k = threadIdx.x; k < C / 4; k += 256) {
+        int bt = bt0, c = c0;
+        int abt = -1;
+        float4 a = make_float4(0.f, 0.f, 0.f, 0.f);
+        for (int h = 0; h < COMBINE_MASK_ROWS / 32; ++h) {
+            const long w0 = r0 + 32 * h;
+            if (w0 >= M) break;
+            unsigned bits[4] = {0u, 0u, 0u, 0u};
+            for (int g = 0; g < 32; g += 4) {
+                if (w0 + g >= M) break;
+                float4 b[4], au[4];
+#pragma unroll
+                for (int i = 0; i < 4; ++i) {
+                    const bool in = w0 + g + i < M;
+                    const int bti = in ? bt : BT - 1, ci = in ? c : NC - 1;
+                    if (bti != abt) au[i] = reinterpret_cast<const float4*>(U + (size_t)bti * C)[k];
+                    else au[i] = i == 0 ? a : au[i - 1];
+                    abt = bti;
+                    b[i] = reinterpret_cast<const float4*>(V + (size_t)cand_vrow(bti, ci, BT, N, pmax, neg_slot) * C)[k];
+                    if (++c == NC) { c = 0; ++bt; }
+                }
+                a = au[3];
+#pragma unroll
+                for (int i = 0; i < 4; ++i) {
+                    const long row = w0 + g + i;
+                    if (row >= M) break;
+                    float4 o;
+                    o.x = act_fwd(au[i].x + b[i].x, ACT_LEAKY); o.y = act_fwd(au[i].y + b[i].y, ACT_LEAKY);
+                    o.z = act_fwd(au[i].z + b[i].z, ACT_LEAKY); o.w = act_fwd(au[i].w + b[i].w, ACT_LEAKY);
+                    const unsigned nib = st4_planes_h2_sign(blocked ? Z1p + h2b_index((size_t)row, 4u * (unsigned)k, ncb) : Z1p + (size_t)row * C + 4 * k, ps, o, sc);
+                    const unsigned sh = (unsigned)(g + i);
+                    bits[0] |= (nib & 1u) << sh; bits[1] |= ((nib >> 1) & 1u) << sh; bits[2] |= ((nib >> 2) & 1u) << sh; bits[3] |= (nib >> 3) << sh;
+                }
+            }
+            uint4 wv; wv.x = bits[0]; wv.y = bits[1]; wv.z = bits[2]; wv.w = bits[3];
+            *reinterpret_cast<uint4*>(mask + (size_t)(w0 >> 5) * ldm + 4 * k) = wv;
         }
     }
 }
@@ -584,6 +635,20 @@
     return CHAM_OK;
 }
 
+extern "C" int cham_combine_fwd_h2m(const float* U, const float* V, int C, int BT, int N, int pmax, const int32_t* neg_slot, void* Z1p,
+                                    long long plane_stride, const void* scale_rec, int blocked, void* sign_mask, int ldm, void* stream) {
+    if (!U || !V || !neg_slot || !Z1p || !scale_rec || C <= 0 || (C & 3) || BT < 0 || N < 0 || (plane_stride & 3)) return -CHAM_ERR_ARG;
+    if (blocked && ((C & 31) || plane_stride < (long long)(((size_t)BT * (N + 1) + 255) / 256) * (C >> 5) * H2B_BLOCK)) return -CHAM_ERR_ARG;
+    if (!sign_mask || ((uintptr_t)sign_mask & 15) || ldm < C || (ldm & 3)) return -CHAM_ERR_ARG;
+    if (BT == 0) return CHAM_OK;
+    const size_t rows = (size_t)BT * (N + 1);
+    hipLaunchKernelGGL(k_combine_fwd_cand_h2m, dim3((unsigned)((rows + COMBINE_MASK_ROWS - 1) / COMBINE_MASK_ROWS)), dim3(256), 0, (hipStream_t)stream,
+                       U, V, C, BT, N, pmax, neg_slot, reinterpret_cast<_Float16*>(Z1p), plane_stride, reinterpret_cast<const H2Scale*>(scale_rec),
+                       blocked ? 1 : 0, reinterpret_cast<unsigned*>(sign_mask), ldm);
+    CHAM_CHECK_LAUNCH();
+    return CHAM_OK;
+}
+
 static inline size_t al256(size_t x) { return (x + 255) & ~(size_t)255; }
 struct SlotWs { size_t bitmap_bytes, partial_bytes, pad_bytes; int W, nchunk, nchunk_pad; };
 static SlotWs slot_ws(int C, int BT, int N, int pmax) {
diff --git a/chameleon_recsys_amd/nar/nar_model.py b/chameleon_recsys_amd/nar/nar_model.py
--- a/chameleon_recsys_amd/nar/nar_model.py
+++ b/chameleon_recsys_amd/nar/nar_model.py
@@ -156,6 +156,7 @@
         self.dev_scalars = os.environ.get("CHAM_DEV_SCALARS", "1") == "1"
         self.loss_side = os.environ.get("CHAM_LOSS_SIDE", "1") == "1"
         self.dgrad_groupsum = os.environ.get("CHAM_DGRAD_GROUPSUM", "1") == "1"
+        self.dgrad_signmask = os.environ.get("CHAM_DGRAD_SIGNMASK", "1") == "1"
         self.feature_bwd_ws = os.environ.get("CHAM_FEATURE_BWD_WS", "1") == "1"
         self.tail_split = os.environ.get("CHAM_TAIL_SPLIT", "1") == "1"
         self.capturing = False
@@ -465,7 +466,7 @@
                              bias=bias is not None, rowscale=False, bf16=False, p3=True, tile=0, epi=int(c[6]), ev=(e0, e1)))
 
     def gemm_h2(self, A, a_ps, lda, a_sc, B, b_ps, ldb, b_sc, tn, C, ldc, M, N, K, bias=None, act=ACT_NONE, dref_h=None, ldr=0, dact=ACT_NONE,
-                accumulate=0, splits=1, a_tiles=0, b_tiles=0, dref_blocked=0, group_rows=0, groupsum=None):
+                accumulate=0, splits=1, a_tiles=0, b_tiles=0, dref_blocked=0, group_rows=0, groupsum=None, sign_mask=None, ldm=0):
         ws = None
         if splits != 1:
             ws = self._lane_ws('gemm_ws')
@@ -476,7 +477,11 @@
             self.lib.cham_gemm_h2_launch_counts(c0, 0)
             e0, e1 = torch.cuda.Event(enable_timing=True), torch.cuda.Event(enable_timing=True)
             e0.record()
-        if groupsum is not None:
+        if sign_mask is not None:
+            check(self.lib.cham_gemm_h2_dgrad_mask(ptr(A), a_ps, lda, ptr(a_sc), ptr(B), b_ps, ldb, ptr(b_sc), tn, ptr(C), ldc, M, N, K, ptr(bias), act,
+                                                   ptr(sign_mask), ldm, dact, a_tiles, group_rows if groupsum is not None else 0, ptr(groupsum),
+                                                   groupsum.numel() * 4 if groupsum is not None else 0, _stream()), "cham_gemm_h2_dgrad_mask")
+        elif groupsum is not None:
             check(self.lib.cham_gemm_h2_dgrad_gs(ptr(A), a_ps, lda, ptr(a_sc), ptr(B), b_ps, ldb, ptr(b_sc), ptr(C), ldc, M, N, K, ptr(dref_h), ldr,
                                                  a_tiles, dref_blocked, group_rows, ptr(groupsum), groupsum.numel() * 4, _stream()), "cham_gemm_h2_dgrad_gs")
         else:
@@ -487,7 +492,7 @@
             e1.record()
             c = (ctypes.c_longlong * 8)()
             self.lib.cham_gemm_h2_launch_counts(c, 0)
-            prof.append(dict(M=M, N=N, K=K, transA=tn, transB=0 if tn else 1, splits=int(c[7]), act=act, dref=dref_h is not None, dact=dact,
+            prof.append(dict(M=M, N=N, K=K, transA=tn, transB=0 if tn else 1, splits=int(c[7]), act=act, dref=dref_h is not None or sign_mask is not None, dact=dact,
                              bias=bias is not None, rowscale=False, bf16=False, h2=True, h2w=bool(c[2] > c0[2]), h2blk=bool(c[3] > c0[3]), tile=0, epi=int(c[6]), ev=(e0, e1)))
 
     def _tile_counts_b16(self):
@@ -650,6 +655,7 @@
                 self.sc_ds1 = torch.zeros(8, dtype=torch.float32, device=dev)
                 self.gsum = (torch.empty(int(rt.lib.cham_gemm_h2_groupsum_bytes(Rc, C, NC)) // 4, dtype=torch.float32, device=dev)
                              if rt.dgrad_groupsum and NC >= 32 and Rc > 0 else None)
+                self.z1_mask = None
             else:
                 self.Z1p, self.dZ2p = bf(3, Rc, C), bf(3, Rc, C)
             self.p3_ps = Rc * C
@@ -698,6 +704,13 @@
             if hasattr(self, 'nbytes'):
                 self.nbytes = self.allocated_bytes()
         return t
+
+    def ensure_signmask(self):
+        if self.z1_mask is None:
+            self.z1_mask = torch.empty(-(-self.Rc // 32), self.C, dtype=torch.int32, device=self.Z1p.device)
+            if hasattr(self, 'nbytes'):
+                self.nbytes = self.allocated_bytes()
+        return self.z1_mask
 
     def dropout_buffers(self, rt):
         if not rt.b16:
@@ -972,7 +985,7 @@
         B, T, N = d['B'], d['T'], self.negative_samples
         pl = rt.plan(B, T, N, self.negative_sample_from_buffer, d['Bg'])
         self._plan, self._d = pl, d
-        pl.used_p3 = False
+        pl.used_p3 = pl.used_mask = False
         check(lib.cham_set_log_bases(self.elapsed_days_smooth_log_base, self.popularity_smooth_log_base), "cham_set_log_bases")
         if d.get('uploaded') is not None:
             torch.cuda.current_stream().wait_event(d['uploaded'])
@@ -1166,8 +1179,14 @@
                 rt.gemm(pl.Xd[BT:], self._drop['W1'], pl.Z1[BT:], Rc, C, Fc + Fi, Fc + Fi, C, C, bias=p('b1'), act=ACT_LEAKY)
             elif use_p3 and rt.h2:
                 check(lib.cham_h2_scale_absmax(ptr(pl.U), BT * C, ptr(pl.V), RV * C, ptr(pl.sc_z1), s), "cham_h2_scale_absmax")
-                check(lib.cham_combine_fwd_h2b(ptr(pl.U), ptr(pl.V), C, BT, N, pmax, ptr(neg_slot), ptr(pl.Z1p), pl.z1_ps, ptr(pl.sc_z1), 1 if pl.z1_tiles else 0, s),
-                      "cham_combine_fwd_h2")
+                pl.used_mask = self.is_training and rt.dgrad_signmask
+                if pl.used_mask:
+                    mask = pl.ensure_signmask()
+                    check(lib.cham_combine_fwd_h2m(ptr(pl.U), ptr(pl.V), C, BT, N, pmax, ptr(neg_slot), ptr(pl.Z1p), pl.z1_ps, ptr(pl.sc_z1),
+                                                   1 if pl.z1_tiles else 0, ptr(mask), C, s), "cham_combine_fwd_h2m")
+                else:
+                    check(lib.cham_combine_fwd_h2b(ptr(pl.U), ptr(pl.V), C, BT, N, pmax, ptr(neg_slot), ptr(pl.Z1p), pl.z1_ps, ptr(pl.sc_z1),
+                                                   1 if pl.z1_tiles else 0, s), "cham_combine_fwd_h2")
             elif use_p3:
                 check(lib.cham_combine_fwd_p3(ptr(pl.U), ptr(pl.V), C, BT, N, pmax, ptr(neg_slot), ptr(pl.Z1p), pl.p3_ps, s), "cham_combine_fwd_p3")
             else:
@@ -1385,8 +1404,12 @@
                 rt.gemm_p3(pl.Z1p, pl.p3_ps, C, pl.dZ2p, pl.p3_ps, C, 1, g('W2'), C, C, C, Rc, splits=splits)
         if h2:
             gsum = getattr(pl, 'gsum', None) if not drop else None
-            rt.gemm_h2(pl.dZ2p, pl.dz2_ps, C, pl.sc_dz2, rt.w2p, C * C, C, rt.sc_w2, 0, pl.dZ1[BT:], C, Rc, C, C, dref_h=pl.Z1p, ldr=C, dact=ACT_LEAKY,
-                       a_tiles=pl.dz2_tiles, dref_blocked=1 if pl.z1_tiles else 0, group_rows=NC, groupsum=gsum)
+            if getattr(pl, 'used_mask', False):
+                rt.gemm_h2(pl.dZ2p, pl.dz2_ps, C, pl.sc_dz2, rt.w2p, C * C, C, rt.sc_w2, 0, pl.dZ1[BT:], C, Rc, C, C, dact=ACT_LEAKY,
+                           a_tiles=pl.dz2_tiles, group_rows=NC, groupsum=gsum, sign_mask=pl.z1_mask, ldm=C)
+            else:
+                rt.gemm_h2(pl.dZ2p, pl.dz2_ps, C, pl.sc_dz2, rt.w2p, C * C, C, rt.sc_w2, 0, pl.dZ1[BT:], C, Rc, C, C, dref_h=pl.Z1p, ldr=C, dact=ACT_LEAKY,
+                           a_tiles=pl.dz2_tiles, dref_blocked=1 if pl.z1_tiles else 0, group_rows=NC, groupsum=gsum)
         elif use_p3:
             rt.gemm_p3(pl.dZ2p, pl.p3_ps, C, rt.w2p, C * C, C, 0, pl.dZ1[BT:], C, Rc, C, C, dref_h=pl.Z1p, ldr=C, dact=ACT_LEAKY)
         elif not b16 and Rc > 0:
diff --git a/include/chameleon_nar.h b/include/chameleon_nar.h
--- a/include/chameleon_nar.h
+++ b/include/chameleon_nar.h
@@ -152,6 +152,12 @@
                           int group_rows, float* groupsum, size_t groupsum_bytes, void* stream);
 int cham_combine_bwd_gs(const float* dpre, int C, int BT, int N, int pmax, const int32_t* neg_slot, float* dU, float* dV, float* workspace,
                         size_t workspace_bytes, const float* groupsum, size_t groupsum_bytes, void* stream);
+int cham_combine_fwd_h2m(const float* U, const float* V, int C, int BT, int N, int pmax, const int32_t* neg_slot, void* Z1p,
+                         long long plane_stride, const void* scale_rec, int blocked, void* sign_mask, int ldm, void* stream);
+int cham_gemm_h2_dgrad_mask(const void* A, long long a_plane_stride, int lda, const float* a_scale, const void* B, long long b_plane_stride,
+                            int ldb, const float* b_scale, int tn, float* C, int ldc, int M, int N, int K, const float* bias, int act,
+                            const void* sign_mask, int ldm, int dact, int a_tiles, int group_rows, float* groupsum, size_t groupsum_bytes,
+                            void* stream);
 
 int cham_combine_fwd_b16(const float* U, const float* V, int C, int BT, int N, int pmax, const int32_t* neg_slot, void* Z1c,
                          void* stream);
```

Result: no change. 34260 (median of 6 runs) (+0.3%).
